# bkj/pytorch-graphsage

Measured on AMD Instinct MI355X. Metric: seed-nodes/sec, higher is better.
Workload: dtype bf16; 1 GPU; Reddit-shaped mean-aggregator 2-layer fanout 25/10 hidden 128/128 (BASELINE configs[1]); N=232965 D=602 nnz=98191232; batch_per_gpu=512, global_batch=512, rng=philox, engine=fused, launch=cmdlist, pipelined=False, batch_queue=True, parallelism=dp1, ranks=1

## Files before the change

include/gsage.h:

```cpp
#ifndef GSAGE_H
#define GSAGE_H

#include <stdint.h>

#ifdef __cplusplus
extern "C" {
#endif

#define GSAGE_ABI_VERSION 6

enum { GSAGE_F32 = 0, GSAGE_BF16 = 1, GSAGE_FP8 = 2 };
enum {
    GSAGE_OK = 0,
    GSAGE_EINVAL = -1,
    GSAGE_ELAUNCH = -2,
    GSAGE_ENODEV = -3
};
enum { GSAGE_POOL_MAX = 0, GSAGE_POOL_MEAN = 1 };
enum { GSAGE_ACT_NONE = 0, GSAGE_ACT_RELU = 1, GSAGE_ACT_TANH = 2 };

int gsage_abi_version(void);
const char *gsage_last_error(void);
uint64_t gsage_launch_count(void);
int gsage_debug_abort_trace(int fd);
int gsage_device_info(char *arch, int arch_len, int *cu_count, int *wave_size);

int gsage_stream_create_masked(const uint32_t *cu_mask, int32_t words, void **stream);
int gsage_stream_destroy(void *stream);
int gsage_event_create(void **event);
void gsage_event_destroy(void *event);
int gsage_cmdlist_replay_pair(const void *list_a, void *stream_a, void *wait_a, void *record_a,
                              const void *list_b, void *stream_b, void *wait_b, void *record_b,
                              void *then_wait_stream, int then_wait_on_b);
int gsage_cmdlist_begin(void);
int gsage_cmdlist_end(void **list);
int gsage_cmdlist_mark(int slot);
int gsage_cmdlist_time_next(int slot_a, int slot_b);
int gsage_cmdlist_elapsed(const void *list, int slot_a, int slot_b, float *ms);
int64_t gsage_cmdlist_size(const void *list);
int gsage_cmdlist_replay(const void *list, void *stream);
int gsage_cmdlist_side_begin(void);
int gsage_cmdlist_side_end(void);
int gsage_cmdlist_join(void);
void gsage_cmdlist_destroy(void *list);
typedef int (*gsage_host_fn)(void *ctx, void *stream);
int gsage_host_call(gsage_host_fn fn, void *ctx, void *stream);

int gsage_comm_load(const char *path);
int gsage_comm_unique_id(void *id128);
int gsage_comm_create(const void *id128, int32_t rank, int32_t world, void **comm);
int gsage_comm_destroy(void *comm);
int gsage_comm_all_reduce_f32(void *comm, float *buf, int64_t n, int32_t average, void *stream);
int gsage_comm_all_gather(void *comm, const void *send, void *recv, int64_t bytes, void *stream);
int gsage_comm_group(void *comm, int32_t begin, void *stream);


int gsage_sample_csr_sel(const int64_t *rowptr, const int32_t *col, int64_t n_rows,
                         const int64_t *ids, int64_t M, int32_t n, const int32_t *sel,
                         int64_t *out, int32_t *err_flag, void *stream);

int gsage_sample_dense(const int64_t *adj, int64_t ld, int64_t n_rows, const int64_t *ids, int64_t M,
                       const int64_t *keep, int32_t n, int64_t *out, int32_t *err_flag, void *stream);

int gsage_sample_csr_philox(const int64_t *rowptr, const int32_t *col, int64_t n_rows,
                            const int64_t *ids, int64_t M, int32_t n, uint32_t max_deg,
                            uint64_t seed, const uint64_t *call_ctr, uint64_t call_base,
                            uint64_t g0, int64_t *out, int32_t *sel_out, int32_t *err_flag,
                            void *stream);

int gsage_sample_hops_philox(const int64_t *rowptr, const int32_t *col, int64_t n_rows, int64_t *ids,
                             int64_t B, int32_t n_hops, const int32_t *fan, uint32_t max_deg,
                             uint64_t seed, const uint64_t *call_ctr, uint64_t call_base,
                             uint64_t rank, const int64_t *seed_queue, const int64_t *batch_idx,
                             int64_t n_batches, int32_t *err_flag, void *stream);
typedef struct gsage_hops_desc {
    const int64_t *rowptr;
    const int32_t *col;
    int64_t n_rows;
    int64_t *ids;
    int64_t B;
    int32_t n_hops;
    int32_t fan[5];
    uint32_t max_deg;
    uint64_t seed;
    const uint64_t *call_ctr;
    uint64_t call_base;
    uint64_t rank;
    const int64_t *seed_queue;
    const int64_t *batch_idx;
    int64_t batch_base;
    int64_t n_batches;
    int32_t *err_flag;
    const int32_t *sel;
    int64_t sel_stride;
    const int64_t *dense_adj;
    int64_t dense_ld;
} gsage_hops_desc;
int gsage_sample_hops(const gsage_hops_desc *hops, void *stream);

int gsage_counter_add(uint64_t *ctr, uint64_t inc, void *stream);
int gsage_copy_pair(void *dst0, const void *src0, int64_t bytes0, void *dst1, const void *src1, int64_t bytes1,
                    void *stream);

void *gsage_mt_create(uint32_t seed);
void gsage_mt_destroy(void *mt);
void gsage_mt_seed(void *mt, uint32_t seed);
int64_t gsage_mt_choice_i32(void *mt, int64_t high, int64_t count, int32_t *out);
int gsage_mt_choice_device(uint32_t *state, int64_t high, int64_t count, int32_t *out, void *stream);
int gsage_mt_choice_segments(uint32_t *state, int64_t high, int64_t n_seg, const int64_t *seg_off,
                             const int64_t *seg_cnt, int32_t *out, void *stream);

int gsage_mt_choice_par(uint32_t *state, int64_t high, int64_t n_seg, const int64_t *seg_cum, const int64_t *seg_off,
                        int64_t n_total, int32_t *out, const uint64_t *table, void *scratch, int64_t scratch_bytes,
                        int32_t n_wg, int32_t units_per_wg, void *stream);
int64_t gsage_mt_choice_par_scratch(int32_t n_wg);
int gsage_mt_jump_table(uint64_t *out, int64_t words);
int64_t gsage_mt_jump_table_words(void);
int gsage_mt_jump_host(const uint32_t *state, const uint64_t *poly, uint32_t *out);
void gsage_mt_permutation(void *mt, int64_t n, int64_t *out);

int gsage_gather_mean(const void *table, int dtype, int64_t ld, const int64_t *ids, int64_t M,
                      int32_t n, int64_t D, void *out, int out_dtype, int64_t out_ld,
                      void *stream);

int gsage_gather_mean_multi(int32_t n_seg, const void *const *tables, const int64_t *const *ids,
                            void *const *outs, const int64_t *M, const int32_t *n, int dtype,
                            int64_t ld, int64_t D, int out_dtype, int64_t out_ld, void *stream);

int gsage_quantize_fp8(const void *table, int dtype, int64_t ld, int64_t n_rows, int64_t D, void *table_q,
                       int64_t ld_q, float *scale, void *stream);

int gsage_gather_rows_fp8(const void *table_q, int64_t ld, const float *scale, const int64_t *ids, int64_t M,
                          int64_t D, void *out, int out_dtype, int64_t out_ld, void *stream);

int gsage_gather_mean_fp8(const void *table_q, int64_t ld, const float *scale, const int64_t *ids, int64_t M,
                          int32_t n, int64_t D, void *out, int out_dtype, int64_t out_ld, void *stream);
int gsage_gather_mean_multi_fp8(int32_t n_seg, const void *const *tables_q, const int64_t *const *ids,
                                void *const *outs, const int64_t *M, const int32_t *n, const float *scale,
                                int64_t ld, int64_t D, int out_dtype, int64_t out_ld, void *stream);

int gsage_segment_mean_bwd(const float *dagg, int64_t ld, int64_t M, int32_t n, int64_t D,
                           float *dneibs, int64_t out_ld, void *stream);

int gsage_scatter_add_rows(const float *rows, int64_t ld, const int64_t *ids, int64_t M,
                           int32_t n, int64_t D, float scale, float *table_grad,
                           int64_t table_ld, void *stream);

int gsage_linear_nt(const void *A, int dtype, int64_t lda, const int64_t *a_rows,
                    int a_rows_group0_only, const void *W, int64_t ldw, const float *bias,
                    void *C, int c_dtype, int64_t ldc, int64_t M, int64_t N, int64_t K, int act,
                    int groups, int64_t a_gstride, int64_t w_gstride, int64_t c_gstride,
                    void *stream);

int64_t gsage_packed_weight_elems(int64_t N, int64_t K, int32_t groups);
int gsage_pack_weight(const void *W, int dtype, int64_t ldw, int64_t w_gstride, int64_t N, int64_t K,
                      int32_t groups, void *Wp, void *stream);
int gsage_linear_nt_packed(const void *A, int64_t lda, const int64_t *a_rows, int a_rows_group0_only,
                           const void *Wp, const float *bias, void *C, int c_dtype, int64_t ldc,
                           int64_t M, int64_t N, int64_t K, int act, int groups, int64_t a_gstride,
                           int64_t c_gstride, void *stream);

int gsage_wgrad(const void *dC, int dtype, int64_t ldc, const void *A, int64_t lda, int64_t a_gstride, int64_t M,
                int64_t Ntot, int64_t K,
                int64_t n_per_group, int64_t rows_per_split, float *slabs, int64_t ldk, float *out,
                int64_t out_gstride, void *stream);
int gsage_wgrad_slabs(int64_t M, int64_t rows_per_split);
typedef struct gsage_wgrad_desc {
    const void *dC;
    const void *A;
    float *slabs;
    int64_t ldc, lda, a_gstride;
    int64_t M, Ntot, K, n_per_group, ldk, rows_per_split;
    const int64_t *a_rows;
} gsage_wgrad_desc;
int gsage_wgrad_multi(int32_t n_prob, const gsage_wgrad_desc *probs, int dtype, void *stream);
int gsage_wgrad_pair_ok(int dtype, int64_t M, int64_t Ntot, int64_t n_per_group, int64_t rows_per_split);
int gsage_wgrad_ticks_next(int64_t *tick, int64_t *tick1, int64_t inc1, int64_t *tick2, int64_t inc2);

int gsage_pool_mlp(const void *A, int dtype, int64_t lda, const int64_t *a_rows, const void *W,
                   int64_t ldw, const float *bias, int64_t M, int32_t n, int64_t H, int64_t K,
                   int pool, float *pooled, int64_t pooled_ld, int32_t *argmax, void *pooled_bf16,
                   int64_t pooled_bf16_ld, uint32_t *relu_mask, void *stream);

int gsage_pool_mlp_packed(const void *A, int64_t lda, const int64_t *a_rows, const void *Wp,
                          const float *bias, int64_t M, int32_t n, int64_t H, int64_t K, int pool,
                          float *pooled, int64_t pooled_ld, int32_t *argmax, void *pooled_bf16,
                          int64_t pooled_bf16_ld, uint32_t *relu_mask, void *stream);

int gsage_pool_route_bwd(const float *g, int64_t ldg, const float *pooled, int64_t ldp,
                         const int32_t *argmax, int64_t lda, int64_t M, int32_t n, int32_t H, void *out,
                         int out_dtype, int64_t ldo, void *stream);

int gsage_pool_route_mean_bwd(const float *g, int64_t ldg, const uint32_t *relu_mask, int64_t M, int32_t n,
                              int32_t H, void *out, int out_dtype, int64_t ldo, float *bias_part, int32_t n_part,
                              void *stream);

int gsage_pool_bias_partials(const float *g, int64_t ldg, const float *pooled, int64_t ldp, int64_t M,
                             int32_t H, float *part, int32_t n_part, void *stream);

int gsage_pool_merge_bwd(const void *Hprev, int dtype, int64_t ldh, const float *DX, int64_t ldx, int64_t r_x,
                         const float *DN, int64_t ldn, int64_t r0, void *dH, int64_t ldo, int64_t R,
                         int32_t D, void *stream);

int gsage_attn_aggregate(const float *na, int64_t na_ld, const float *xa, int64_t xa_ld,
                         const void *table, int dtype, int64_t ld, const int64_t *ids, int64_t M,
                         int32_t n, int64_t Ha, int64_t D, float *agg, int64_t agg_ld, float *ws,
                         void *stream);
int gsage_attn_aggregate_lp(const float *na, int64_t na_ld, const float *xa, int64_t xa_ld, const void *table,
                            int dtype, int64_t ld, const int64_t *ids, int64_t M, int32_t n, int64_t Ha, int64_t D,
                            float *agg, int64_t agg_ld, float *ws, void *agg_lp, int64_t agg_lp_ld, void *stream);
int gsage_attn_mlp2_fwd(const void *hid, int dtype, int64_t ldh, const void *W2, int64_t ldw, float *a, int64_t lda,
                        int64_t M, int32_t Ha, void *stream);
int gsage_attn_mlp2_bwd(const float *dan, int64_t ldn, const float *dax, int64_t ldx, const void *hid, int dtype,
                        int64_t ldh, const void *W2T, int64_t ldw, void *da, int64_t ldda, void *dhid, int64_t lddh,
                        int64_t M, int32_t Ha, void *stream);
int gsage_attn_bwd(const float *g, int64_t g_ld, const float *ws, const float *na, int64_t na_ld,
                   const float *xa, int64_t xa_ld, const void *table, int dtype, int64_t ld,
                   const int64_t *ids, int64_t M, int32_t n, int64_t Ha, int64_t D, float *dna,
                   int64_t dna_ld, float *dxa, int64_t dxa_ld, void *stream);

int gsage_attn_fused_ok(int dtype, int64_t ld, int64_t D, int32_t n, int64_t Ha);
int gsage_attn_fused_fwd(const void *table, int dtype, int64_t ld, const int64_t *ids, int64_t row0, const void *W0,
                         int64_t ldw0, const void *W2, int64_t ldw2, const float *xa, int64_t xa_ld, int64_t M,
                         int32_t n, int64_t D, void *hid, int64_t hid_ld, float *a, int64_t a_ld, float *ws, void *agg_lp,
                         int64_t lp_ld, void *stream);
int gsage_attn_fused_bwd(const void *table, int dtype, int64_t ld, const int64_t *ids, int64_t row0, const void *W2T,
                         int64_t ldw2t, const float *g, int64_t g_ld, const float *ws, const float *na, int64_t na_ld,
                         const float *xa, int64_t xa_ld, const void *hid, int64_t hid_ld, int64_t M, int32_t n, int64_t D,
                         void *da, int64_t da_ld, void *dhid, int64_t dhid_ld, float *dxa, int64_t dxa_ld, void *stream);

int gsage_prep_rows_ok(int dtype, int64_t E);
int gsage_prep_rows_fwd(const float *table, int64_t ldt, const int64_t *ids, int64_t n_seed, int64_t spare, const void *W,
                        int64_t ldw, const float *bias, int64_t M, int64_t E, void *eraw, int64_t lde, void *out,
                        int64_t ldo, void *stream);
int gsage_prep_rows_bwd(const void *dhid, int64_t lddh, const void *W0T, int64_t ldw0t, const float *DATT, int64_t ldatt,
                        const float *DX, int64_t ldx, int64_t r_x, const float *DAGG, int64_t ldagg, const float *ws,
                        int32_t n_hops, const int64_t *off, const int32_t *fan, int64_t R, int64_t E, void *din0,
                        int64_t ldd, float *bias_part, int32_t n_part, const void *WpT, int64_t ldwpt, const int64_t *ids,
                        int64_t n_seed, int64_t spare, float *g_table, int64_t ldg, float *deraw, int64_t ldde,
                        void *stream);

int gsage_lstm_ok(int dtype, int64_t H, int32_t n);
int gsage_lstm_tile(int dtype, int64_t M, int64_t H, int backward);
int64_t gsage_lstm_packed_elems(int64_t H);
int gsage_lstm_pack_whh(const float *W_hh, int64_t ldw, int64_t H, int dtype, void *Wp, void *stream);
int gsage_lstm_fwd(void *gates, int dtype, int64_t ldg, const void *Wp, int64_t M, int32_t n, int64_t H, float *cseq,
                   void *hprev, int64_t ldh, void *out, int64_t ldo, void *stream);
int gsage_lstm_bwd(const void *gates, int dtype, int64_t ldg, const void *Wp, int64_t M, int32_t n, int64_t H,
                   const float *cseq, const float *dh, int64_t lddh, void *dG, int64_t lddg, float *carry, void *stream);

int gsage_add_cast(const float *a, int64_t lda, const float *b, int64_t ldb, void *dst, int dst_dtype, int64_t ldd,
                   int64_t M, int64_t D, void *stream);
int gsage_tanh_bwd(const float *g, int64_t ldg, const void *hid, int dtype, int64_t ldh, void *out, int64_t ldo,
                   int64_t M, int64_t D, void *stream);
int gsage_attn_merge_bwd(const void *H, int h_dtype, int64_t ldh, const float *DATT, int64_t ldatt, const float *DX,
                         int64_t ldx, int64_t r_x, const float *DAGG, int64_t ldagg, const float *ws, void *out,
                         int out_dtype, int64_t ldo, int64_t R, int32_t D, int32_t n_hops, const int64_t *off,
                         const int32_t *fan, void *stream);
int gsage_attn_merge_bwd2(const void *H, int h_dtype, int64_t ldh, const float *DATT, int64_t ldatt, const float *DX,
                         int64_t ldx, int64_t r_x, const float *DAGG, int64_t ldagg, const float *ws, void *out,
                         int out_dtype, int64_t ldo, int64_t R, int32_t D, int32_t n_hops, const int64_t *off,
                         const int32_t *fan, void *out2_bf16, int64_t ldo2,
                          void *stream);

int gsage_head_l1(const float *E, int64_t lde, const float *W, const float *bias, const float *targets, int64_t B,
                  int64_t D, float *preds, void *dE, int dE_dtype, int64_t ldd, float *scratch, void *stream);
int gsage_head_l1_scratch(int64_t B, int64_t D);
int gsage_head_l1_sharded(const float *E, int64_t lde, const float *W, const float *bias, const float *targets,
                          int64_t T, int64_t B, int64_t D, float *preds, void *dE, int dE_dtype, int64_t ldd,
                          float *scratch, void *stream);

int gsage_head_ce(const float *E, int64_t lde, const float *W, const float *bias,
                  const int64_t *targets, int32_t B, int32_t C, int32_t D, float *preds, void *dE,
                  int dE_dtype, int64_t ldd, float *dW, float *db, float *loss, float *scratch,
                  const int64_t *batch_idx, int64_t n_batches, void *stream);
int64_t gsage_head_ce_scratch(int32_t B, int32_t C, int32_t D);

int gsage_head_wide(const float *E, int64_t lde, const float *W, const float *bias, const void *targets, int task,
                    int64_t ldy, int32_t B, int32_t C, int32_t D, float *preds, void *dE, int dE_dtype, int64_t ldd,
                    float *dW, float *db, float *loss, float *scratch, const int64_t *batch_idx, int64_t n_batches,
                    void *stream);
int64_t gsage_head_wide_scratch(int32_t B, int32_t C, int32_t D);

typedef struct gsage_tail_gather_desc {
    const void *table;
    const int64_t *ids;
    void *out;
    int64_t ld, out_ld, D, rows;
    int32_t n, n_workgroups;
} gsage_tail_gather_desc;
int gsage_mean_tail_ce(const void *H, int32_t B, int32_t n, const void *w2, int64_t ldw2,
                       const void *w2t, int64_t ldw2t, const float *Wfc, const float *bfc, int32_t C,
                       const int64_t *targets, const int64_t *batch_idx, int64_t n_batches, void *agg,
                       void *dE, float *preds, void *dH, float *partial,
                       const gsage_tail_gather_desc *gather, int dtype, void *stream);
int gsage_gather_role_next(const gsage_tail_gather_desc *gather);
int gsage_hops_role_next(const gsage_hops_desc *hops);
int64_t gsage_mean_tail_ce_scratch(int32_t B, int32_t C);
int gsage_mean_tail_mfma(const void *H, int32_t B, int32_t n, const void *w2, int64_t ldw2,
                         const void *w2t, int64_t ldw2t, const float *Wfc, const float *bfc, int32_t C,
                         const int64_t *targets, const int64_t *batch_idx, int64_t n_batches, void *agg,
                         void *dE, float *preds, void *dH, float *partial,
                         const gsage_tail_gather_desc *gather, void *stream);
int64_t gsage_mean_tail_mfma_scratch(int32_t B, int32_t C);
int32_t gsage_mean_tail_mfma_sampler_wgs(int64_t B, int64_t widest);


int gsage_clip_adam_step(float *p, float *g, float *m, float *v, int64_t n, float *partial,
                         const float *lr, int64_t *step, float beta1, float beta2, float eps,
                         float weight_decay, float max_norm, float *norm_out, int step_is_current,
                         int32_t n_partial_ready, const void *prep_descs, int32_t n_prep,
                         int64_t *tick1, int64_t inc1, int64_t *tick2, int64_t inc2, void *stream);
typedef struct gsage_adam_desc {
    float *p, *g, *m, *v;
    int64_t n;
    float *partial;
    const float *lr;
    int64_t *step;
    float beta1, beta2, eps, weight_decay, max_norm;
    float *norm_out;
    int32_t step_is_current, n_partial_ready;
    const void *prep_descs;
    int32_t n_prep;
    int64_t *tick1;
    int64_t inc1;
    int64_t *tick2;
    int64_t inc2;
    uint64_t *norm_slots;
    const void *reduce_descs;
    int32_t n_reduce;
} gsage_adam_desc;
int gsage_clip_adam_meet(const gsage_adam_desc *adam, void *stream);
int gsage_gather_adam_capacity(int dtype, int64_t lds_bytes);
int gsage_head_n_valid_next(const int32_t *n_valid);
int gsage_head_n_valid_pending(void);

int gsage_gather_mean_multi_adam(int32_t n_seg, const void *const *tables, const int64_t *const *ids,
                                 void *const *outs, const int64_t *M, const int32_t *n, int dtype,
                                 int64_t ld, int64_t D, int out_dtype, int64_t out_ld,
                                 const gsage_adam_desc *adam, const gsage_hops_desc *hops, void *stream);

typedef struct {
    const float *src;
    int64_t stride;
    int64_t out_off;
    int32_t S, rows, cols, ld;
} gsage_reduce_desc;
int gsage_finalize_grads(const void *descs, int32_t n_desc, int64_t max_elems, float *flat_g,
                         float *partial_sq, int64_t *tick, int64_t *tick1, int64_t inc1,
                         int64_t *tick2, int64_t inc2, void *stream);
int gsage_finalize_partials(int32_t n_desc, int64_t max_elems);
int gsage_grad_sqnorm(const float *g, int64_t n, float *partial, int32_t n_partial, void *stream);
int gsage_zero_rows(float *table, int64_t ld, const int64_t *ids, int64_t M, int64_t D, void *stream);
int gsage_colsum_partials(const float *src, int64_t ld, int64_t M, int32_t D, float *part, int32_t n_part, void *stream);
int gsage_adam_partials(int64_t n);

typedef struct gsage_row_adam {
    float *p, *g, *m, *v;
    int32_t *last, *seen;
    float *hist;
    const float *lr;
    const int64_t *step;
    int64_t n_rows;
    int32_t E, hist_cap;
    float beta1, beta2, eps, weight_decay, max_norm;
    int32_t sorted_ids;
} gsage_row_adam;
int gsage_rows_catch_up(const gsage_row_adam *d, const int64_t *ids0, int64_t n0, const int64_t *ids1, int64_t n1,
                        int32_t step_off, void *stream);
int gsage_rows_catch_up_all(const gsage_row_adam *d, int32_t step_off, void *stream);
int gsage_rows_sqnorm(const gsage_row_adam *d, const int64_t *ids0, int64_t n0, const int64_t *ids1, int64_t n1,
                      int32_t step_off, float *partial, int32_t n_partial, void *stream);
int gsage_rows_adam(const gsage_row_adam *d, const int64_t *ids0, int64_t n0, const int64_t *ids1, int64_t n1,
                    int32_t step_off, const float *partial, int32_t n_partial_ready, void *stream);

int64_t gsage_sort_rows_temp_bytes(int64_t n, int32_t key_bits);
int gsage_sort_rows(const int64_t *ids0, int64_t n0, int64_t tail_id, int64_t n_tail, int32_t key_bits,
                    int64_t *ids_sorted, int32_t *pos_sorted, void *temp, int64_t temp_bytes, void *stream);
int gsage_segment_sum_rows(const int64_t *ids_sorted, const int32_t *pos_sorted, int64_t n, const float *rows0,
                           int64_t ld0, int64_t n0, const float *rows1, int64_t ld1, int32_t E, float scale,
                           float *table, int64_t ldt, void *stream);

typedef struct {
    const float *src;
    uint16_t *dst;
    uint16_t *dst_t;
    int32_t rows, cols, dst_ld, dst_t_ld;
    uint16_t *dst_p;
    int64_t kc_p;
    int32_t dst_f32;
    int32_t reserved;
} gsage_prep_desc;
int gsage_prep_weights(const void *descs, int32_t n_desc, int64_t max_elems, int64_t *tick0,
                       int64_t inc0, int64_t *tick1, int64_t inc1, void *stream);

int gsage_bwd_merge(const void *H, int dtype, int64_t ldh, const float *DG, int64_t ldg, int64_t dagg_off,
                    void *dH, int64_t ldo, int64_t R, int64_t r_x, int32_t D, int32_t n_hops,
                    const int64_t *off, const int32_t *fan, void *stream);

int gsage_metric_f1(const float *logits, int64_t ld, const void *targets, int multilabel, int targets_f32,
                    int64_t ldy, int64_t B, int32_t C, int32_t *counts, double *out, void *stream);
int gsage_metric_mae(const float *y_true, const float *y_pred, int64_t n, double *out, void *stream);

enum { GSAGE_SEG_MEAN = 0, GSAGE_SEG_MAX = 1, GSAGE_SEG_SOFTMAX_WEIGHTED = 2, GSAGE_SEG_WEIGHTED_MEAN = 3 };
int64_t gsage_segment_reduce_ldp(int64_t D);
int gsage_segment_reduce(int mode, const void *table, int dtype, int64_t ld, int64_t D, const float *keys,
                         int64_t ldk, const int64_t *rowptr, const int32_t *col, int64_t n_rows,
                         const int32_t *order, int64_t n_short, const int64_t *slices, int64_t n_slices,
                         const int64_t *long_rows, int64_t n_long, int32_t slice_len, float *partials,
                         int64_t ldp, void *out, int out_dtype, int64_t out_ld, int act, int32_t *err_flag,
                         void *stream);

int gsage_unsup_batch(const int64_t *rowptr, const int32_t *col, int64_t n_rows, const int64_t *seeds, int64_t B,
                      int32_t walk_len, int64_t Q, const double *cdf, double cdf_total, uint64_t seed,
                      const uint64_t *call_ctr, uint64_t call_base, uint64_t g0, int64_t *ids, float *pair_w,
                      int32_t *err_flag, void *stream);

int gsage_head_skipgram(const float *E, int64_t lde, int32_t B, int32_t Q, int32_t D, const float *pair_w,
                        float neg_weight, void *dE, int dE_dtype, int64_t ldd, float *loss, float *aff, float *scratch,
                        void *stream);
int64_t gsage_head_skipgram_scratch(int32_t B, int32_t Q, int32_t D);

int gsage_head_skipgram_live(const float *E, int64_t lde, int32_t B, int32_t Q, int32_t D, const float *pair_w,
                             float neg_weight, const int32_t *n_valid, void *dE, int dE_dtype, int64_t ldd, float *loss,
                             float *aff, float *scratch, void *stream);

int gsage_edge_cdf_build(const int64_t *rowptr, const float *weight, int64_t n_rows, uint64_t *cdf, void *stream);
int gsage_sample_csr_weighted(const int64_t *rowptr, const int32_t *col, const uint64_t *cdf, int64_t n_rows,
                              const int64_t *ids, int64_t M, int32_t n, uint64_t seed, const uint64_t *call_ctr,
                              uint64_t call_base, uint64_t g0, int64_t *out, int32_t *err_flag, void *stream);
int gsage_segment_reduce_weighted(const void *table, int dtype, int64_t ld, int64_t D, const int64_t *rowptr,
                                  const int32_t *col, const uint64_t *cdf, int64_t n_rows, const int32_t *order,
                                  int64_t n_short, const int64_t *slices, int64_t n_slices, const int64_t *long_rows,
                                  int64_t n_long, int32_t slice_len, float *partials, int64_t ldp, void *out,
                                  int out_dtype, int64_t out_ld, int act, int32_t *err_flag, void *stream);

int64_t gsage_closure_span(void);
int gsage_closure_seed_count(const int64_t *queries, int64_t nq, int64_t n_rows, int32_t *local, int64_t *sums,
                             int64_t *counts, int32_t *err_flag, void *stream);
int gsage_closure_seed_write(const int64_t *queries, int64_t nq, int64_t n_rows, int32_t *local, const int64_t *sums,
                             int64_t *set, int64_t n_set, int64_t *pos, void *stream);
int gsage_closure_expand_count(const int64_t *rowptr, const int32_t *col, int64_t n_rows, const int64_t *set, int64_t lo,
                               int64_t hi, const int32_t *local, uint32_t *bitmap, int64_t *sums_words,
                               int64_t *sums_rows, int64_t *counts, int32_t *err_flag, void *stream);
int gsage_closure_expand_write(const int64_t *rowptr, const int32_t *col, const uint64_t *cdf, int64_t n_rows,
                               int64_t *set, int64_t n_dst, int32_t *local, uint32_t *bitmap, const int64_t *sums_words,
                               const int64_t *sums_rows, int64_t *blk_rowptr, int32_t *blk_col, uint64_t *blk_cdf,
                               int32_t *err_flag, void *stream);
int gsage_closure_restore(const int64_t *set, int64_t n, int32_t *local, void *stream);
int gsage_segment_reduce_block(int mode, const void *table, int dtype, int64_t ld, int64_t D, const float *keys,
                               int64_t ldk, const int64_t *rowptr, const int32_t *col, const uint64_t *cdf,
                               int64_t n_dst, int64_t n_src, int64_t dummy, const int32_t *order, int64_t n_short,
                               const int64_t *slices, int64_t n_slices, const int64_t *long_rows, int64_t n_long,
                               int32_t slice_len, float *partials, int64_t ldp, void *out, int out_dtype,
                               int64_t out_ld, int act, int32_t *err_flag, void *stream);

int64_t gsage_topk_ip_workspace(int64_t Q, int64_t N, int64_t k, int64_t splits, int64_t *splits_used);
int gsage_topk_ip(const void *table, int table_dtype, int64_t ldt, int64_t N, const void *queries, int query_dtype,
                  int64_t ldq, int64_t Q, int64_t D, const int64_t *query_ids, const int64_t *rowptr,
                  const int32_t *col, int exclude, int32_t k, int32_t splits, void *workspace, int64_t workspace_bytes,
                  int64_t *out_ids, float *out_scores, void *stream);

int64_t gsage_rank_ip_workspace(int64_t Q, int64_t N, int64_t splits, int64_t *splits_used);
int gsage_rank_ip(const void *table, int table_dtype, int64_t ldt, int64_t N, const void *queries, int query_dtype,
                  int64_t ldq, int64_t Q, int64_t D, const int64_t *target_ids, const int64_t *query_ids,
                  const int64_t *rowptr, const int32_t *col, int exclude, int32_t splits, void *workspace,
                  int64_t workspace_bytes, int64_t *out_rank, float *out_score, int32_t *err_flag, void *stream);

int64_t gsage_probe_pass_scratch(int64_t n, int32_t C, int32_t D, int32_t splits);
int gsage_probe_loss_index_next(const int64_t *index);
int gsage_probe_pass(const void *table, int dtype, int64_t ldx, int64_t N, const int64_t *ids, int64_t n,
                     const void *targets, int task, int64_t ldy, const float *W, const float *bias, int32_t C,
                     int32_t D, int32_t splits, float *partial, float *loss_out, void *stream);

#ifdef __cplusplus
}
#endif
#endif
```

pytorch-graphsage_amd/_native.py:

```python
import ctypes
import os

_HERE = os.path.dirname(os.path.abspath(__file__))
LIB_PATH = os.path.join(_HERE, "libgsage_hip.so")

F32, BF16, FP8 = 0, 1, 2
POOL_MAX, POOL_MEAN = 0, 1
ACT_NONE, ACT_RELU, ACT_TANH = 0, 1, 2
SEG_MEAN, SEG_MAX, SEG_SOFTMAX_WEIGHTED, SEG_WEIGHTED_MEAN = 0, 1, 2, 3
ABI_VERSION = 6

_vp = ctypes.c_void_p
_i64 = ctypes.c_int64
_i32 = ctypes.c_int32
_u32 = ctypes.c_uint32
_u64 = ctypes.c_uint64
_int = ctypes.c_int
_f32 = ctypes.c_float

SIGNATURES = {
    "gsage_abi_version": (_int, []),
    "gsage_last_error": (ctypes.c_char_p, []),
    "gsage_launch_count": (_u64, []),
    "gsage_debug_abort_trace": (_int, [_int]),
    "gsage_device_info": (_int, [ctypes.c_char_p, _int, ctypes.POINTER(_int), ctypes.POINTER(_int)]),
    "gsage_stream_create_masked": (_int, [_vp, _i32, ctypes.POINTER(_vp)]),
    "gsage_stream_destroy": (_int, [_vp]),
    "gsage_event_create": (_int, [ctypes.POINTER(_vp)]),
    "gsage_event_destroy": (None, [_vp]),
    "gsage_cmdlist_replay_pair": (_int, [_vp, _vp, _vp, _vp, _vp, _vp, _vp, _vp, _vp, _int]),
    "gsage_cmdlist_begin": (_int, []),
    "gsage_cmdlist_end": (_int, [ctypes.POINTER(_vp)]),
    "gsage_cmdlist_mark": (_int, [_int]),
    "gsage_cmdlist_time_next": (_int, [_int, _int]),
    "gsage_cmdlist_elapsed": (_int, [_vp, _int, _int, ctypes.POINTER(_f32)]),
    "gsage_cmdlist_size": (_i64, [_vp]),
    "gsage_cmdlist_replay": (_int, [_vp, _vp]),
    "gsage_cmdlist_side_begin": (_int, []),
    "gsage_cmdlist_side_end": (_int, []),
    "gsage_cmdlist_join": (_int, []),
    "gsage_cmdlist_destroy": (None, [_vp]),
    "gsage_host_call": (_int, [_vp, _vp, _vp]),
    "gsage_comm_load": (_int, [ctypes.c_char_p]),
    "gsage_comm_unique_id": (_int, [_vp]),
    "gsage_comm_create": (_int, [_vp, _i32, _i32, ctypes.POINTER(_vp)]),
    "gsage_comm_destroy": (_int, [_vp]),
    "gsage_comm_all_reduce_f32": (_int, [_vp, _vp, _i64, _i32, _vp]),
    "gsage_comm_all_gather": (_int, [_vp, _vp, _vp, _i64, _vp]),
    "gsage_comm_group": (_int, [_vp, _i32, _vp]),
    "gsage_sort_rows_temp_bytes": (_i64, [_i64, _i32]),
    "gsage_sort_rows": (_int, [_vp, _i64, _i64, _i64, _i32, _vp, _vp, _vp, _i64, _vp]),
    "gsage_segment_sum_rows": (_int, [_vp, _vp, _i64, _vp, _i64, _i64, _vp, _i64, _i32, _f32, _vp, _i64, _vp]),
    "gsage_head_l1_sharded": (_int, [_vp, _i64, _vp, _vp, _vp, _i64, _i64, _i64, _vp, _vp, _int, _i64, _vp, _vp]),
    "gsage_sample_csr_sel": (_int, [_vp, _vp, _i64, _vp, _i64, _i32, _vp, _vp, _vp, _vp]),
    "gsage_sample_dense": (_int, [_vp, _i64, _i64, _vp, _i64, _vp, _i32, _vp, _vp, _vp]),
    "gsage_sample_csr_philox": (_int, [_vp, _vp, _i64, _vp, _i64, _i32, _u32, _u64, _vp, _u64, _u64,
                                       _vp, _vp, _vp, _vp]),
    "gsage_sample_hops_philox": (_int, [_vp, _vp, _i64, _vp, _i64, _i32, _vp, _u32, _u64, _vp, _u64, _u64,
                                        _vp, _vp, _i64, _vp, _vp]),
    "gsage_sample_hops": (_int, [_vp, _vp]),
    "gsage_counter_add": (_int, [_vp, _u64, _vp]),
    "gsage_copy_pair": (_int, [_vp, _vp, _i64, _vp, _vp, _i64, _vp]),
    "gsage_mt_create": (_vp, [_u32]),
    "gsage_mt_destroy": (None, [_vp]),
    "gsage_mt_seed": (None, [_vp, _u32]),
    "gsage_mt_choice_i32": (_i64, [_vp, _i64, _i64, _vp]),
    "gsage_mt_permutation": (None, [_vp, _i64, _vp]),
    "gsage_mt_choice_device": (_int, [_vp, _i64, _i64, _vp, _vp]),
    "gsage_mt_choice_segments": (_int, [_vp, _i64, _i64, _vp, _vp, _vp, _vp]),
    "gsage_mt_choice_par": (_int, [_vp, _i64, _i64, _vp, _vp, _i64, _vp, _vp, _vp, _i64, _i32, _i32, _vp]),
    "gsage_mt_choice_par_scratch": (_i64, [_i32]),
    "gsage_mt_jump_table": (_int, [_vp, _i64]),
    "gsage_mt_jump_table_words": (_i64, []),
    "gsage_mt_jump_host": (_int, [_vp, _vp, _vp]),
    "gsage_head_n_valid_next": (_int, [_vp]),
    "gsage_head_n_valid_pending": (_int, []),
    "gsage_gather_role_next": (_int, [_vp]),
    "gsage_hops_role_next": (_int, [_vp]),
    "gsage_gather_mean": (_int, [_vp, _int, _i64, _vp, _i64, _i32, _i64, _vp, _int, _i64, _vp]),
    "gsage_gather_mean_multi": (_int, [_i32, _vp, _vp, _vp, _vp, _vp, _int, _i64, _i64, _int, _i64, _vp]),
    "gsage_gather_mean_multi_adam": (_int, [_i32, _vp, _vp, _vp, _vp, _vp, _int, _i64, _i64, _int, _i64,
                                            _vp, _vp, _vp]),
    "gsage_quantize_fp8": (_int, [_vp, _int, _i64, _i64, _i64, _vp, _i64, _vp, _vp]),
    "gsage_gather_rows_fp8": (_int, [_vp, _i64, _vp, _vp, _i64, _i64, _vp, _int, _i64, _vp]),
    "gsage_gather_mean_fp8": (_int, [_vp, _i64, _vp, _vp, _i64, _i32, _i64, _vp, _int, _i64, _vp]),
    "gsage_gather_mean_multi_fp8": (_int, [_i32, _vp, _vp, _vp, _vp, _vp, _vp, _i64, _i64, _int, _i64, _vp]),
    "gsage_segment_mean_bwd": (_int, [_vp, _i64, _i64, _i32, _i64, _vp, _i64, _vp]),
    "gsage_scatter_add_rows": (_int, [_vp, _i64, _vp, _i64, _i32, _i64, _f32, _vp, _i64, _vp]),
    "gsage_linear_nt": (_int, [_vp, _int, _i64, _vp, _int, _vp, _i64, _vp, _vp, _int, _i64, _i64,
                               _i64, _i64, _int, _int, _i64, _i64, _i64, _vp]),
    "gsage_packed_weight_elems": (_i64, [_i64, _i64, _i32]),
    "gsage_pack_weight": (_int, [_vp, _int, _i64, _i64, _i64, _i64, _i32, _vp, _vp]),
    "gsage_linear_nt_packed": (_int, [_vp, _i64, _vp, _int, _vp, _vp, _vp, _int, _i64, _i64, _i64, _i64, _int,
                                      _int, _i64, _i64, _vp]),
    "gsage_wgrad": (_int, [_vp, _int, _i64, _vp, _i64, _i64, _i64, _i64, _i64, _i64, _i64, _vp, _i64, _vp,
                           _i64, _vp]),
    "gsage_wgrad_slabs": (_int, [_i64, _i64]),
    "gsage_pool_route_bwd": (_int, [_vp, _i64, _vp, _i64, _vp, _i64, _i64, _i32, _i32, _vp, _int, _i64, _vp]),
    "gsage_wgrad_multi": (_int, [_i32, _vp, _int, _vp]),
    "gsage_wgrad_pair_ok": (_int, [_int, _i64, _i64, _i64, _i64]),
    "gsage_wgrad_ticks_next": (_int, [_vp, _vp, _i64, _vp, _i64]),
    "gsage_clip_adam_meet": (_int, [_vp, _vp]),
    "gsage_gather_adam_capacity": (_int, [_int, _i64]),
    "gsage_head_ce": (_int, [_vp, _i64, _vp, _vp, _vp, _i32, _i32, _i32, _vp, _vp, _int, _i64, _vp, _vp,
                             _vp, _vp, _vp, _i64, _vp]),
    "gsage_head_ce_scratch": (_i64, [_i32, _i32, _i32]),
    "gsage_head_wide": (_int, [_vp, _i64, _vp, _vp, _vp, _int, _i64, _i32, _i32, _i32, _vp, _vp, _int, _i64, _vp, _vp,
                               _vp, _vp, _vp, _i64, _vp]),
    "gsage_head_wide_scratch": (_i64, [_i32, _i32, _i32]),
    "gsage_mean_tail_ce": (_int, [_vp, _i32, _i32, _vp, _i64, _vp, _i64, _vp, _vp, _i32, _vp, _vp, _i64,
                                  _vp, _vp, _vp, _vp, _vp, _vp, _int, _vp]),
    "gsage_mean_tail_ce_scratch": (_i64, [_i32, _i32]),
    "gsage_mean_tail_mfma": (_int, [_vp, _i32, _i32, _vp, _i64, _vp, _i64, _vp, _vp, _i32, _vp, _vp, _i64,
                                    _vp, _vp, _vp, _vp, _vp, _vp, _vp]),
    "gsage_mean_tail_mfma_scratch": (_i64, [_i32, _i32]),
    "gsage_mean_tail_mfma_sampler_wgs": (_i32, [_i64, _i64]),
    "gsage_clip_adam_step": (_int, [_vp, _vp, _vp, _vp, _i64, _vp, _vp, _vp, _f32, _f32, _f32, _f32,
                                    _f32, _vp, _int, _i32, _vp, _i32, _vp, _i64, _vp, _i64, _vp]),
    "gsage_finalize_grads": (_int, [_vp, _i32, _i64, _vp, _vp, _vp, _vp, _i64, _vp, _i64, _vp]),
    "gsage_finalize_partials": (_int, [_i32, _i64]),
    "gsage_grad_sqnorm": (_int, [_vp, _i64, _vp, _i32, _vp]),
    "gsage_zero_rows": (_int, [_vp, _i64, _vp, _i64, _i64, _vp]),
    "gsage_colsum_partials": (_int, [_vp, _i64, _i64, _i32, _vp, _i32, _vp]),
    "gsage_rows_catch_up": (_int, [_vp, _vp, _i64, _vp, _i64, _i32, _vp]),
    "gsage_rows_catch_up_all": (_int, [_vp, _i32, _vp]),
    "gsage_rows_sqnorm": (_int, [_vp, _vp, _i64, _vp, _i64, _i32, _vp, _i32, _vp]),
    "gsage_rows_adam": (_int, [_vp, _vp, _i64, _vp, _i64, _i32, _vp, _i32, _vp]),
    "gsage_adam_partials": (_int, [_i64]),
    "gsage_prep_weights": (_int, [_vp, _i32, _i64, _vp, _i64, _vp, _i64, _vp]),
    "gsage_bwd_merge": (_int, [_vp, _int, _i64, _vp, _i64, _i64, _vp, _i64, _i64, _i64, _i32, _i32, _vp,
                               _vp, _vp]),
    "gsage_pool_mlp": (_int, [_vp, _int, _i64, _vp, _vp, _i64, _vp, _i64, _i32, _i64, _i64, _int,
                              _vp, _i64, _vp, _vp, _i64, _vp, _vp]),
    "gsage_pool_mlp_packed": (_int, [_vp, _i64, _vp, _vp, _vp, _i64, _i32, _i64, _i64, _int, _vp, _i64, _vp, _vp,
                                     _i64, _vp, _vp]),
    "gsage_pool_route_mean_bwd": (_int, [_vp, _i64, _vp, _i64, _i32, _i32, _vp, _int, _i64, _vp, _i32, _vp]),
    "gsage_pool_bias_partials": (_int, [_vp, _i64, _vp, _i64, _i64, _i32, _vp, _i32, _vp]),
    "gsage_pool_merge_bwd": (_int, [_vp, _int, _i64, _vp, _i64, _i64, _vp, _i64, _i64, _vp, _i64, _i64, _i32, _vp]),
    "gsage_attn_aggregate": (_int, [_vp, _i64, _vp, _i64, _vp, _int, _i64, _vp, _i64, _i32, _i64,
                                    _i64, _vp, _i64, _vp, _vp]),
    "gsage_attn_aggregate_lp": (_int, [_vp, _i64, _vp, _i64, _vp, _int, _i64, _vp, _i64, _i32, _i64,
                                       _i64, _vp, _i64, _vp, _vp, _i64, _vp]),
    "gsage_attn_fused_ok": (_int, [_int, _i64, _i64, _i32, _i64]),
    "gsage_attn_fused_fwd": (_int, [_vp, _int, _i64, _vp, _i64, _vp, _i64, _vp, _i64, _vp, _i64, _i64, _i32, _i64, _vp,
                                    _i64, _vp, _i64, _vp, _vp, _i64, _vp]),
    "gsage_attn_fused_bwd": (_int, [_vp, _int, _i64, _vp, _i64, _vp, _i64, _vp, _i64, _vp, _vp, _i64, _vp, _i64, _vp, _i64,
                                    _i64, _i32, _i64, _vp, _i64, _vp, _i64, _vp, _i64, _vp]),
    "gsage_prep_rows_ok": (_int, [_int, _i64]),
    "gsage_prep_rows_fwd": (_int, [_vp, _i64, _vp, _i64, _i64, _vp, _i64, _vp, _i64, _i64, _vp, _i64, _vp, _i64, _vp]),
    "gsage_prep_rows_bwd": (_int, [_vp, _i64, _vp, _i64, _vp, _i64, _vp, _i64, _i64, _vp, _i64, _vp, _i32, _vp, _vp, _i64,
                                   _i64, _vp, _i64, _vp, _i32, _vp, _i64, _vp, _i64, _i64, _vp, _i64, _vp, _i64, _vp]),
    "gsage_lstm_ok": (_int, [_int, _i64, _i32]),
    "gsage_lstm_tile": (_int, [_int, _i64, _i64, _int]),
    "gsage_lstm_packed_elems": (_i64, [_i64]),
    "gsage_lstm_pack_whh": (_int, [_vp, _i64, _i64, _int, _vp, _vp]),
    "gsage_lstm_fwd": (_int, [_vp, _int, _i64, _vp, _i64, _i32, _i64, _vp, _vp, _i64, _vp, _i64, _vp]),
    "gsage_lstm_bwd": (_int, [_vp, _int, _i64, _vp, _i64, _i32, _i64, _vp, _vp, _i64, _vp, _i64, _vp, _vp]),
    "gsage_attn_mlp2_fwd": (_int, [_vp, _int, _i64, _vp, _i64, _vp, _i64, _i64, _i32, _vp]),
    "gsage_attn_mlp2_bwd": (_int, [_vp, _i64, _vp, _i64, _vp, _int, _i64, _vp, _i64, _vp, _i64, _vp, _i64, _i64, _i32,
                                   _vp]),
    "gsage_add_cast": (_int, [_vp, _i64, _vp, _i64, _vp, _int, _i64, _i64, _i64, _vp]),
    "gsage_tanh_bwd": (_int, [_vp, _i64, _vp, _int, _i64, _vp, _i64, _i64, _i64, _vp]),
    "gsage_attn_merge_bwd": (_int, [_vp, _int, _i64, _vp, _i64, _vp, _i64, _i64, _vp, _i64, _vp, _vp, _int, _i64,
                                    _i64, _i32, _i32, _vp, _vp, _vp]),
    "gsage_attn_merge_bwd2": (_int, [_vp, _int, _i64, _vp, _i64, _vp, _i64, _i64, _vp, _i64, _vp, _vp, _int, _i64,
                                     _i64, _i32, _i32, _vp, _vp, _vp, _i64, _vp]),
    "gsage_head_l1": (_int, [_vp, _i64, _vp, _vp, _vp, _i64, _i64, _vp, _vp, _int, _i64, _vp, _vp]),
    "gsage_head_l1_scratch": (_int, [_i64, _i64]),
    "gsage_metric_f1": (_int, [_vp, _i64, _vp, _int, _int, _i64, _i64, _i32, _vp, _vp, _vp]),
    "gsage_metric_mae": (_int, [_vp, _vp, _i64, _vp, _vp]),
    "gsage_segment_reduce_ldp": (_i64, [_i64]),
    "gsage_segment_reduce": (_int, [_int, _vp, _int, _i64, _i64, _vp, _i64, _vp, _vp, _i64, _vp, _i64, _vp, _i64,
                                    _vp, _i64, _i32, _vp, _i64, _vp, _int, _i64, _int, _vp, _vp]),
    "gsage_attn_bwd": (_int, [_vp, _i64, _vp, _vp, _i64, _vp, _i64, _vp, _int, _i64, _vp, _i64, _i32, _i64, _i64,
                              _vp, _i64, _vp, _i64, _vp]),
    "gsage_unsup_batch": (_int, [_vp, _vp, _i64, _vp, _i64, _i32, _i64, _vp, ctypes.c_double, _u64, _vp, _u64, _u64,
                                 _vp, _vp, _vp, _vp]),
    "gsage_head_skipgram": (_int, [_vp, _i64, _i32, _i32, _i32, _vp, _f32, _vp, _int, _i64, _vp, _vp, _vp, _vp]),
    "gsage_head_skipgram_scratch": (_i64, [_i32, _i32, _i32]),
    "gsage_head_skipgram_live": (_int, [_vp, _i64, _i32, _i32, _i32, _vp, _f32, _vp, _vp, _int, _i64, _vp, _vp, _vp,
                                        _vp]),
    "gsage_edge_cdf_build": (_int, [_vp, _vp, _i64, _vp, _vp]),
    "gsage_sample_csr_weighted": (_int, [_vp, _vp, _vp, _i64, _vp, _i64, _i32, _u64, _vp, _u64, _u64, _vp, _vp, _vp]),
    "gsage_segment_reduce_weighted": (_int, [_vp, _int, _i64, _i64, _vp, _vp, _vp, _i64, _vp, _i64, _vp, _i64, _vp, _i64,
                                             _i32, _vp, _i64, _vp, _int, _i64, _int, _vp, _vp]),
    "gsage_closure_span": (_i64, []),
    "gsage_closure_seed_count": (_int, [_vp, _i64, _i64, _vp, _vp, _vp, _vp, _vp]),
    "gsage_closure_seed_write": (_int, [_vp, _i64, _i64, _vp, _vp, _vp, _i64, _vp, _vp]),
    "gsage_closure_expand_count": (_int, [_vp, _vp, _i64, _vp, _i64, _i64, _vp, _vp, _vp, _vp, _vp, _vp, _vp]),
    "gsage_closure_expand_write": (_int, [_vp, _vp, _vp, _i64, _vp, _i64, _vp, _vp, _vp, _vp, _vp, _vp, _vp, _vp, _vp]),
    "gsage_closure_restore": (_int, [_vp, _i64, _vp, _vp]),
    "gsage_segment_reduce_block": (_int, [_int, _vp, _int, _i64, _i64, _vp, _i64, _vp, _vp, _vp, _i64, _i64, _i64, _vp,
                                          _i64, _vp, _i64, _vp, _i64, _i32, _vp, _i64, _vp, _int, _i64, _int, _vp, _vp]),
    "gsage_topk_ip_workspace": (_i64, [_i64, _i64, _i64, _i64, ctypes.POINTER(_i64)]),
    "gsage_topk_ip": (_int, [_vp, _int, _i64, _i64, _vp, _int, _i64, _i64, _i64, _vp, _vp, _vp, _int, _i32, _i32, _vp,
                             _i64, _vp, _vp, _vp]),
    "gsage_rank_ip_workspace": (_i64, [_i64, _i64, _i64, ctypes.POINTER(_i64)]),
    "gsage_rank_ip": (_int, [_vp, _int, _i64, _i64, _vp, _int, _i64, _i64, _i64, _vp, _vp, _vp, _vp, _int, _i32, _vp, _i64,
                             _vp, _vp, _vp, _vp]),
    "gsage_probe_pass_scratch": (_i64, [_i64, _i32, _i32, _i32]),
    "gsage_probe_loss_index_next": (_int, [_vp]),
    "gsage_probe_pass": (_int, [_vp, _int, _i64, _i64, _vp, _i64, _vp, _int, _i64, _vp, _vp, _i32, _i32, _i32, _vp, _vp,
                                _vp]),
}


class NativeLibraryError(RuntimeError):
    pass


_LIB = None


def lib():
    global _LIB
    if _LIB is not None:
        return _LIB
    if not os.path.exists(LIB_PATH):
        raise NativeLibraryError(
            "libgsage_hip.so is missing (%s). Build it with `make hip` or "
            "`python -c 'import __graft_entry__ as g; g.build()'`; there is no fallback path."
            % LIB_PATH)
    try:
        L = ctypes.CDLL(LIB_PATH)
    except OSError as e:
        raise NativeLibraryError("cannot load %s: %s" % (LIB_PATH, e))
    for name, (res, args) in SIGNATURES.items():
        try:
            fn = getattr(L, name)
        except AttributeError:
            raise NativeLibraryError("%s does not export %s (stale build?)" % (LIB_PATH, name))
        fn.restype = res
        fn.argtypes = args
    if L.gsage_abi_version() != ABI_VERSION:
        raise NativeLibraryError("ABI version mismatch: library %d, binding %d"
                                 % (L.gsage_abi_version(), ABI_VERSION))
    _LIB = L
    return _LIB


def available():
    try:
        lib()
        return True
    except NativeLibraryError:
        return False


def check(rc, what=""):
    if rc != 0:
        msg = lib().gsage_last_error()
        raise RuntimeError("gsage %s failed (%d): %s" % (what, rc, msg.decode() if msg else "?"))


def launch_count():
    return int(lib().gsage_launch_count())


class HopsDesc(ctypes.Structure):
    _fields_ = [("rowptr", _vp), ("col", _vp), ("n_rows", _i64), ("ids", _vp), ("B", _i64),
                ("n_hops", _i32), ("fan", _i32 * 5), ("max_deg", _u32), ("seed", _u64),
                ("call_ctr", _vp), ("call_base", _u64), ("rank", _u64), ("seed_queue", _vp),
                ("batch_idx", _vp), ("batch_base", _i64), ("n_batches", _i64), ("err_flag", _vp),
                ("sel", _vp), ("sel_stride", _i64), ("dense_adj", _vp), ("dense_ld", _i64)]


class AdamDesc(ctypes.Structure):
    _fields_ = [("p", _vp), ("g", _vp), ("m", _vp), ("v", _vp), ("n", _i64), ("partial", _vp),
                ("lr", _vp), ("step", _vp), ("beta1", _f32), ("beta2", _f32), ("eps", _f32),
                ("weight_decay", _f32), ("max_norm", _f32), ("norm_out", _vp),
                ("step_is_current", _i32), ("n_partial_ready", _i32), ("prep_descs", _vp),
                ("n_prep", _i32), ("tick1", _vp), ("inc1", _i64), ("tick2", _vp), ("inc2", _i64),
                ("norm_slots", _vp), ("reduce_descs", _vp), ("n_reduce", _i32)]


class RowAdamDesc(ctypes.Structure):
    _fields_ = [("p", _vp), ("g", _vp), ("m", _vp), ("v", _vp), ("last", _vp), ("seen", _vp), ("hist", _vp),
                ("lr", _vp), ("step", _vp), ("n_rows", _i64), ("E", _i32), ("hist_cap", _i32), ("beta1", _f32),
                ("beta2", _f32), ("eps", _f32), ("weight_decay", _f32), ("max_norm", _f32), ("sorted_ids", _i32)]


class TailGatherDesc(ctypes.Structure):
    _fields_ = [("table", _vp), ("ids", _vp), ("out", _vp), ("ld", _i64), ("out_ld", _i64), ("D", _i64),
                ("rows", _i64), ("n", _i32), ("n_workgroups", _i32)]


class WgradDesc(ctypes.Structure):
    _fields_ = [("dC", _vp), ("A", _vp), ("slabs", _vp), ("ldc", _i64), ("lda", _i64),
                ("a_gstride", _i64), ("M", _i64), ("Ntot", _i64), ("K", _i64), ("n_per_group", _i64),
                ("ldk", _i64), ("rows_per_split", _i64), ("a_rows", _vp)]


class CommandList(object):

    def __init__(self):
        self._h = None

    @classmethod
    def record(cls):
        return _Recorder(cls())

    def __len__(self):
        return int(lib().gsage_cmdlist_size(self._h)) if self._h else 0

    def replay(self, stream):
        check(lib().gsage_cmdlist_replay(self._h, stream), "cmdlist_replay")

    def elapsed_ms(self, slot_a, slot_b):
        ms = _f32(0.0)
        check(lib().gsage_cmdlist_elapsed(self._h, slot_a, slot_b, ctypes.byref(ms)), "cmdlist_elapsed")
        return float(ms.value)

    def __del__(self):
        if self._h and _LIB is not None:
            _LIB.gsage_cmdlist_destroy(self._h)
            self._h = None


class _Recorder(object):
    def __init__(self, cl):
        self.cl = cl

    def __enter__(self):
        check(lib().gsage_cmdlist_begin(), "cmdlist_begin")
        return self.cl

    def __exit__(self, et, ev, tb):
        h = _vp()
        rc = lib().gsage_cmdlist_end(ctypes.byref(h))
        if rc == 0:
            self.cl._h = h.value
        if et is None:
            check(rc, "cmdlist_end")
        return False


HOST_FN = ctypes.CFUNCTYPE(_int, _vp, _vp)


def host_call(fn, stream=None):
    def tramp(_ctx, s):
        try:
            fn(s)
            return 0
        except Exception:
            import traceback
            traceback.print_exc()
            return 1
    cb = HOST_FN(tramp)
    check(lib().gsage_host_call(ctypes.cast(cb, _vp), None, stream), "host_call")
    return cb


class NativeComm(object):

    @staticmethod
    def load():
        import torch
        cand = os.path.join(os.path.dirname(torch.__file__), "lib", "librccl.so")
        check(lib().gsage_comm_load(cand.encode() if os.path.exists(cand) else None), "comm_load")

    def __init__(self, rank, world, exchange_id):
        self.load()
        buf = ctypes.create_string_buffer(128)
        err = None
        if rank == 0:
            try:
                check(lib().gsage_comm_unique_id(buf), "comm_unique_id")
            except Exception as e:
                err = e
        raw = exchange_id((b"\0" * 128 if err is not None else bytes(buf.raw)) if rank == 0 else None)
        if err is not None:
            raise err
        if len(raw) != 128 or raw == b"\0" * 128:
            raise NativeLibraryError("gsage_comm_unique_id failed on rank 0: no RCCL id to join")
        h = _vp()
        check(lib().gsage_comm_create(ctypes.create_string_buffer(raw, 128), rank, world, ctypes.byref(h)), "comm_create")
        self._h, self.rank, self.world = h.value, rank, world

    def all_reduce(self, t, average, stream):
        assert t.dtype.is_floating_point and t.element_size() == 4 and t.is_contiguous()
        check(lib().gsage_comm_all_reduce_f32(self._h, t.data_ptr(), t.numel(), 1 if average else 0, stream),
              "comm_all_reduce_f32")

    def all_gather(self, send, recv, stream):
        nbytes = send.numel() * send.element_size()
        assert send.is_contiguous() and recv.is_contiguous() and recv.numel() * recv.element_size() == nbytes * self.world
        check(lib().gsage_comm_all_gather(self._h, send.data_ptr(), recv.data_ptr(), nbytes, stream), "comm_all_gather")

    def group(self, begin, stream):
        check(lib().gsage_comm_group(self._h, 1 if begin else 0, stream), "comm_group")

    def close(self):
        if self._h and _LIB is not None:
            _LIB.gsage_comm_destroy(self._h)
        self._h = None


def device_info():
    arch = ctypes.create_string_buffer(64)
    cu, ws = _int(0), _int(0)
    rc = lib().gsage_device_info(arch, 64, ctypes.byref(cu), ctypes.byref(ws))
    if rc != 0:
        return None
    return {"arch": arch.value.decode(), "cu_count": cu.value, "wave_size": ws.value}
```

pytorch-graphsage_amd/csrc/gsage_packed.hip:

```cpp
#include "gsage_common.h"
#include "gsage_gather_dev.h"
#include "gsage_mma_dev.h"
#include "gsage_sample_dev.h"

namespace gsage {

#ifndef GSAGE_WP_R
#define GSAGE_WP_R 4
#endif
constexpr int WP_R = GSAGE_WP_R;
constexpr int WP_WAIT = ((6 * (WP_R - 1)) & 15) | (7 << 4) | (15 << 8) | (((6 * (WP_R - 1)) >> 4) << 14);
static_assert(WP_R == 4 || WP_R == 6 || WP_R == 8, "WP_R");
static_assert(WP_R != 4 || WP_WAIT == 0x4F72, "vmcnt(18)");
constexpr int WP_NBUF = WP_R + 1;
constexpr int WP_UNROLL = 24;

struct PackedParams {
    const uint16_t *A;
    const uint16_t *Wp;
    const float *bias;
    const int64_t *a_rows;
    void *C;
    int64_t lda, ldc;
    int64_t M, N, K;
    int64_t a_gstride, wp_gstride, c_gstride;
    int32_t kc_total;
    int32_t a_rows_group0_only;
    int32_t c_dtype;
};

constexpr int WP_SMEM_VEC = (BM * (BN + 4) * 4) / 16 > WP_NBUF * (BM * CH) ? (BM * (BN + 4) * 4) / 16 : WP_NBUF * (BM * CH);

template <int ACT, int GN, bool HOPS>
__global__ void __launch_bounds__(256)
k_linear_nt_packed(const PackedParams p, const TailGather tg, const HopsParams hp)
{
    constexpr int EPC = 8;
    constexpr int ATILE = BM * CH;
    __shared__ vec16 smem[WP_SMEM_VEC];
    if (HOPS && blockIdx.z + 1 == gridDim.z) {
        sample_hops_workgroup<false>(hp, (int)(blockIdx.y * gridDim.x + blockIdx.x), reinterpret_cast<int64_t *>(smem));
        return;
    }
    if (GN > 0 && blockIdx.z + 1 == gridDim.z) {
        gather_role<(GN > 0 ? GN : 1), 2>(tg, (int)(blockIdx.y * gridDim.x + blockIdx.x));
        return;
    }

    const int tid = threadIdx.x;
    const int lane = tid & 63;
    const int wave = tid >> 6;
    const int g = blockIdx.z;
    const int64_t m0 = (int64_t)blockIdx.x * BM;
    const int64_t n0 = (int64_t)blockIdx.y * BN;
    const uint16_t *A = p.A + (int64_t)g * p.a_gstride;
    const int64_t *a_rows = (p.a_rows && (g == 0 || !p.a_rows_group0_only)) ? p.a_rows : nullptr;
    const int nk = (int)((p.K + 63) / 64);
    const int64_t jb_last = (p.N - 1) >> 5;
    const int64_t jb = min((n0 >> 5) + wave, jb_last);
    const vec16 *wp = reinterpret_cast<const vec16 *>(p.Wp + (int64_t)g * p.wp_gstride) +
                      (jb * p.kc_total) * 64 + lane;

    const int cdst = lane & 7;
    const uint16_t *a_src[2];
#pragma unroll
    for (int s2 = 0; s2 < 2; ++s2) {
        const int R = 32 * s2 + 8 * wave + (lane >> 3);
        const int row = (R & ~9) | ((R & 1) << 3) | ((R >> 3) & 1);
        int64_t m = m0 + row;
        if (m >= p.M) m = p.M - 1;
        const int64_t r = a_rows ? a_rows[m] : m;
        a_src[s2] = A + r * p.lda + (cdst ^ (row & 7)) * EPC;
    }
    const int a_dst0 = (8 * wave) * CH, a_dst1 = (32 + 8 * wave) * CH;

    vec16 wr[WP_R][4];
    auto issue_tile = [&](int kt, int buf, vec16 (&w)[4]) {
        vec16 *base = smem + buf * ATILE;
        const int64_t ko = (int64_t)kt * 64;
        __builtin_amdgcn_sched_barrier(0);
        __builtin_amdgcn_global_load_lds((global_void_t *)(a_src[0] + ko), (lds_void_t *)(base + a_dst0), 16, 0, 0);
        __builtin_amdgcn_global_load_lds((global_void_t *)(a_src[1] + ko), (lds_void_t *)(base + a_dst1), 16, 0, 0);
#pragma unroll
        for (int kk = 0; kk < 4; ++kk) w[kk] = wp[(int64_t)(kt * 4 + kk) * 64];
        __builtin_amdgcn_sched_barrier(0);
    };

    f32x16_t acc0, acc1;
#pragma unroll
    for (int r = 0; r < 16; ++r) { acc0[r] = 0.f; acc1[r] = 0.f; }
    const int arow0 = lane & 31, arow1 = arow0 + 32;

    auto compute_tile = [&](int kt, const vec16 (&w)[4]) {
        const vec16 *sA = smem + (kt % WP_NBUF) * ATILE;
        vec16 fa0[4], fa1[4];
#pragma unroll
        for (int kk = 0; kk < 4; ++kk) {
            const int ch = kk * 2 + (lane >> 5);
            fa0[kk] = sA[lds_slot(arow0, ch)];
            fa1[kk] = sA[lds_slot(arow1, ch)];
        }
        __builtin_amdgcn_s_waitcnt(0xC07F);
        __builtin_amdgcn_sched_barrier(0);
#pragma unroll
        for (int kk = 0; kk < 4; ++kk) {
            mma_chunk<uint16_t>::run(fa0[kk], w[kk], acc0);
            mma_chunk<uint16_t>::run(fa1[kk], w[kk], acc1);
        }
        __builtin_amdgcn_sched_barrier(0);
    };

    int kt = 0, phase = 0;
    if (nk > WP_R) {
#pragma unroll
        for (int t = 0; t < WP_R; ++t) issue_tile(t, t, wr[t]);
#pragma unroll
        for (int u = 0; u < WP_UNROLL; ++u) {
            if (kt + WP_R >= nk) { phase = u % WP_R; goto drain; }
            __builtin_amdgcn_s_waitcnt(WP_WAIT);
            __builtin_amdgcn_s_barrier();
            compute_tile(kt, wr[u % WP_R]);
            issue_tile(kt + WP_R, (kt + WP_R) % WP_NBUF, wr[u % WP_R]);
            ++kt;
        }
        for (;;) {
#pragma unroll
            for (int s = 0; s < WP_R; ++s) {
                if (kt + WP_R >= nk) { phase = s; goto drain; }
                __builtin_amdgcn_s_waitcnt(WP_WAIT);
                __builtin_amdgcn_s_barrier();
                compute_tile(kt, wr[s]);
                issue_tile(kt + WP_R, (kt + WP_R) % WP_NBUF, wr[s]);
                ++kt;
            }
        }
    } else {
#pragma unroll
        for (int t = 0; t < WP_R; ++t)
            if (t < nk) issue_tile(t, t, wr[t]);
    }
drain:
    __builtin_amdgcn_s_waitcnt(0x0F70);
    __builtin_amdgcn_s_barrier();
#pragma unroll
    for (int t = 0; t < WP_R; ++t) {
        if (kt + t < nk) {
            const int idx = (phase + t) % WP_R;
#pragma unroll
            for (int s = 0; s < WP_R; ++s)
                if (idx == s) compute_tile(kt + t, wr[s]);
        }
    }

    const float *bias = p.bias ? p.bias + (int64_t)g * p.N : nullptr;
    const int esz = p.c_dtype == GSAGE_BF16 ? 2 : 4;
    const int epc = 16 / esz;
    const int64_t cbase = (int64_t)g * p.c_gstride + n0;
    const bool wide = n0 + BN <= p.N && p.ldc % epc == 0 && cbase % epc == 0 && ((uintptr_t)p.C % 16) == 0;
    const int jl = wave * 32 + (lane & 31);
    const float bj = (bias && n0 + jl < p.N) ? bias[n0 + jl] : 0.f;
    if (wide) {
        __syncthreads();
        const int ldt = BN + epc;
#pragma unroll
        for (int rb = 0; rb < 2; ++rb) {
            const f32x16_t &acc = rb ? acc1 : acc0;
#pragma unroll
            for (int r = 0; r < 16; ++r) {
                const int i = rb * 32 + (r & 3) + 8 * (r >> 2) + 4 * (lane >> 5);
                const float v = apply_act(acc[r] + bj, ACT);
                if (p.c_dtype == GSAGE_BF16)
                    ((uint16_t *)smem)[i * ldt + jl] = f32_to_bf16(v);
                else
                    ((float *)smem)[i * ldt + jl] = v;
            }
        }
        __syncthreads();
        const int cpr = BN / epc;
        for (int q = tid; q < BM * cpr; q += 256) {
            const int row = q / cpr, ch = q - row * cpr;
            const int64_t m = m0 + row;
            if (m < p.M) {
                const vec16 v = *reinterpret_cast<const vec16 *>((const char *)smem +
                                                                 ((size_t)row * ldt + ch * epc) * esz);
                *reinterpret_cast<vec16 *>((char *)p.C + ((size_t)m * p.ldc + cbase + ch * epc) * esz) = v;
            }
        }
        return;
    }
    const int64_t j = n0 + jl;
#pragma unroll
    for (int rb = 0; rb < 2; ++rb) {
        const f32x16_t &acc = rb ? acc1 : acc0;
#pragma unroll
        for (int r = 0; r < 16; ++r) {
            const int64_t m = m0 + rb * 32 + (r & 3) + 8 * (r >> 2) + 4 * (lane >> 5);
            if (m < p.M && j < p.N) {
                const float v = apply_act(acc[r] + bj, ACT);
                const int64_t off = m * p.ldc + (int64_t)g * p.c_gstride + j;
                if (p.c_dtype == GSAGE_BF16)
                    ((uint16_t *)p.C)[off] = f32_to_bf16(v);
                else
                    ((float *)p.C)[off] = v;
            }
        }
    }
}

constexpr int WS_TPW = 8;
constexpr int WS_LDT = BN + 8;

template <int NK> constexpr int ws_ring() { return NK == 3 ? 3 : 4; }
template <int NK> constexpr size_t ws_lds_bytes()
{
    return (size_t)(ws_ring<NK>() + 1) * BM * CH * 16 + (size_t)BM * WS_LDT * 2 + (size_t)WS_TPW * 2 * 256 * 4;
}

template <int N>
__device__ __forceinline__ void ws_wait_vm()
{
    static_assert(N >= 0 && N < 64, "vmcnt is six bits");
    asm volatile("s_waitcnt vmcnt(%0)" ::"n"(N) : "memory");
}

template <int BASE, int STEP>
__device__ __forceinline__ void ws_wait_vm_sel(int t)
{
    if (t == 0) ws_wait_vm<BASE>();
    else if (t == 1) ws_wait_vm<BASE + STEP>();
    else if (t == 2) ws_wait_vm<BASE + 2 * STEP>();
    else ws_wait_vm<BASE + 3 * STEP>();
}

template <int ACT, int NK>
__global__ void __launch_bounds__(256)
k_linear_nt_packed_ws(const PackedParams p, const int tpw)
{
    constexpr int R = ws_ring<NK>(), TR = R / NK, NBUF = R + 1, ATILE = BM * CH, NST = 4;
    constexpr int STEADY = 2 * (R - 1) + NST * TR;
    extern __shared__ __attribute__((aligned(16))) char ws_smem[];
    vec16 *ring = reinterpret_cast<vec16 *>(ws_smem);
    uint16_t *stage = reinterpret_cast<uint16_t *>(ws_smem + (size_t)NBUF * ATILE * 16);
    uint32_t *rid_s = reinterpret_cast<uint32_t *>(ws_smem + (size_t)NBUF * ATILE * 16 + (size_t)BM * WS_LDT * 2);

    const int tid = threadIdx.x, lane = tid & 63;
    const int wave = __builtin_amdgcn_readfirstlane(tid >> 6);
    const int g = blockIdx.z;
    const int64_t n0 = (int64_t)blockIdx.y * BN;
    const int64_t n_tiles = (p.M + BM - 1) / BM;
    const int64_t tile0 = (int64_t)blockIdx.x * tpw;
    const uint16_t *A = p.A + (int64_t)g * p.a_gstride;
    const int64_t *a_rows = (p.a_rows && (g == 0 || !p.a_rows_group0_only)) ? p.a_rows : nullptr;

    const int cdst = lane & 7;
    int rowof[2];
#pragma unroll
    for (int s2 = 0; s2 < 2; ++s2) {
        const int Rr = 32 * s2 + 8 * wave + (lane >> 3);
        rowof[s2] = (Rr & ~9) | ((Rr & 1) << 3) | ((Rr >> 3) & 1);
    }
    for (int t = 0; t < tpw; ++t) {
        int64_t tile = tile0 + t;
        if (tile >= n_tiles) tile = n_tiles - 1;
#pragma unroll
        for (int s2 = 0; s2 < 2; ++s2) {
            int64_t m = tile * BM + rowof[s2];
            if (m >= p.M) m = p.M - 1;
            rid_s[(t * 2 + s2) * 256 + tid] = (uint32_t)(a_rows ? a_rows[m] : m);
        }
    }
    const vec16 *wp = reinterpret_cast<const vec16 *>(p.Wp + (int64_t)g * p.wp_gstride) +
                      (((n0 >> 5) + wave) * p.kc_total) * 64 + lane;
    vec16 wr[NK][4];
#pragma unroll
    for (int kt = 0; kt < NK; ++kt)
#pragma unroll
        for (int kk = 0; kk < 4; ++kk) wr[kt][kk] = wp[(int64_t)(kt * 4 + kk) * 64];
    const int jl = wave * 32 + (lane & 31);
    float bj = p.bias ? p.bias[(int64_t)g * p.N + n0 + jl] : 0.f;
    const uint32_t ring_lds = (uint32_t)(uintptr_t)(lds_void_t *)ring;
    const uint32_t dst0 = (uint32_t)((8 * wave) * CH * 16), dst1 = (uint32_t)((32 + 8 * wave) * CH * 16);

    auto issue = [&](int t, int kt, int buf) {
        const int tc = t < tpw ? t : tpw - 1;
        const uint32_t r0 = rid_s[(tc * 2 + 0) * 256 + tid], r1 = rid_s[(tc * 2 + 1) * 256 + tid];
        const uint16_t *s0 = A + (int64_t)r0 * p.lda + (cdst ^ (rowof[0] & 7)) * 8 + kt * 64;
        const uint16_t *s1 = A + (int64_t)r1 * p.lda + (cdst ^ (rowof[1] & 7)) * 8 + kt * 64;
        const uint32_t base = ring_lds + (uint32_t)(buf * ATILE * 16);
        const uint32_t m0a = __builtin_amdgcn_readfirstlane(base + dst0), m0b = __builtin_amdgcn_readfirstlane(base + dst1);
        asm volatile("s_mov_b32 m0, %1\n\ts_nop 0\n\tglobal_load_lds_dwordx4 %0, off" ::"v"(s0), "s"(m0a) : "memory", "m0");
        asm volatile("s_mov_b32 m0, %1\n\ts_nop 0\n\tglobal_load_lds_dwordx4 %0, off" ::"v"(s1), "s"(m0b) : "memory", "m0");
    };
    f32x16_t acc0, acc1;
    const int arow0 = lane & 31, arow1 = arow0 + 32;
    auto compute = [&](int buf, const vec16 (&w)[4]) {
        const vec16 *sA = ring + buf * ATILE;
        vec16 fa0[4], fa1[4];
#pragma unroll
        for (int kk = 0; kk < 4; ++kk) {
            const int ch = kk * 2 + (lane >> 5);
            fa0[kk] = sA[lds_slot(arow0, ch)];
            fa1[kk] = sA[lds_slot(arow1, ch)];
        }
        asm volatile("s_waitcnt lgkmcnt(0)" ::: "memory");
        __builtin_amdgcn_sched_barrier(0);
#pragma unroll
        for (int kk = 0; kk < 4; ++kk) {
            mma_chunk<uint16_t>::run(fa0[kk], w[kk], acc0);
            mma_chunk<uint16_t>::run(fa1[kk], w[kk], acc1);
        }
        __builtin_amdgcn_sched_barrier(0);
    };
    auto epilogue = [&](int t) {
        int64_t tile = tile0 + t;
        if (tile >= n_tiles) tile = n_tiles - 1;
#pragma unroll
        for (int rb = 0; rb < 2; ++rb) {
            const f32x16_t &acc = rb ? acc1 : acc0;
#pragma unroll
            for (int r = 0; r < 16; ++r) {
                const int i = rb * 32 + (r & 3) + 8 * (r >> 2) + 4 * (lane >> 5);
                stage[i * WS_LDT + jl] = f32_to_bf16(apply_act(acc[r] + bj, ACT));
            }
        }
        __syncthreads();
        const int64_t cbase = (int64_t)g * p.c_gstride + n0;
#pragma unroll
        for (int u = 0; u < NST; ++u) {
            const int qd = tid + 256 * u, row = qd >> 4, ch = qd & 15;
            int64_t m = tile * BM + row;
            if (m >= p.M) m = p.M - 1;
            const vec16 v = *reinterpret_cast<const vec16 *>(stage + row * WS_LDT + ch * 8);
            *reinterpret_cast<vec16 *>((uint16_t *)p.C + m * p.ldc + cbase + ch * 8) = v;
        }
    };
    auto zero = [&]() {
#pragma unroll
        for (int r = 0; r < 16; ++r) { acc0[r] = 0.f; acc1[r] = 0.f; }
    };

    asm volatile("s_waitcnt vmcnt(0) lgkmcnt(0)" ::: "memory");
#pragma unroll
    for (int kt = 0; kt < NK; ++kt)
        asm volatile("" : "+v"(wr[kt][0]), "+v"(wr[kt][1]), "+v"(wr[kt][2]), "+v"(wr[kt][3]));
    asm volatile("" : "+v"(bj));
#pragma unroll
    for (int j = 0; j < R; ++j) issue(j / NK, j % NK, j);
    int buf = 0;
#pragma unroll
    for (int t = 0; t < TR; ++t) {
        zero();
#pragma unroll
        for (int kt = 0; kt < NK; ++kt) {
            ws_wait_vm_sel<2 * (R - 1), NST>(t);
            __builtin_amdgcn_s_barrier();
            compute(buf, wr[kt]);
            issue(t + TR, kt, (buf + R) % NBUF);
            buf = (buf + 1) % NBUF;
        }
        epilogue(t);
    }
    for (int t = TR; t < tpw; ++t) {
        zero();
#pragma unroll
        for (int kt = 0; kt < NK; ++kt) {
            ws_wait_vm<STEADY>();
            __builtin_amdgcn_s_barrier();
            compute(buf, wr[kt]);
            issue(t + TR, kt, buf == 0 ? NBUF - 1 : buf - 1);
            buf = buf + 1 == NBUF ? 0 : buf + 1;
        }
        epilogue(t);
    }
    asm volatile("s_waitcnt vmcnt(0)" ::: "memory");
}

constexpr int PK_R = 3;
constexpr int PK_NBUF = PK_R + 1;

struct PoolPackedParams {
    const uint16_t *A;
    const uint16_t *Wp;
    const float *bias;
    const int64_t *a_rows;
    int64_t lda;
    int64_t M, N, K;
    int32_t kc_total;
    int32_t pool_n, pool_groups, pool_mode;
    float *pooled;
    int64_t pooled_ld;
    uint16_t *pooled_b;
    int64_t pooled_b_ld;
    int32_t *argmax;
    uint32_t *relu_mask;
};

template <int NW, int PN>
__global__ void __launch_bounds__(NW * 64)
k_pool_mlp_packed(const PoolPackedParams p)
{
    constexpr int EPC = 8;
    constexpr int PK_BN = NW * 64;
    constexpr int PK_LDT = PK_BN + 8;
    constexpr int NDMA = 8 / NW;
    constexpr int WAIT_STEADY = NW == 8 ? 0x4F72 : 0x4F74;
    constexpr int ATILE = BM * CH;
    __shared__ vec16 smem[PN > 0 ? PK_NBUF * ATILE : (BM * PK_LDT * 4) / 16];

    const int tid = threadIdx.x;
    const int lane = tid & 63;
    const int wave = tid >> 6;
    const int rows_per_wg = p.pool_groups * p.pool_n;
    const int64_t m0 = (int64_t)blockIdx.x * rows_per_wg;
    const int64_t n0 = (int64_t)blockIdx.y * PK_BN;
    const int nk = (int)((p.K + 63) / 64);
    const int64_t jb_last = (p.N - 1) >> 5;
    const int64_t jb0 = min((n0 >> 5) + wave * 2, jb_last), jb1 = min((n0 >> 5) + wave * 2 + 1, jb_last);
    const vec16 *wp0 = reinterpret_cast<const vec16 *>(p.Wp) + (jb0 * p.kc_total) * 64 + lane;
    const vec16 *wp1 = reinterpret_cast<const vec16 *>(p.Wp) + (jb1 * p.kc_total) * 64 + lane;

    const uint16_t *a_src[NDMA];
#pragma unroll
    for (int d = 0; d < NDMA; ++d) {
        const int R = 8 * (NW * d + wave) + (lane >> 3);
        const int row = (R & ~9) | ((R & 1) << 3) | ((R >> 3) & 1);
        int64_t m = m0 + min(row, rows_per_wg - 1);
        if (m >= p.M) m = p.M - 1;
        const int64_t r = p.a_rows ? p.a_rows[m] : m;
        a_src[d] = p.A + r * p.lda + ((lane & 7) ^ (row & 7)) * EPC;
    }
    const int a_dst = (8 * wave) * CH;

    vec16 wr[PK_R][2][4];
    auto issue_tile = [&](int kt, int buf, vec16 (&w)[2][4]) {
        vec16 *base = smem + buf * ATILE;
        __builtin_amdgcn_sched_barrier(0);
#pragma unroll
        for (int d = 0; d < NDMA; ++d)
            __builtin_amdgcn_global_load_lds((global_void_t *)(a_src[d] + (int64_t)kt * 64),
                                             (lds_void_t *)(base + a_dst + 8 * NW * d * CH), 16, 0, 0);
#pragma unroll
        for (int kk = 0; kk < 4; ++kk) {
            w[0][kk] = wp0[(int64_t)(kt * 4 + kk) * 64];
            w[1][kk] = wp1[(int64_t)(kt * 4 + kk) * 64];
        }
        __builtin_amdgcn_sched_barrier(0);
    };

    f32x16_t acc[2][2];
#pragma unroll
    for (int i = 0; i < 2; ++i)
#pragma unroll
        for (int j = 0; j < 2; ++j)
#pragma unroll
            for (int r = 0; r < 16; ++r) acc[i][j][r] = 0.f;
    const int arow0 = lane & 31, arow1 = arow0 + 32;

#ifndef GSAGE_PK_READ_AHEAD
#define GSAGE_PK_READ_AHEAD 1
#endif
    auto compute_tile = [&](int kt, const vec16 (&w)[2][4]) {
        const vec16 *sA = smem + (kt % PK_NBUF) * ATILE;
        vec16 fa0[4], fa1[4];
#if GSAGE_PK_READ_AHEAD
        auto rd = [&](int kk) {
            const int ch = kk * 2 + (lane >> 5);
            fa0[kk] = sA[lds_slot(arow0, ch)];
            fa1[kk] = sA[lds_slot(arow1, ch)];
        };
        rd(0);
        rd(1);
        __builtin_amdgcn_sched_barrier(0);
#pragma unroll
        for (int kk = 0; kk < 4; ++kk) {
            if (kk < 3) __builtin_amdgcn_s_waitcnt(0xC27F);
            else __builtin_amdgcn_s_waitcnt(0xC07F);
            __builtin_amdgcn_sched_barrier(0);
            mma_chunk<uint16_t>::run(fa0[kk], w[0][kk], acc[0][0]);
            mma_chunk<uint16_t>::run(fa0[kk], w[1][kk], acc[0][1]);
            mma_chunk<uint16_t>::run(fa1[kk], w[0][kk], acc[1][0]);
            mma_chunk<uint16_t>::run(fa1[kk], w[1][kk], acc[1][1]);
            if (kk + 2 < 4) rd(kk + 2);
            __builtin_amdgcn_sched_barrier(0);
        }
#else
#pragma unroll
        for (int kk = 0; kk < 4; ++kk) {
            const int ch = kk * 2 + (lane >> 5);
            fa0[kk] = sA[lds_slot(arow0, ch)];
            fa1[kk] = sA[lds_slot(arow1, ch)];
        }
        __builtin_amdgcn_s_waitcnt(0xC07F);
        __builtin_amdgcn_sched_barrier(0);
#pragma unroll
        for (int kk = 0; kk < 4; ++kk) {
            mma_chunk<uint16_t>::run(fa0[kk], w[0][kk], acc[0][0]);
            mma_chunk<uint16_t>::run(fa0[kk], w[1][kk], acc[0][1]);
            mma_chunk<uint16_t>::run(fa1[kk], w[0][kk], acc[1][0]);
            mma_chunk<uint16_t>::run(fa1[kk], w[1][kk], acc[1][1]);
        }
        __builtin_amdgcn_sched_barrier(0);
#endif
    };

    int kt = 0, phase = 0;
    if (nk > PK_R) {
#pragma unroll
        for (int t = 0; t < PK_R; ++t) issue_tile(t, t, wr[t]);
#pragma unroll
        for (int u = 0; u < WP_UNROLL; ++u) {
            if (kt + PK_R >= nk) { phase = u % PK_R; goto drain; }
            __builtin_amdgcn_s_waitcnt(WAIT_STEADY);
            __builtin_amdgcn_s_barrier();
            compute_tile(kt, wr[u % PK_R]);
            issue_tile(kt + PK_R, (kt + PK_R) % PK_NBUF, wr[u % PK_R]);
            ++kt;
        }
        for (;;) {
#pragma unroll
            for (int s = 0; s < PK_R; ++s) {
                if (kt + PK_R >= nk) { phase = s; goto drain; }
                __builtin_amdgcn_s_waitcnt(WAIT_STEADY);
                __builtin_amdgcn_s_barrier();
                compute_tile(kt, wr[s]);
                issue_tile(kt + PK_R, (kt + PK_R) % PK_NBUF, wr[s]);
                ++kt;
            }
        }
    } else {
#pragma unroll
        for (int t = 0; t < PK_R; ++t)
            if (t < nk) issue_tile(t, t, wr[t]);
    }
drain:
    __builtin_amdgcn_s_waitcnt(0x0F70);
    __builtin_amdgcn_s_barrier();
#pragma unroll
    for (int t = 0; t < PK_R; ++t) {
        if (kt + t < nk) {
            const int idx = (phase + t) % PK_R;
#pragma unroll
            for (int s = 0; s < PK_R; ++s)
                if (idx == s) compute_tile(kt + t, wr[s]);
        }
    }

    if constexpr (PN > 0) {
        constexpr int G = BM / PN;
        const int h = lane >> 5;
        float best[2][G];
        int arg[2][G];
#pragma unroll
        for (int cb = 0; cb < 2; ++cb) {
            const int64_t jc = n0 + wave * 64 + cb * 32 + (lane & 31);
            const float bj = (p.bias && jc < p.N) ? p.bias[jc] : 0.f;
#pragma unroll
            for (int sg = 0; sg < G; ++sg) { best[cb][sg] = -1.f; arg[cb][sg] = 0; }
#pragma unroll
            for (int rb = 0; rb < 2; ++rb)
#pragma unroll
                for (int r = 0; r < 16; ++r) {
                    const int i0 = 32 * rb + (r & 3) + 8 * (r >> 2);
                    float v = acc[rb][cb][r] + bj;
                    v = v > 0.f ? v : 0.f;
#pragma unroll
                    for (int sg = 0; sg < G; ++sg) {
                        const bool in0 = i0 / PN == sg, in1 = (i0 + 4) / PN == sg;
                        if (!in0 && !in1) continue;
                        const bool mine = (in0 && in1) || (in0 ? h == 0 : h == 1);
                        const bool take = mine && v > best[cb][sg];
                        best[cb][sg] = take ? v : best[cb][sg];
                        arg[cb][sg] = take ? i0 - sg * PN + 4 * h : arg[cb][sg];
                    }
                }
#pragma unroll
            for (int sg = 0; sg < G; ++sg) {
                const float ob = __shfl_xor(best[cb][sg], 32, 64);
                const int oa = __shfl_xor(arg[cb][sg], 32, 64);
                const bool take = ob > best[cb][sg] || (ob == best[cb][sg] && oa < arg[cb][sg]);
                best[cb][sg] = take ? ob : best[cb][sg];
                arg[cb][sg] = take ? oa : arg[cb][sg];
            }
        }
        const int64_t j = n0 + wave * 64 + lane;
#pragma unroll
        for (int sg = 0; sg < G; ++sg) {
            const float bv = h ? best[1][sg] : best[0][sg];
            const int av = h ? arg[1][sg] : arg[0][sg];
            const int64_t seg = (int64_t)blockIdx.x * G + sg;
            if (seg * PN < p.M && j < p.N) {
                p.pooled[seg * p.pooled_ld + j] = bv;
                if (p.pooled_b) p.pooled_b[seg * p.pooled_b_ld + j] = f32_to_bf16(bv);
                if (p.argmax) p.argmax[seg * p.N + j] = av;
            }
        }
        return;
    }
    float *tile = reinterpret_cast<float *>(smem);
    __syncthreads();
#pragma unroll
    for (int cb = 0; cb < 2; ++cb) {
        const int jl = wave * 64 + cb * 32 + (lane & 31);
        const int64_t j = n0 + jl;
        const float bj = (p.bias && j < p.N) ? p.bias[j] : 0.f;
#pragma unroll
        for (int rb = 0; rb < 2; ++rb)
#pragma unroll
            for (int r = 0; r < 16; ++r) {
                const int i = rb * 32 + (r & 3) + 8 * (r >> 2) + 4 * (lane >> 5);
                const float v = acc[rb][cb][r] + bj;
                tile[i * PK_LDT + jl] = v > 0.f ? v : 0.f;
            }
    }
    __syncthreads();
    if (p.relu_mask) {
        for (int task = tid; task < BM * (PK_BN / 32); task += NW * 64) {
            const int i = task / (PK_BN / 32), q = task % (PK_BN / 32);
            const int64_t row = m0 + i;
            if (i < rows_per_wg && row < p.M && n0 + q * 32 < p.N) {
                uint32_t bits = 0;
#pragma unroll
                for (int e0 = 0; e0 < 32; ++e0) {
                    const int e = (e0 + i) & 31;
                    bits |= (tile[i * PK_LDT + q * 32 + e] > 0.f ? 1u : 0u) << e;
                }
                p.relu_mask[row * (p.N / 32) + (n0 >> 5) + q] = bits;
            }
        }
    }
    const int64_t j = n0 + tid;
    if (j < p.N) {
        for (int sg = 0; sg < p.pool_groups; ++sg) {
            const int64_t seg = (int64_t)blockIdx.x * p.pool_groups + sg;
            if (seg * p.pool_n >= p.M) break;
            const float *colp = tile + (sg * p.pool_n) * PK_LDT + tid;
            float best = colp[0];
            int arg = 0;
            float sum = best;
            for (int r = 1; r < p.pool_n; ++r) {
                const float v = colp[r * PK_LDT];
                sum += v;
                if (v > best) { best = v; arg = r; }
            }
            if (p.pool_mode == GSAGE_POOL_MAX) {
                p.pooled[seg * p.pooled_ld + j] = best;
                if (p.pooled_b) p.pooled_b[seg * p.pooled_b_ld + j] = f32_to_bf16(best);
                if (p.argmax) p.argmax[seg * p.N + j] = arg;
            } else {
                p.pooled[seg * p.pooled_ld + j] = sum / (float)p.pool_n;
                if (p.pooled_b) p.pooled_b[seg * p.pooled_b_ld + j] = f32_to_bf16(sum / (float)p.pool_n);
            }
        }
    }
}


template <typename TW>
__global__ void __launch_bounds__(256)
k_pack_weight(const TW *__restrict__ W, int64_t ldw, int64_t w_gstride, int64_t N, int64_t K,
              int32_t kc_total, int32_t jb_total, int32_t groups, uint16_t *__restrict__ Wp)
{
    const int64_t total = (int64_t)groups * jb_total * kc_total * 64;
    const int64_t stride = (int64_t)gridDim.x * 256;
    for (int64_t t = (int64_t)blockIdx.x * 256 + threadIdx.x; t < total; t += stride) {
        const int lane = (int)(t & 63);
        int64_t u = t >> 6;
        const int kc = (int)(u % kc_total);
        u /= kc_total;
        const int jb = (int)(u % jb_total);
        const int g = (int)(u / jb_total);
        const int64_t j = (int64_t)jb * 32 + (lane & 31);
        const int64_t k0 = (int64_t)kc * 16 + (lane >> 5) * 8;
        uint16_t out[8];
#pragma unroll
        for (int e = 0; e < 8; ++e) {
            float v = 0.f;
            if (j < N && k0 + e < K) {
                const TW w = W[(int64_t)g * w_gstride + j * ldw + k0 + e];
                v = sizeof(TW) == 2 ? bf16_to_f32((uint16_t)w) : (float)w;
            }
            out[e] = f32_to_bf16(v);
        }
        vec16 o;
#pragma unroll
        for (int e = 0; e < 4; ++e) o[e] = (uint32_t)out[2 * e] | ((uint32_t)out[2 * e + 1] << 16);
        reinterpret_cast<vec16 *>(Wp)[t] = o;
    }
}

}

using namespace gsage;

extern "C" {

int64_t gsage_packed_weight_elems(int64_t N, int64_t K, int32_t groups)
{
    return (int64_t)groups * ceil_div(N, 32) * (ceil_div(K, 64) * 4) * 64 * 8;
}

int gsage_pack_weight(const void *W, int dtype, int64_t ldw, int64_t w_gstride, int64_t N, int64_t K,
                      int32_t groups, void *Wp, void *stream)
{
    GSAGE_REQUIRE(W && Wp && N > 0 && K > 0 && groups >= 1 && ldw >= K, "pack_weight: bad arguments");
    GSAGE_REQUIRE(dtype == GSAGE_BF16 || dtype == GSAGE_F32, "pack_weight: bad dtype %d", dtype);
    GSAGE_REQUIRE(((uintptr_t)Wp % 16) == 0, "pack_weight: output must be 16-byte aligned");
    const int32_t kc = (int32_t)(ceil_div(K, 64) * 4), jb = (int32_t)ceil_div(N, 32);
    const int64_t slots = (int64_t)groups * jb * kc * 64;
    int64_t blocks = ceil_div(slots, 256);
    if (blocks > 4096) blocks = 4096;
    if (dtype == GSAGE_BF16)
        launch(k_pack_weight<uint16_t>, dim3((unsigned)blocks), dim3(256), 0, (hipStream_t)stream,
               (const uint16_t *)W, ldw, w_gstride, N, K, kc, jb, groups, (uint16_t *)Wp);
    else
        launch(k_pack_weight<float>, dim3((unsigned)blocks), dim3(256), 0, (hipStream_t)stream,
               (const float *)W, ldw, w_gstride, N, K, kc, jb, groups, (uint16_t *)Wp);
    return check_launch("pack_weight");
}

int gsage_linear_nt_packed(const void *A, int64_t lda, const int64_t *a_rows, int a_rows_group0_only,
                           const void *Wp, const float *bias, void *C, int c_dtype, int64_t ldc,
                           int64_t M, int64_t N, int64_t K, int act, int groups, int64_t a_gstride,
                           int64_t c_gstride, void *stream)
{
    const gsage_tail_gather_desc *gd = take_gather_role();
    const gsage_hops_desc *hd = t_hops_role;
    t_hops_role = nullptr;
    GSAGE_REQUIRE(A && Wp && C, "linear_nt_packed: null pointer");
    GSAGE_REQUIRE(M >= 0 && N > 0 && K > 0, "linear_nt_packed: bad sizes");
    GSAGE_REQUIRE(c_dtype == GSAGE_BF16 || c_dtype == GSAGE_F32, "linear_nt_packed: bad c_dtype");
    GSAGE_REQUIRE(groups >= 1 && groups <= 65535, "linear_nt_packed: bad group count");
    GSAGE_REQUIRE(act >= ACT_NONE && act <= ACT_TANH, "linear_nt_packed: bad activation code");
    GSAGE_REQUIRE(lda % 64 == 0 && ceil_div(K, 64) * 64 <= lda && ((uintptr_t)A % 16) == 0 &&
                  ((uintptr_t)Wp % 16) == 0, "linear_nt_packed: A rows must be whole zero-padded 128-byte lines");
    if (M == 0) return GSAGE_OK;
    PackedParams p;
    p.A = (const uint16_t *)A; p.Wp = (const uint16_t *)Wp; p.bias = bias; p.a_rows = a_rows; p.C = C;
    p.lda = lda; p.ldc = ldc; p.M = M; p.N = N; p.K = K;
    p.a_gstride = a_gstride; p.c_gstride = c_gstride;
    p.kc_total = (int32_t)(ceil_div(K, 64) * 4);
    p.wp_gstride = ceil_div(N, 32) * (int64_t)p.kc_total * 64 * 8;
    p.a_rows_group0_only = a_rows_group0_only; p.c_dtype = c_dtype;
    dim3 grid((unsigned)ceil_div(M, BM), (unsigned)ceil_div(N, BN), (unsigned)groups);
    hipStream_t s = (hipStream_t)stream;
    TailGather tg = {};
    HopsParams hp = {};
    if (hd) {
        GSAGE_REQUIRE(!(gd && gd->rows > 0) && act == ACT_RELU && !hd->dense_adj,
                      "linear_nt_packed: the sampler role rides with the ReLU projection, walks a CSR, and excludes the "
                      "gather role");
        size_t lds = 0;
        const int rc = fill_hops(hp, lds, *hd);
        if (rc != GSAGE_OK) return rc;
        const int64_t slots = (int64_t)grid.x * grid.y;
        hp.spw = (int32_t)ceil_div(hd->B > 0 ? hd->B : 1, slots);
        int64_t widest = 1, width = 1;
        for (int k = 1; k <= hp.n_hops; ++k) { width *= hp.fan[k]; widest = width > widest ? width : widest; }
        GSAGE_REQUIRE(sizeof(int64_t) * 2 * (size_t)hp.spw * (size_t)widest <= sizeof(vec16) * WP_SMEM_VEC,
                      "linear_nt_packed: the sampler role's frontier (%d seeds x %lld ids, twice) does not fit the "
                      "projection's LDS", hp.spw, (long long)widest);
        grid.z += 1;
        launch(k_linear_nt_packed<ACT_RELU, 0, true>, grid, dim3(256), 0, s, p, tg, hp);
        return check_launch("linear_nt_packed");
    }
    if (gd && gd->rows > 0) {
        const int rc = fill_gather_role(tg, *gd, "linear_nt_packed (gather role)");
        if (rc != GSAGE_OK) return rc;
        GSAGE_REQUIRE(act == ACT_RELU && (gd->n == 10 || gd->n == 5),
                      "linear_nt_packed: the gather role rides with the ReLU projection, fan-out 5 or 10");
        tg.n_wg = (int32_t)(grid.x * grid.y);
        grid.z += 1;
        if (gd->n == 10) launch(k_linear_nt_packed<ACT_RELU, 10, false>, grid, dim3(256), 0, s, p, tg, hp);
        else launch(k_linear_nt_packed<ACT_RELU, 5, false>, grid, dim3(256), 0, s, p, tg, hp);
        return check_launch("linear_nt_packed");
    }
    {
        const char *ws_env = getenv("GSAGE_K5_WS");
        const bool ws_on = !ws_env || atoi(ws_env) != 0;
        const int nk = (int)ceil_div(K, 64);
        const int tr = nk == 1 ? 4 : nk == 2 ? 2 : 1;
        const int64_t n_tiles = ceil_div(M, BM);
        if (ws_on && c_dtype == GSAGE_BF16 && nk <= 4 && N % BN == 0 && ldc % 8 == 0 && c_gstride % 8 == 0 &&
            ((uintptr_t)C % 16) == 0 && n_tiles >= 4 * tr && (act == ACT_RELU || act == ACT_NONE)) {
            int dev = 0, cus = 256;
            if (hipGetDevice(&dev) == hipSuccess) {
                int v = 0;
                if (hipDeviceGetAttribute(&v, hipDeviceAttributeMultiprocessorCount, dev) == hipSuccess && v > 0) cus = v;
                else (void)hipGetLastError();
            } else (void)hipGetLastError();
            const int64_t slices = (int64_t)grid.y * groups;
            int64_t per = ceil_div(2 * (int64_t)cus, slices);
            if (per < 1) per = 1;
            int64_t tpw = ceil_div(n_tiles, per);
            if (const char *e = getenv("GSAGE_K5_WS_TPW")) tpw = atoi(e);
            if (tpw < tr) tpw = tr;
            if (tpw > WS_TPW) tpw = WS_TPW;
            grid.x = (unsigned)ceil_div(n_tiles, tpw);
#define GSAGE_WS_LAUNCH(ACTV, NKV)                                                                                        \
            do {                                                                                                      \
                static bool raised = false;                                                                           \
                if (!raised) {                                                                                        \
                    if (hipFuncSetAttribute((const void *)k_linear_nt_packed_ws<ACTV, NKV>,                           \
                                            hipFuncAttributeMaxDynamicSharedMemorySize, (int)ws_lds_bytes<NKV>()) != hipSuccess) { \
                        (void)hipGetLastError();                                                                      \
                        set_error("linear_nt_packed: cannot raise the dynamic LDS limit");                          \
                        return GSAGE_ELAUNCH;                                                                         \
                    }                                                                                                 \
                    raised = true;                                                                                    \
                }                                                                                                     \
                launch(k_linear_nt_packed_ws<ACTV, NKV>, grid, dim3(256), ws_lds_bytes<NKV>(), s, p, (int)tpw);       \
            } while (0)
#define GSAGE_WS_NK(ACTV)                                                                                                 \
            do {                                                                                                      \
                if (nk == 1) GSAGE_WS_LAUNCH(ACTV, 1);                                                                \
                else if (nk == 2) GSAGE_WS_LAUNCH(ACTV, 2);                                                           \
                else if (nk == 3) GSAGE_WS_LAUNCH(ACTV, 3);                                                           \
                else GSAGE_WS_LAUNCH(ACTV, 4);                                                                        \
            } while (0)
            if (act == ACT_RELU) GSAGE_WS_NK(ACT_RELU);
            else GSAGE_WS_NK(ACT_NONE);
#undef GSAGE_WS_NK
#undef GSAGE_WS_LAUNCH
            return check_launch("linear_nt_packed");
        }
    }
    if (act == ACT_RELU)
        launch(k_linear_nt_packed<ACT_RELU, 0, false>, grid, dim3(256), 0, s, p, tg, hp);
    else if (act == ACT_TANH)
        launch(k_linear_nt_packed<ACT_TANH, 0, false>, grid, dim3(256), 0, s, p, tg, hp);
    else
        launch(k_linear_nt_packed<ACT_NONE, 0, false>, grid, dim3(256), 0, s, p, tg, hp);
    return check_launch("linear_nt_packed");
}

int gsage_pool_mlp_packed(const void *A, int64_t lda, const int64_t *a_rows, const void *Wp,
                          const float *bias, int64_t M, int32_t n, int64_t H, int64_t K, int pool,
                          float *pooled, int64_t pooled_ld, int32_t *argmax, void *pooled_bf16,
                          int64_t pooled_bf16_ld, uint32_t *relu_mask, void *stream)
{
    GSAGE_REQUIRE(A && Wp && pooled && pooled_ld >= H, "pool_mlp_packed: bad pointers / output");
    GSAGE_REQUIRE(M >= 0 && H > 0 && K > 0, "pool_mlp_packed: bad sizes");
    GSAGE_REQUIRE(n >= 1 && n <= BM, "pool_mlp_packed: fanout must be in [1, %d]", BM);
    GSAGE_REQUIRE(!relu_mask || H % 32 == 0, "pool_mlp_packed: relu_mask needs H % 32 == 0");
    GSAGE_REQUIRE(!pooled_bf16 || pooled_bf16_ld >= H, "pool_mlp_packed: bad bf16 output");
    GSAGE_REQUIRE(pool == GSAGE_POOL_MAX || pool == GSAGE_POOL_MEAN, "pool_mlp_packed: bad pool mode");
    GSAGE_REQUIRE(lda % 64 == 0 && ceil_div(K, 64) * 64 <= lda && ((uintptr_t)A % 16) == 0 &&
                  ((uintptr_t)Wp % 16) == 0, "pool_mlp_packed: A rows must be whole zero-padded 128-byte lines");
    if (M == 0) return GSAGE_OK;
    PoolPackedParams p;
    p.A = (const uint16_t *)A; p.Wp = (const uint16_t *)Wp; p.bias = bias; p.a_rows = a_rows; p.lda = lda;
    p.M = M * (int64_t)n; p.N = H; p.K = K; p.kc_total = (int32_t)(ceil_div(K, 64) * 4);
    p.pool_n = n; p.pool_groups = BM / n; p.pool_mode = pool; p.pooled = pooled; p.pooled_ld = pooled_ld;
    p.pooled_b = (uint16_t *)pooled_bf16; p.pooled_b_ld = pooled_bf16_ld; p.argmax = argmax;
    p.relu_mask = relu_mask;
    const int64_t subs = ceil_div(M, p.pool_groups);
    dim3 grid((unsigned)subs, (unsigned)ceil_div(H, 256), 1);
    static const bool regs = [] { const char *e = getenv("GSAGE_POOL_REGS"); return !e || atoi(e) != 0; }();
    const bool rp = regs && pool == GSAGE_POOL_MAX && !relu_mask;
    hipStream_t s = (hipStream_t)stream;
    if (rp && n == 10) launch(k_pool_mlp_packed<4, 10>, grid, dim3(256), 0, s, p);
    else if (rp && n == 25) launch(k_pool_mlp_packed<4, 25>, grid, dim3(256), 0, s, p);
    else if (rp && n == 5) launch(k_pool_mlp_packed<4, 5>, grid, dim3(256), 0, s, p);
    else if (rp && n == 15) launch(k_pool_mlp_packed<4, 15>, grid, dim3(256), 0, s, p);
    else if (rp && n == 20) launch(k_pool_mlp_packed<4, 20>, grid, dim3(256), 0, s, p);
    else launch(k_pool_mlp_packed<4, 0>, grid, dim3(256), 0, s, p);
    return check_launch("pool_mlp_packed");
}

}
```

pytorch-graphsage_amd/csrc/gsage_tail_mfma.hip:

```cpp
#include "gsage_common.h"
#include "gsage_gather_dev.h"
#include "gsage_sample_dev.h"

namespace gsage {

typedef __attribute__((ext_vector_type(8))) __bf16 tm_bf16x8;
typedef float tm_f32x4 __attribute__((ext_vector_type(4)));

constexpr int TM_S = 16;
constexpr int TM_T = 512;
constexpr int TM_D = 256;
constexpr int TM_CMAX = 64;
constexpr int TM_LDH = 264;
constexpr int TM_LDF = 260;
constexpr int TM_LDP = 68;

struct TailMfmaParams {
    const uint16_t *H;
    const uint16_t *w2;
    const uint16_t *w2t;
    const float *Wfc;
    const float *bfc;
    const int64_t *targets;
    const int64_t *batch_idx;
    int64_t n_batches;
    const int32_t *n_valid;
    uint16_t *agg;
    uint16_t *dE;
    float *preds;
    uint16_t *dH;
    float *partial;
    int64_t ldw2, ldw2t;
    int32_t B, n, C;
    int32_t stop;
    int32_t n_smp;
};

constexpr size_t tm_lds_bytes()
{
    return sizeof(float) * ((size_t)TM_CMAX * TM_LDF
                            + (size_t)TM_S * TM_LDF
                            + (size_t)8 * TM_S * TM_LDP
                            + (size_t)TM_S * TM_LDP
                            + 2 * 8 * TM_S + TM_S + 16)
           + sizeof(uint16_t) * (size_t)3 * TM_S * TM_LDH;
}
static_assert(2 * TM_S * TM_LDF <= 8 * TM_S * TM_LDP, "gxs | gns must fit the logit partials they alias");
static_assert(tm_lds_bytes() <= 160 * 1024, "seed level: LDS budget");

__device__ __forceinline__ uint32_t tm_bf16(float f)
{
    const uint32_t u = __float_as_uint(f);
    const uint32_t r = (u + 0x7fffu + ((u >> 16) & 1u)) >> 16;
    return (u & 0x7fffffffu) > 0x7f800000u ? ((u >> 16) | 0x0040u) : r;
}
__device__ __forceinline__ uint32_t tm_pack(float lo, float hi) { return tm_bf16(lo) | (tm_bf16(hi) << 16); }

__device__ __forceinline__ float tm_wave_sum(float v)
{
#pragma unroll
    for (int o = 32; o > 0; o >>= 1) v += __shfl_xor(v, o, 64);
    return v;
}
__device__ __forceinline__ float tm_wave_max(float v)
{
#pragma unroll
    for (int o = 32; o > 0; o >>= 1) v = fmaxf(v, __shfl_xor(v, o, 64));
    return v;
}
__device__ __forceinline__ float tm_sum16(float v)
{
#pragma unroll
    for (int o = 8; o > 0; o >>= 1) v += __shfl_xor(v, o, 64);
    return v;
}

typedef __attribute__((__vector_size__(4 * sizeof(unsigned int)))) unsigned int tm_u32x4;
__device__ __forceinline__ __amdgpu_buffer_rsrc_t tm_rsrc(const void *base, uint32_t bytes)
{
    return __builtin_amdgcn_make_buffer_rsrc(const_cast<void *>(base), 0, (int)bytes, 0x00020000);
}
__device__ __forceinline__ vec16 tm_bload(__amdgpu_buffer_rsrc_t r, uint32_t voff, uint32_t soff)
{
    return __builtin_bit_cast(vec16, __builtin_amdgcn_raw_buffer_load_b128(r, (int)voff, (int)soff, 0));
}

__device__ __forceinline__ tm_f32x4 tm_mma_bf16(const vec16 a, const vec16 b, const tm_f32x4 c)
{
    return __builtin_amdgcn_mfma_f32_16x16x32_bf16(__builtin_bit_cast(tm_bf16x8, a), __builtin_bit_cast(tm_bf16x8, b),
                                                   c, 0, 0, 0);
}
__device__ __forceinline__ tm_f32x4 tm_mma_f32(const float a, const float b, const tm_f32x4 c)
{
    return __builtin_amdgcn_mfma_f32_16x16x4f32(a, b, c, 0, 0, 0);
}

#ifndef GSAGE_TM_ROLE_U
#define GSAGE_TM_ROLE_U 2
#endif
template <int N, int GN>
__global__ void __launch_bounds__(TM_T)
k_mean_tail_mfma(const TailMfmaParams p, const TailGather tg, const HopsParams hp)
{
    extern __shared__ __attribute__((aligned(16))) unsigned char lds_raw[];
    if (GN > 0) {
        const int n_tail = (p.B + TM_S - 1) / TM_S;
        if ((int)blockIdx.x >= n_tail) {
            const int r = (int)blockIdx.x - n_tail;
            if (r < p.n_smp) {
                sample_hops_wide<TM_T, 4>(hp, r, reinterpret_cast<int64_t *>(lds_raw));
                return;
            }
            gather_role<(GN > 0 ? GN : 1), (GN > 10 ? 2 : GSAGE_TM_ROLE_U), TM_T>(tg, r - p.n_smp);
            return;
        }
    }
    constexpr int NB = N > 0 ? N : 32;
    float *Ws = reinterpret_cast<float *>(lds_raw);
    float *zs = Ws + TM_CMAX * TM_LDF;
    float *part = zs + TM_S * TM_LDF;
    float *gxs = part, *gns = part + TM_S * TM_LDF;
    float *dls = part + 8 * TM_S * TM_LDP;
    float *red = dls + TM_S * TM_LDP;
    float *red2 = red + 8 * TM_S;
    float *lss = red2 + 8 * TM_S;
    uint16_t *xs = reinterpret_cast<uint16_t *>(lss + TM_S + 16);
    uint16_t *as = xs + TM_S * TM_LDH;
    uint16_t *des = as + TM_S * TM_LDH;

    const int t = threadIdx.x, lane = t & 63;
    const int wave = __builtin_amdgcn_readfirstlane(t >> 6);
    const int half = lane >> 5, cg = lane & 31;
    const int li = lane & 15, lg = lane >> 4;
    const int sr = 2 * wave + half;
    const int C = p.C, n = p.n;
    const int CT = (C + 15) >> 4;
    const int64_t B = p.B;
    const int row0 = blockIdx.x * TM_S;

    const int64_t bq = p.batch_idx ? (int64_t)((uint64_t)*p.batch_idx % (uint64_t)p.n_batches) : 0;
    const int64_t *tgt = p.targets + bq * B;
    const int64_t Bv = p.n_valid ? (int64_t)min(max(p.n_valid[bq], 1), (int32_t)B) : B;

    const int64_t iw = row0 + sr;
    const bool live = iw < B;
    const int64_t iwc = live ? iw : B - 1;
    vec16 wf[8];
    {
        const __amdgpu_buffer_rsrc_t rF = tm_rsrc(p.Wfc, (uint32_t)(C * TM_D * 4));
#pragma unroll
        for (int u = 0; u < 8; ++u) wf[u] = tm_bload(rF, (uint32_t)t * 16u, (uint32_t)u * TM_T * 16u);
    }
    const __amdgpu_buffer_rsrc_t rH = tm_rsrc(p.H, (uint32_t)(B * (1 + n) * TM_D * 2));
    vec16 xraw = tm_bload(rH, (uint32_t)(iwc * TM_D + cg * 8) * 2u, 0u);
    vec16 nb[NB];
    {
        const uint32_t base = (uint32_t)((B + iwc * n) * TM_D + cg * 8) * 2u;
#pragma unroll
        for (int u = 0; u < NB; ++u) {
            if (N > 0) nb[u] = tm_bload(rH, base, (uint32_t)u * TM_D * 2u);
            else nb[u] = tm_bload(rH, base + (uint32_t)(u < n ? u : n - 1) * TM_D * 2u, 0u);
        }
    }
    const int g2 = wave >> 2;
    vec16 bw[2][8];
    const __amdgpu_buffer_rsrc_t rW = tm_rsrc(p.w2, (uint32_t)(2 * 128 * p.ldw2 * 2));
    auto load_fwd_frags = [&]() {
        const uint32_t wr = (uint32_t)(((int64_t)g2 * 128 + (wave & 3) * 32 + li) * p.ldw2 + 8 * lg) * 2u;
        const uint32_t ct1 = (uint32_t)(16 * p.ldw2) * 2u;
#pragma unroll
        for (int ks = 0; ks < 8; ++ks) {
            bw[0][ks] = tm_bload(rW, wr, 64u * ks);
            bw[1][ks] = tm_bload(rW, wr + ct1, 64u * ks);
        }
    };
    if (N > 0) load_fwd_frags();
    __builtin_amdgcn_sched_barrier(0);
#pragma unroll
    for (int u = 0; u < 8; ++u) {
        const int q = t + u * TM_T;
        *reinterpret_cast<vec16 *>(Ws + (q >> 6) * TM_LDF + (q & 63) * 4) = wf[u];
    }
    __builtin_amdgcn_sched_barrier(0);

    uint32_t mbits[(NB + 3) / 4];
    uint32_t xbits = 0;
    {
        float s[8];
#pragma unroll
        for (int e = 0; e < 8; ++e) s[e] = 0.f;
#pragma unroll
        for (int w = 0; w < (NB + 3) / 4; ++w) mbits[w] = 0;
#pragma unroll
        for (int u = 0; u < NB; ++u) {
            const bool valid = N > 0 || u < n;
#pragma unroll
            for (int e = 0; e < 8; ++e) {
                const float f = valid ? tail_elem(nb[u], e) : 0.f;
                s[e] += f;
                mbits[u >> 2] |= (f > 0.f ? 1u : 0u) << ((u & 3) * 8 + e);
            }
            asm volatile("" : "+v"(s[0]), "+v"(s[1]), "+v"(s[2]), "+v"(s[3]), "+v"(s[4]), "+v"(s[5]), "+v"(s[6]),
                         "+v"(s[7]), "+v"(mbits[u >> 2]));
            __builtin_amdgcn_sched_barrier(0);
        }
        vec16 am;
        const float fn = (float)n;
#pragma unroll
        for (int e = 0; e < 8; e += 2) am[e >> 1] = tm_pack(s[e] / fn, s[e + 1] / fn);
#pragma unroll
        for (int e = 0; e < 8; ++e) xbits |= (tail_elem(xraw, e) > 0.f ? 1u : 0u) << e;
#pragma unroll
        for (int w = 0; w < (NB + 3) / 4; ++w) asm volatile("" : "+v"(mbits[w]));
        asm volatile("" : "+v"(xbits));
        if (live) *reinterpret_cast<vec16 *>(p.agg + iw * TM_D + cg * 8) = am;
        const vec16 zero = {0u, 0u, 0u, 0u};
        *reinterpret_cast<vec16 *>(xs + sr * TM_LDH + cg * 8) = live ? xraw : zero;
        *reinterpret_cast<vec16 *>(as + sr * TM_LDH + cg * 8) = live ? am : zero;
    }
    if (N == 0) load_fwd_frags();
    const float my_bias = (lane < C) ? p.bfc[lane] : 0.f;
    const int64_t tg0 = (row0 + 2 * wave < B) ? tgt[row0 + 2 * wave] : -1;
    const int64_t tg1 = (row0 + 2 * wave + 1 < B) ? tgt[row0 + 2 * wave + 1] : -1;
    lds_barrier();
    if (p.stop == 1) return;

    tm_f32x4 acc[2];
    acc[0] = tm_f32x4{0.f, 0.f, 0.f, 0.f};
    acc[1] = acc[0];
    {
        const uint16_t *arow = (g2 ? as : xs) + li * TM_LDH + 8 * lg;
#pragma unroll
        for (int ks = 0; ks < 8; ++ks) {
            const vec16 a = *reinterpret_cast<const vec16 *>(arow + 32 * ks);
            acc[0] = tm_mma_bf16(a, bw[0][ks], acc[0]);
            acc[1] = tm_mma_bf16(a, bw[1][ks], acc[1]);
        }
    }
    const int col0 = 32 * wave + li;
#pragma unroll
    for (int r = 0; r < 4; ++r) {
        const float q = tm_sum16(acc[0][r] * acc[0][r] + acc[1][r] * acc[1][r]);
        if (li == 0) red[wave * TM_S + 4 * lg + r] = q;
    }
    vec16 bb[2][2][4];
    {
        const __amdgpu_buffer_rsrc_t rT = tm_rsrc(p.w2t, (uint32_t)(2 * TM_D * p.ldw2t * 2));
        const uint32_t wr = (uint32_t)((32 * wave + li) * p.ldw2t + 8 * lg) * 2u;
        const uint32_t ct1 = (uint32_t)(16 * p.ldw2t) * 2u, g1 = (uint32_t)(TM_D * p.ldw2t) * 2u;
#pragma unroll
        for (int g = 0; g < 2; ++g)
#pragma unroll
            for (int ct = 0; ct < 2; ++ct)
#pragma unroll
                for (int ks = 0; ks < 4; ++ks) bb[g][ct][ks] = tm_bload(rT, wr + g * g1 + ct * ct1, 64u * ks);
    }
    lds_barrier();
    float nrm[4], z[2][4];
#pragma unroll
    for (int r = 0; r < 4; ++r) {
        float ss = 0.f;
#pragma unroll
        for (int w = 0; w < 8; ++w) ss += red[w * TM_S + 4 * lg + r];
        nrm[r] = fmaxf(sqrtf(ss), 1e-12f);
#pragma unroll
        for (int ct = 0; ct < 2; ++ct) {
            z[ct][r] = acc[ct][r] / nrm[r];
            zs[(4 * lg + r) * TM_LDF + col0 + 16 * ct] = z[ct][r];
        }
    }
    lds_barrier();
    if (p.stop == 2) return;

    {
        const float *za = zs + li * TM_LDF + 32 * wave + lg;
        float a[8];
#pragma unroll
        for (int ks = 0; ks < 8; ++ks) a[ks] = za[4 * ks];
        for (int tt = 0; tt < CT; ++tt) {
            const float *wb = Ws + (16 * tt + li) * TM_LDF + 32 * wave + lg;
            tm_f32x4 lacc = {0.f, 0.f, 0.f, 0.f};
#pragma unroll
            for (int ks = 0; ks < 8; ++ks) lacc = tm_mma_f32(a[ks], wb[4 * ks], lacc);
#pragma unroll
            for (int r = 0; r < 4; ++r) part[(wave * TM_S + 4 * lg + r) * TM_LDP + 16 * tt + li] = lacc[r];
        }
    }
    lds_barrier();
    const float invB = 1.f / (float)Bv;
#pragma unroll
    for (int q = 0; q < 2; ++q) {
        const int s = 2 * wave + q;
        const int64_t i = row0 + s;
        const int64_t my_target = q ? tg1 : tg0;
        float logit = -INFINITY;
        if (lane < C) {
            float v = 0.f;
#pragma unroll
            for (int w = 0; w < 8; ++w) v += part[(w * TM_S + s) * TM_LDP + lane];
            logit = v + my_bias;
        }
        const float mx = tm_wave_max(logit);
        const float ex = (lane < C) ? expf(logit - mx) : 0.f;
        const float den = tm_wave_sum(ex);
        const bool ok = lane < C && i < Bv;
        dls[s * TM_LDP + lane] = ok ? (ex / den - ((int64_t)lane == my_target ? 1.f : 0.f)) * invB : 0.f;
        if (lane < C && i < B) p.preds[i * C + lane] = logit;
        const int tl = (my_target >= 0 && my_target < C) ? (int)my_target : 0;
        const float lt = __shfl(logit, tl, 64);
        if (lane == 0) lss[s] = (i < Bv && my_target >= 0 && my_target < C) ? -(lt - mx - logf(den)) : 0.f;
    }
    lds_barrier();
    if (p.stop == 3) return;

    {
        tm_f32x4 dz[2];
        dz[0] = tm_f32x4{0.f, 0.f, 0.f, 0.f};
        dz[1] = dz[0];
        const float *da = dls + li * TM_LDP + lg;
        const float *wb = Ws + lg * TM_LDF + col0;
        for (int ks = 0; ks < 4 * CT; ++ks) {
            const float a = da[4 * ks];
            dz[0] = tm_mma_f32(a, wb[4 * ks * TM_LDF], dz[0]);
            dz[1] = tm_mma_f32(a, wb[4 * ks * TM_LDF + 16], dz[1]);
        }
#pragma unroll
        for (int r = 0; r < 4; ++r) {
            const float q = tm_sum16(z[0][r] * dz[0][r] + z[1][r] * dz[1][r]);
            if (li == 0) red2[wave * TM_S + 4 * lg + r] = q;
        }
        lds_barrier();
#pragma unroll
        for (int r = 0; r < 4; ++r) {
            float zdz = 0.f;
#pragma unroll
            for (int w = 0; w < 8; ++w) zdz += red2[w * TM_S + 4 * lg + r];
            const bool in = row0 + 4 * lg + r < B;
#pragma unroll
            for (int ct = 0; ct < 2; ++ct) {
                const float gb = (dz[ct][r] - z[ct][r] * zdz) / nrm[r];
                des[(4 * lg + r) * TM_LDH + col0 + 16 * ct] = in ? (uint16_t)tm_bf16(gb) : (uint16_t)0;
            }
        }
    }
    {
        float *out = p.partial + (int64_t)blockIdx.x * ((int64_t)C * TM_D + C + 1);
        for (int rt = 0; rt < CT; ++rt) {
            tm_f32x4 wacc[2];
            wacc[0] = tm_f32x4{0.f, 0.f, 0.f, 0.f};
            wacc[1] = wacc[0];
#pragma unroll
            for (int ks = 0; ks < 4; ++ks) {
                const float a = dls[(4 * ks + lg) * TM_LDP + 16 * rt + li];
                const float *zb = zs + (4 * ks + lg) * TM_LDF + col0;
                wacc[0] = tm_mma_f32(a, zb[0], wacc[0]);
                wacc[1] = tm_mma_f32(a, zb[16], wacc[1]);
            }
#pragma unroll
            for (int r = 0; r < 4; ++r) {
                const int c = 16 * rt + 4 * lg + r;
                if (c < C) {
                    out[c * TM_D + col0] = wacc[0][r];
                    out[c * TM_D + col0 + 16] = wacc[1][r];
                }
            }
        }
        if (wave == 0) {
            if (lane < C) {
                float s = 0.f;
#pragma unroll
                for (int q = 0; q < TM_S; ++q) s += dls[q * TM_LDP + lane];
                out[C * TM_D + lane] = s;
            }
            if (lane == 0) {
                float s = 0.f;
#pragma unroll
                for (int q = 0; q < TM_S; ++q) s += lss[q];
                out[C * TM_D + C] = s;
            }
        }
    }
    lds_barrier();
    if (p.stop == 4) return;

    if (live) *reinterpret_cast<vec16 *>(p.dE + iw * TM_D + cg * 8) = *reinterpret_cast<const vec16 *>(des + sr * TM_LDH + cg * 8);
    {
        tm_f32x4 ga[2][2];
#pragma unroll
        for (int g = 0; g < 2; ++g)
#pragma unroll
            for (int ct = 0; ct < 2; ++ct) ga[g][ct] = tm_f32x4{0.f, 0.f, 0.f, 0.f};
        const uint16_t *drow = des + li * TM_LDH + 8 * lg;
#pragma unroll
        for (int g = 0; g < 2; ++g)
#pragma unroll
            for (int ks = 0; ks < 4; ++ks) {
                const vec16 a = *reinterpret_cast<const vec16 *>(drow + 128 * g + 32 * ks);
                ga[g][0] = tm_mma_bf16(a, bb[g][0][ks], ga[g][0]);
                ga[g][1] = tm_mma_bf16(a, bb[g][1][ks], ga[g][1]);
            }
#pragma unroll
        for (int r = 0; r < 4; ++r)
#pragma unroll
            for (int ct = 0; ct < 2; ++ct) {
                gxs[(4 * lg + r) * TM_LDF + col0 + 16 * ct] = ga[0][ct][r];
                gns[(4 * lg + r) * TM_LDF + col0 + 16 * ct] = ga[1][ct][r];
            }
    }
    lds_barrier();
    if (p.stop == 5) return;

    if (live) {
        const float inv_n = 1.f / (float)n;
        const float4 x0 = *reinterpret_cast<const float4 *>(gxs + sr * TM_LDF + cg * 8);
        const float4 x1 = *reinterpret_cast<const float4 *>(gxs + sr * TM_LDF + cg * 8 + 4);
        const float4 a0 = *reinterpret_cast<const float4 *>(gns + sr * TM_LDF + cg * 8);
        const float4 a1 = *reinterpret_cast<const float4 *>(gns + sr * TM_LDF + cg * 8 + 4);
        const float gx[8] = {x0.x, x0.y, x0.z, x0.w, x1.x, x1.y, x1.z, x1.w};
        const float gz[8] = {a0.x, a0.y, a0.z, a0.w, a1.x, a1.y, a1.z, a1.w};
        uint32_t zb[8];
#pragma unroll
        for (int q = 0; q < 8; ++q) zb[q] = tm_bf16(gz[q] * inv_n);
        {
            vec16 o;
#pragma unroll
            for (int q = 0; q < 8; q += 2)
                o[q >> 1] = tm_pack(((xbits >> q) & 1u) ? gx[q] : 0.f, ((xbits >> (q + 1)) & 1u) ? gx[q + 1] : 0.f);
            *reinterpret_cast<vec16 *>(p.dH + iw * TM_D + cg * 8) = o;
        }
        uint16_t *base = p.dH + (B + iw * n) * TM_D + cg * 8;
#pragma unroll
        for (int u = 0; u < NB; ++u) {
            if (N > 0 || u < n) {
                const uint32_t m = mbits[u >> 2] >> ((u & 3) * 8);
                vec16 o;
#pragma unroll
                for (int q = 0; q < 8; q += 2)
                    o[q >> 1] = (((m >> q) & 1u) ? zb[q] : 0u) | ((((m >> (q + 1)) & 1u) ? zb[q + 1] : 0u) << 16);
                *reinterpret_cast<vec16 *>(base + (int64_t)u * TM_D) = o;
            }
        }
    }
}

}

using namespace gsage;

extern "C" {

int64_t gsage_mean_tail_mfma_scratch(int32_t B, int32_t C)
{
    const int64_t n_wg = (B + TM_S - 1) / TM_S;
    return n_wg * ((int64_t)C * TM_D + C + 1);
}

int32_t gsage_mean_tail_mfma_sampler_wgs(int64_t B_hops, int64_t widest)
{
    const char *e = getenv("GSAGE_TAIL_SMP_WGS");
    const int x = e ? atoi(e) : 32;
    const int want = x >= 1 && x <= 128 ? x : 32;
    if (B_hops <= 0 || widest <= 0) return 0;
    const int64_t spw = ceil_div(B_hops, (int64_t)want);
    if (sizeof(int64_t) * 2 * (size_t)spw * (size_t)widest > tm_lds_bytes()) return 0;
    return (int32_t)ceil_div(B_hops, spw);
}

int gsage_mean_tail_mfma(const void *H, int32_t B, int32_t n, const void *w2, int64_t ldw2,
                         const void *w2t, int64_t ldw2t, const float *Wfc, const float *bfc, int32_t C,
                         const int64_t *targets, const int64_t *batch_idx, int64_t n_batches, void *agg,
                         void *dE, float *preds, void *dH, float *partial, const gsage_tail_gather_desc *gather,
                         void *stream)
{
    const int32_t *n_valid = take_head_n_valid();
    const gsage_hops_desc *hd = t_hops_role;
    t_hops_role = nullptr;
    GSAGE_REQUIRE(H && w2 && w2t && Wfc && bfc && targets && agg && dE && preds && dH && partial,
                  "mean_tail_mfma: null pointer");
    GSAGE_REQUIRE(B > 0 && n >= 1 && n <= 32 && C >= 1 && C <= TM_CMAX,
                  "mean_tail_mfma: needs fan-out <= 32 and n_classes <= %d", TM_CMAX);
    GSAGE_REQUIRE(ldw2 >= TM_D && ldw2t >= 128 && ldw2 % 8 == 0 && ldw2t % 8 == 0,
                  "mean_tail_mfma: operand copies too narrow or rows not 16-byte multiples");
    GSAGE_REQUIRE((((uintptr_t)H | (uintptr_t)w2 | (uintptr_t)w2t | (uintptr_t)Wfc | (uintptr_t)agg | (uintptr_t)dE |
                    (uintptr_t)dH) & 15) == 0, "mean_tail_mfma: buffers must be 16-byte aligned");
    GSAGE_REQUIRE(!batch_idx || n_batches > 0, "mean_tail_mfma: bad target queue");
    GSAGE_REQUIRE((int64_t)B * (1 + n) * TM_D * 2 < ((int64_t)1 << 31) && 2 * 128 * ldw2 * 2 < ((int64_t)1 << 31) &&
                  2 * TM_D * ldw2t * 2 < ((int64_t)1 << 31),
                  "mean_tail_mfma: H and the operand copies are addressed with 32-bit buffer offsets (< 2 GiB each)");
    TailMfmaParams p;
    p.H = (const uint16_t *)H; p.w2 = (const uint16_t *)w2; p.w2t = (const uint16_t *)w2t;
    p.Wfc = Wfc; p.bfc = bfc; p.targets = targets; p.batch_idx = batch_idx; p.n_batches = n_batches;
    p.n_valid = n_valid;
    p.agg = (uint16_t *)agg; p.dE = (uint16_t *)dE; p.preds = preds; p.dH = (uint16_t *)dH;
    p.partial = partial; p.ldw2 = ldw2; p.ldw2t = ldw2t; p.B = B; p.n = n; p.C = C;
    {
        const char *e = getenv("GSAGE_TAIL_STOP");
        p.stop = e ? atoi(e) : 0;
    }
    TailGather tg = {};
    const bool fused = gather && gather->rows > 0;
    if (fused) {
        const int rc = fill_gather_role(tg, *gather, "mean_tail_mfma");
        if (rc != GSAGE_OK) return rc;
    }
    HopsParams hp = {};
    p.n_smp = 0;
    if (hd) {
        GSAGE_REQUIRE(fused && !hd->dense_adj, "mean_tail_mfma: the sampler role rides beside the gather role and walks a CSR");
        size_t lds = 0;
        const int rc = fill_hops(hp, lds, *hd);
        if (rc != GSAGE_OK) return rc;
        int64_t widest = 1, width = 1;
        for (int k = 1; k <= hp.n_hops; ++k) { width *= hp.fan[k]; widest = width > widest ? width : widest; }
        p.n_smp = gsage_mean_tail_mfma_sampler_wgs(hd->B, widest);
        GSAGE_REQUIRE(p.n_smp > 0, "mean_tail_mfma: the sampler role's frontier (%lld ids per seed, twice) does not fit the "
                      "launch's LDS (gsage_mean_tail_mfma_sampler_wgs)", (long long)widest);
        hp.spw = (int32_t)ceil_div(hd->B, (int64_t)p.n_smp);
    }
    const int gn = fused ? gather->n : 0;
    const int ex = n == 25 ? 1 : n == 15 ? 2 : n == 10 ? 3 : 0;
    typedef void (*kern_t)(const TailMfmaParams, const TailGather, const HopsParams);
    static const kern_t table[4][4] = {
        {k_mean_tail_mfma<0, 0>, k_mean_tail_mfma<0, 10>, k_mean_tail_mfma<0, 5>, k_mean_tail_mfma<0, 15>},
        {k_mean_tail_mfma<25, 0>, k_mean_tail_mfma<25, 10>, k_mean_tail_mfma<25, 5>, k_mean_tail_mfma<25, 15>},
        {k_mean_tail_mfma<15, 0>, k_mean_tail_mfma<15, 10>, k_mean_tail_mfma<15, 5>, k_mean_tail_mfma<15, 15>},
        {k_mean_tail_mfma<10, 0>, k_mean_tail_mfma<10, 10>, k_mean_tail_mfma<10, 5>, k_mean_tail_mfma<10, 15>}};
    const int gi = gn == 10 ? 1 : gn == 5 ? 2 : gn == 15 ? 3 : 0;
    kern_t kern = table[ex][gi];
    {
        static bool raised[16] = {};
        const int slot = ex * 4 + gi;
        if (!raised[slot]) {
            if (hipFuncSetAttribute((const void *)kern, hipFuncAttributeMaxDynamicSharedMemorySize,
                                    (int)tm_lds_bytes()) != hipSuccess) {
                (void)hipGetLastError();
                set_error("mean_tail_mfma: cannot raise the dynamic LDS limit");
                return GSAGE_ELAUNCH;
            }
            raised[slot] = true;
        }
    }
    const unsigned n_tail = (unsigned)((B + TM_S - 1) / TM_S);
    launch(kern, dim3(n_tail + (unsigned)p.n_smp + (fused ? (unsigned)tg.n_wg : 0u)), dim3(TM_T), tm_lds_bytes(),
           (hipStream_t)stream, p, tg, hp);
    return check_launch("mean_tail_mfma");
}

}
```

pytorch-graphsage_amd/engine/mean.py:

```python
import ctypes
import os

import torch

from .. import _native as nat
from .. import ops
from ..nn_modules import IdentityPrep, MeanAggregator
from .common import FusedTrainStep, _PrepDesc, _Wgrad, _round64


class FusedMeanTrainStep(FusedTrainStep):

    MEAN_ENGINE = True
    TIMED = {"gather": (0, 1), "seed_level": (2, 3), "k5": (4, 5), "k5b": (6, 7)}

    @classmethod
    def why_not(cls, model, feats, ddp=None):
        why = cls._why_not_common(model, feats, (MeanAggregator,), "mean") or \
            cls._why_not_input(model, feats, ddp, concat_ok=True, fp8_ok=True)
        if why:
            return why
        if not all(l.output_dim_ % 8 == 0 for l in model.agg_layers.children()):
            return "output dims that are not multiples of 8"
        return None

    def _init_levels(self, example_ids, example_targets):
        model, feats, dev, L, B = self.model, self.store, self.dev, self.L, self.B
        self.h = [l.output_dim_ for l in self.layers]
        if self.emb:
            d0 = self.D0 + self.E
            ld0 = _round64(d0) if (self.tdt == torch.bfloat16 or self.D0) else d0
        elif self.fp8:
            d0, ld0 = feats.dim, _round64(feats.dim)
        else:
            d0, ld0 = feats.dim, feats.ld
        self.din = [d0] + [2 * h for h in self.h[:-1]]
        self.ldin = [ld0] + [2 * h for h in self.h[:-1]]
        self.rows = [self.off[L - l] for l in range(L)]
        self.w2, self.w2t, self.wp = [], [], []
        for l, layer in enumerate(self.layers):
            h, din = self.h[l], self.din[l]
            assert tuple(layer.fc_x.weight.shape) == (h, din) == tuple(layer.fc_neib.weight.shape)
            ix, inb = self.pidx[id(layer.fc_x.weight)], self.pidx[id(layer.fc_neib.weight)]
            assert inb == ix + 1, "fc_x / fc_neib must be adjacent in the parameter order"
            w2 = torch.zeros(2, h, _round64(din), dtype=self.tdt, device=dev)
            w2t = torch.zeros(2, din, _round64(h), dtype=self.tdt, device=dev) if (l > 0 or self.emb) else None
            tail_level = self._will_fuse_tail(example_targets) and l == L - 1
            self.w2.append(w2)
            self.w2t.append(w2t)
            lda = self.ldin[l]
            packed = (self.code == nat.BF16 and lda % 64 == 0 and lda >= -(-din // 64) * 64 and not tail_level)
            gstride = nat.lib().gsage_packed_weight_elems(h, din, 1)
            wp = torch.zeros(2 * gstride, dtype=torch.bfloat16, device=dev) if packed else None
            self.wp.append(wp)
            for g, prm in enumerate((layer.fc_x.weight, layer.fc_neib.weight)):
                self._prep_descs.append(_PrepDesc(
                    prm.data_ptr(), w2[g].data_ptr() if (not packed or tail_level) else None,
                    w2t[g].data_ptr() if w2t is not None else None, h, din, w2.shape[2],
                    w2t.shape[2] if w2t is not None else 0, wp[g * gstride:].data_ptr() if packed else None,
                    4 * (-(-din // 64)), int(self.code == nat.F32), 0))
        if self.emb:
            self._init_emb()

        bf, f32 = self.tdt, torch.float32
        r0 = self.off[L + 1] if self.emb else self.rows[0]
        self.xa0_set = [torch.zeros(2, r0, ld0, dtype=bf, device=dev) for _ in range(self.nset)]
        self.g0_set = [xa[0] for xa in self.xa0_set]
        self.inplace_x = (os.environ.get("GSAGE_MEAN_INPLACE_X", "1") == "1" and self.L >= 2 and not self.emb
                          and not self.fp8)
        self.agg, self.hout, self.dc, self.dg = [], [], [], []
        for l in range(L):
            R = self.rows[l]
            ld = self.ldin[l]
            assert ld % 8 == 0
            self.agg.append(None if l == 0 else torch.zeros(R, ld, dtype=bf, device=dev))
            last = l == L - 1
            self.hout.append(torch.zeros(R, 2 * self.h[l], dtype=f32 if last else bf, device=dev))
            self.dc.append(torch.zeros(R, 2 * self.h[l], dtype=bf, device=dev))
            self.dg.append(torch.zeros(R, 2 * (self.din[l] if l > 0 else self.E), dtype=f32, device=dev)
                           if (l > 0 or self.emb) else None)

    def _will_fuse_tail(self, example_targets):
        L = self.L
        hs = [l.output_dim_ for l in self.layers]
        return bool(self._will_fuse_head(example_targets) and L >= 2 and
                    2 * hs[L - 2] == 256 and 2 * hs[L - 1] == 256 and self.fan[1] <= 32 and
                    os.environ.get("GSAGE_NO_FUSED_TAIL", "0") != "1")

    def _tail_on_mfma(self):
        return self.code == nat.BF16 and os.environ.get("GSAGE_TAIL_MFMA", "1") == "1"

    def _init_reduce(self):
        srcs = self._plan_wgrad()
        prms = [p for layer in self.layers for p in (layer.fc_x.weight, layer.fc_neib.weight)]
        prms += [self.model.prep.fc.weight] if self.emb else []
        self._install_reduce([srcs[id(p)] for p in prms if id(p) in srcs])

    def _wgrad_problems(self, s):
        probs = [self._emb_wgrad_problem()] if self.emb else []
        for l in range(self.L - 1, -1, -1):
            R, h, din, dc, layer = self.rows[l], self.h[l], self.din[l], self.dc[l], self.layers[l]
            xbuf, lda = (self.xa0_set[s][0], self.ldin[0]) if l == 0 else (self.hout[l - 1], din)
            rows = None
            if l == 0 and self.inplace_x:
                xbuf, rows = self.store.data, self._front
            aggl = self.xa0_set[s][1] if l == 0 else self.agg[l]
            if h % 128 == 0:
                delta = (aggl.data_ptr() - xbuf.data_ptr()) // self.esz
                probs.append(_Wgrad(dc, xbuf, lda, delta, R, 2 * h, din, h, rows, layer.fc_x.weight))
            else:
                probs += [_Wgrad(dc, xbuf, lda, 0, R, h, din, h, rows, layer.fc_x.weight),
                          _Wgrad(dc[:, h:], aggl, lda, 0, R, h, din, h, None, layer.fc_neib.weight)]
        return probs

    def _wgrad_targets(self, probs):
        shapes = [(p.M, p.Ntot, p.K) for p in probs]
        plain = [int(os.environ.get("GSAGE_WGRAD_TARGET", "240"))] * len(shapes)
        n_wg = sum(ops.wgrad_plan(m, nt, k, t)[1] * ((nt + 127) // 128) * ((k + 127) // 128)
                   for (m, nt, k), t in zip(shapes, plain))
        cus = int(torch.cuda.get_device_properties(self.dev).multi_processor_count)
        return ops.wgrad_balance(shapes, budget=cus - 8) if n_wg > cus else plain

    def _stage_gather(self, s, with_adam=False, ids=None, hops=None, skip_rows=0, part=None, adam=None, stop_rows=None):
        L, st = self.L, self.store
        if self.emb:
            return False
        if ids is None:
            ids = self.ids_set[s]
        R = self.rows[0]
        xa = self.xa0_set[s]
        segs = []
        for k in range(L):
            n, r0 = self.fan[k + 1], (skip_rows if k == L - 1 else 0)
            r1 = self.size[k] if (k < L - 1 or stop_rows is None) else min(int(stop_rows), self.size[k])
            if r1 > r0 and (part is None or (part == "means") == (k == L - 1)):
                segs.append((st.data, ids[self.off[k + 1] + r0 * n:self.off[k + 1] + r1 * n],
                             xa[1][self.off[k] + r0:self.off[k] + r1], r1 - r0, n))
        if part != "means" and not self.inplace_x:
            segs.append((st.data, ids[:R], xa[0], R, 1))
        if adam is None and with_adam:
            adam = self._adam_desc()
        if self.fp8:
            if segs:
                ops.gather_mean_multi(segs, st.ld, st.dim, self.ldin[0], scale=st.scale)
            if adam is not None:
                self._stage_opt(adam)
            if hops is not None:
                nat.check(nat.lib().gsage_sample_hops(ctypes.addressof(hops), ops._stream()), "sample_hops")
            return bool(segs)
        if not segs:
            return False
        ops.gather_mean_multi(segs, st.ld, st.dim, st.ld, adam=adam, hops=hops)
        return True

    def _stage_compute(self, s):
        L, B, st, lib = self.L, self.B, self.store, nat.lib()
        stream = ops._stream()
        esz = self.esz
        if self.emb:
            self._prep_forward(s)
        for l in range(L - 1 if self.fused_tail else L):
            R, h, din = self.rows[l], self.h[l], self.din[l]
            rows = None
            if l == 0 and self.emb:
                xa, ld0 = self.xa0_set[s], self.ldin[0]
                xbuf, agg, lda = xa[0], xa[1], ld0
                segs = [(xa[0][self.off[k + 1]:self.off[k + 2]], None, xa[1][self.off[k]:self.off[k + 1]],
                         self.size[k], self.fan[k + 1]) for k in range(L)]
                ops.gather_mean_multi(segs, ld0, din, ld0)
            elif l == 0 and self.inplace_x:
                xbuf, agg, lda = st.data, self.xa0_set[s][1], st.ld
                rows = self._front.data_ptr()
            elif l == 0:
                xbuf, agg, lda = self.xa0_set[s][0], self.xa0_set[s][1], self.ldin[0]
            else:
                xbuf, agg, lda = self.hout[l - 1], self.agg[l], din
                segs = [(xbuf[self.off[k + 1]:self.off[k + 2]], None, agg[self.off[k]:self.off[k + 1]],
                         self.size[k], self.fan[k + 1]) for k in range(L - l)]
                ops.gather_mean_multi(segs, din, din, din)
            delta = agg.data_ptr() - xbuf.data_ptr()
            assert delta % esz == 0 and agg.stride(0) == lda
            last = l == L - 1
            if self.wp[l] is not None:
                if l == 0 and self._k5_hops is not None and self._k1_in_k5():
                    nat.check(lib.gsage_hops_role_next(ctypes.addressof(self._k5_hops)), "hops_role_next")
                if l == 0:
                    self._time_next(4, 5)
                ops._linear_packed_launch(xbuf.data_ptr(), lda, rows, int(rows is not None), self.wp[l].data_ptr(), None,
                                          self.hout[l].data_ptr(), 2 * h, R, h, din,
                                          nat.ACT_NONE if last else nat.ACT_RELU, 2, delta // esz, h,
                                          nat.F32 if last else nat.BF16)
                continue
            self._linear(xbuf.data_ptr(), lda, rows, int(rows is not None), self.w2[l].data_ptr(), self.w2[l].shape[2],
                         self.hout[l].data_ptr(), nat.F32 if last else self.code, 2 * h, R, h, din,
                         nat.ACT_NONE if last else nat.ACT_RELU, delta // esz,
                         h * self.w2[l].shape[2], h)

        m = self.model
        if self.fused_tail:
            C = m.fc.weight.shape[0]
            tg = self.queue[1] if self.queue else self.tg_set[s].view(-1)
            self._time_next(2, 3)
            self._head_live_rows()
            args = (self.hout[L - 2].data_ptr(), B, self.fan[1], self.w2[L - 1].data_ptr(),
                    self.w2[L - 1].shape[2], self.w2t[L - 1].data_ptr(), self.w2t[L - 1].shape[2],
                    m.fc.weight.data_ptr(), m.fc.bias.data_ptr(), C, tg.data_ptr(),
                    self.batch_idx.data_ptr() if self.queue else None, self.queue[2] if self.queue else 0,
                    self.agg[L - 1].data_ptr(), self.dc[L - 1].data_ptr(), self.preds.data_ptr(),
                    self.dc[L - 2].data_ptr(), self.head_scratch.data_ptr(),
                    ctypes.addressof(self._tail_gather) if self._tail_gather is not None else None)
            if self._tail_on_mfma():
                if self._k5_hops is not None and self._tail_gather is not None and self._k1_in_tail():
                    nat.check(lib.gsage_hops_role_next(ctypes.addressof(self._k5_hops)), "hops_role_next")
                nat.check(lib.gsage_mean_tail_mfma(*args, stream), "mean_tail_mfma")
            else:
                nat.check(lib.gsage_mean_tail_ce(*args, self.code, stream), "mean_tail_ce")
        else:
            self._stage_head(s)
        if self.eval_only:
            return
        self._backward_levels(s)

    def _backward_levels(self, s):
        L, lib = self.L, nat.lib()
        stream = ops._stream()
        esz = self.esz
        for l in range(L - 1, 0, -1):
            if self.fused_tail and l == L - 1:
                continue
            R, h, din = self.rows[l], self.h[l], self.din[l]
            w2t = self.w2t[l]
            self._linear(self.dc[l].data_ptr(), 2 * h, None, 0, w2t.data_ptr(), w2t.shape[2],
                         self.dg[l].data_ptr(), nat.F32, 2 * din, R, din, h, nat.ACT_NONE, h,
                         din * w2t.shape[2], din)
            below = self.hout[l - 1]
            nat.check(lib.gsage_bwd_merge(below.data_ptr(), self.code, below.stride(0), self.dg[l].data_ptr(),
                                          2 * din, din, self.dc[l - 1].data_ptr(),
                                          self.dc[l - 1].stride(0), self.rows[l - 1], R, din,
                                          L - l + 1, self.off_host, self.fan_host, stream),
                      "bwd_merge")
        if self.emb:
            R, h, E, d0 = self.rows[0], self.h[0], self.E, self.din[0]
            w2t, dg = self.w2t[0], self.dg[0]
            self._linear(self.dc[0].data_ptr(), 2 * h, None, 0, w2t.data_ptr() + self.D0 * w2t.shape[2] * esz,
                         w2t.shape[2], dg.data_ptr(), nat.F32, 2 * E, R, E, h, nat.ACT_NONE, h, d0 * w2t.shape[2], E)
            if self.rows_ok:
                self._prep_backward_rows(s, None, None, None, 0, dg.data_ptr(), 2 * E, R, dg.data_ptr() + 4 * E, 2 * E, None)
            else:
                lp = self.din0 is not self.din0f
                nat.check(lib.gsage_attn_merge_bwd2(
                    None, self.code, 0, None, 0, dg.data_ptr(), 2 * E, R, dg.data_ptr() + 4 * E, 2 * E, None,
                    self.din0f.data_ptr(), nat.F32, E, self.off[L + 1], E, L + 1, self.off_host, self.fan_host,
                    self.din0.data_ptr() if lp else None, self.din0.stride(0) if lp else 0, stream), "merge_bwd (level 0)")
                self._prep_backward(s)
        self._stage_wgrad(s)
        self._stage_finalize(s)

    def gather_launch_rows(self):
        total = self.off[self.L + 1]
        tail = self._tail_rows * self.fan[self.L]
        if self.inplace_x:
            total -= self.rows[0]
        return total - tail, tail

    def _tail_gather_rows(self):
        if not self.fused_tail or self.emb or self.fan[self.L] not in (5, 10, 15) or self.code != nat.BF16 or self.fp8:
            return 0
        mfma = self._tail_on_mfma()
        n_idle = self._tail_idle_cus(self._k1_in_tail())
        if n_idle < 32:
            return 0
        frac = float(os.environ.get("GSAGE_TAIL_GATHER_FRAC", "0.7" if mfma else "0.4"))
        n_idle = max(32, min(n_idle, int(os.environ.get("GSAGE_TAIL_GATHER_WGS", n_idle))))
        self._tail_wgs = n_idle
        per_cu = 100.0 * frac * (10.0 * 1204.0) / (self.fan[self.L] * max(self.store.dim * self.esz, 256))
        return min(int(self.size[self.L - 1]), max(int(per_cu * n_idle), 0))

    def _tail_idle_cus(self, with_sampler):
        n_cu = int(torch.cuda.get_device_properties(self.dev).multi_processor_count)
        n_idle = n_cu - ((self.B + 15) // 16 if self._tail_on_mfma() else (self.B + 3) // 4)
        if with_sampler:
            n_smp = self._tail_sampler_wgs()
            n_idle = n_idle - n_smp if n_smp > 0 else -1
        return n_idle

    def _tail_sampler_wgs(self):
        widest, width = 1, 1
        for k in range(1, self.L + 1):
            width *= int(self.fan[k])
            widest = max(widest, width)
        return int(nat.lib().gsage_mean_tail_mfma_sampler_wgs(self.B, widest))

    def _k1_early(self):
        return (not self.dense) and os.environ.get("GSAGE_DDP_K1_EARLY", "1") == "1"

    def _queue_front_means(self, par):
        self._stage_gather(self._qset(1 - par), ids=self.ids_q[1 - par], skip_rows=self._ahead_rows(), part="means",
                           hops=self._hops_desc(self.ids_q[par], True) if self._k1_early() else None)

    def _queue_front_rest(self, par):
        d = self._adam_desc()
        if not d.norm_slots:
            n = self.flat_g.numel()
            n_sq = nat.lib().gsage_adam_partials(n)
            nat.check(nat.lib().gsage_grad_sqnorm(self.flat_g.data_ptr(), n, self.partial.data_ptr(), n_sq, ops._stream()),
                      "grad_sqnorm")
            d.n_partial_ready = n_sq
        self._stage_gather(self._qset(1 - par), ids=self.ids_q[1 - par], part="rest", adam=d,
                           hops=None if (self.dense or self._k1_early()) else self._hops_desc(self.ids_q[par], True))
        if self.dense:
            self._stage_sample(0, ids=self.ids_q[par], ahead=True)

    def _k1_in_k5(self):
        if self._k1_where is not None:
            return self._k1_where == "k5"
        return bool(self.wp and self.wp[0] is not None and self.L >= 2 and not self.dense and not self.emb and
                    self.ddp is None and os.environ.get("GSAGE_K1_IN_K5", "0") == "1")

    def _k1_in_tail(self):
        if self._k1_where is not None:
            return self._k1_where == "tail"
        return bool(self.fused_tail and self._tail_on_mfma() and self.L >= 2 and not self.dense and not self.emb and
                    self.ddp is None and self.fan[self.L] in (5, 10, 15) and not self._k1_in_k5() and
                    self._tail_idle_cus(True) >= 32 and
                    float(os.environ.get("GSAGE_TAIL_GATHER_FRAC", "0.7")) > 0 and
                    os.environ.get("GSAGE_K1_IN_TAIL", "1") == "1")

    def _queue_compute_body(self, par):
        nx = self._nx(par)
        if self.P == 3:
            self._k5_hops = self._hops_desc(self.ids_q[self._nx2(par)], 2)
        if self._tail_rows:
            L, st, nxt = self.L, self.store, self.ids_q[nx]
            d = nat.TailGatherDesc()
            d.table, d.ids = st.data.data_ptr(), nxt[self.off[L]:].data_ptr()
            d.out = self.xa0_set[nx][1][self.off[L - 1]:].data_ptr()
            d.ld, d.out_ld, d.D, d.rows = st.ld, st.ld, st.dim, self._tail_rows
            d.n, d.n_workgroups = self.fan[L], self._tail_wgs
            self._tail_gather = d
        try:
            self._stage_compute(self._qset(par))
        finally:
            self._tail_gather = None
            self._k5_hops = None
```

pytorch-graphsage_amd/ops.py:

```python
import ctypes
import os

import numpy as np
import torch
import torch.nn.functional as F

from . import _native as nat
from .store import FP8, FeatureStore, RowRef, _round_up, quantize_fp8_host

_vp = ctypes.c_void_p


class _Config(object):
    compute_dtype = "bf16"


config = _Config()


def set_compute_dtype(name):
    assert name in ("bf16", "fp32")
    config.compute_dtype = name


# ... 264 lines not shown


def sample_csr_weighted(csr, ids, n, philox, out=None):
    assert n > 0, "SparseWeightedNeighborSampler: n_samples must be set explicitly"
    if csr.edge_cdf is None:
        raise ValueError("sample_csr_weighted: the adjacency carries no edge weights (DeviceCSR.with_weights)")
    ids = ids.contiguous().view(-1)
    M = int(ids.shape[0])
    seed, base, g0 = int(philox["seed"]), int(philox.get("call_base", 0)), int(philox.get("g0", 0))
    ctr = philox.get("call_ctr")
    if ids.is_cuda:
        if out is None:
            out = torch.empty(M * n, dtype=torch.int64, device=ids.device)
        assert out.dtype == torch.int64 and out.numel() == M * n and out.is_contiguous()
        nat.check(nat.lib().gsage_sample_csr_weighted(_ptr(csr.rowptr), _ptr(csr.col), _ptr(csr.edge_cdf), csr.n_rows,
                                                      _ptr(ids), M, n, seed, _ptr(ctr), base, g0, _ptr(out),
                                                      _ptr(csr.err_flag), _stream()), "sample_csr_weighted")
        return out
    idn = ids.numpy()
    if idn.size and (idn.min() < 0 or idn.max() >= csr.n_rows):
        raise IndexError("sampler: node id out of range of the adjacency")
    count = M * n
    if count == 0 or csr.nnz == 0:
        return torch.zeros(count, dtype=torch.int64)
    call = (base + (int(ctr.item()) if ctr is not None else 0)) & 0xFFFFFFFFFFFFFFFF
    g = (np.arange(count, dtype=np.uint64) + np.uint64(g0 & 0xFFFFFFFFFFFFFFFF))
    blk = g >> np.uint64(1)
    mask, s32 = np.uint64(0xFFFFFFFF), np.uint64(32)
    c = [blk & mask, blk >> s32, np.full(count, call & 0xFFFFFFFF, dtype=np.uint64),
         np.full(count, call >> 32, dtype=np.uint64)]
    k0, k1 = seed & 0xFFFFFFFF, ((seed >> 32) & 0xFFFFFFFF) ^ WEIGHTED_TAG
    for _ in range(10):
        p0 = np.uint64(0xD2511F53) * c[0]
        p1 = np.uint64(0xCD9E8D57) * c[2]
        c = [((p1 >> s32) ^ c[1] ^ np.uint64(k0)) & mask, p1 & mask, ((p0 >> s32) ^ c[3] ^ np.uint64(k1)) & mask, p0 & mask]
        k0, k1 = (k0 + 0x9E3779B9) & 0xFFFFFFFF, (k1 + 0xBB67AE85) & 0xFFFFFFFF
    odd = (g & np.uint64(1)).astype(bool)
    r64 = (np.where(odd, c[2], c[0]) << s32) | np.where(odd, c[3], c[1])
    rp, col, cdf = csr.rowptr.numpy(), csr.col.numpy(), csr.edge_cdf.numpy().view(np.uint64)
    beg, end = np.repeat(rp[idn], n), np.repeat(rp[idn + 1], n)
    T = np.where(end > beg, cdf[np.maximum(end, 1) - 1], np.uint64(0)).astype(np.uint64)
    live = T > 0
    x = _mulhi64(r64, T)
    lo, hi = np.where(live, beg, 0), np.where(live, end - 1, 0)
    while True:
        act = lo < hi
        if not act.any():
            break
        mid = (lo + hi) >> 1
        gt = cdf[mid] > x
        hi = np.where(act & gt, mid, hi)
        lo = np.where(act & ~gt, mid + 1, lo)
    vals = col[lo].astype(np.int64) if col.shape[0] else np.zeros(count, dtype=np.int64)
    return torch.from_numpy(np.where(live, vals, 0).astype(np.int64))


UNSUP_TAG_LEN, UNSUP_TAG_STEP, UNSUP_TAG_NEG = 0x4C000000, 0x53000000, 0x4E000000


def _philox4(ctr, key):
    c0, c1, c2, c3 = ctr
    k0, k1 = key
    m = 0xFFFFFFFF
    for _ in range(10):
        p0, p1 = 0xD2511F53 * c0, 0xCD9E8D57 * c2
        c0, c1, c2, c3 = ((p1 >> 32) ^ c1 ^ k0) & m, p1 & m, ((p0 >> 32) ^ c3 ^ k1) & m, p0 & m
        k0, k1 = (k0 + 0x9E3779B9) & m, (k1 + 0xBB67AE85) & m
    return c0, c1, c2, c3


def neg_cdf(csr):
    deg = (csr.rowptr[1:] - csr.rowptr[:-1]).to(torch.float64)
    cdf = torch.cumsum(deg.clamp(min=0).pow(0.75), 0).contiguous()
    cdf._gsage_total = float(cdf[-1].item())
    return cdf


def unsup_batch(csr, seeds, walk_len, Q, cdf, philox):
    seeds = seeds.contiguous().view(-1)
    B, Q, walk_len = int(seeds.shape[0]), int(Q), int(walk_len)
    total = getattr(cdf, "_gsage_total", None)
    if total is None:
        total = float(cdf[-1].item())
    seed, base, g0 = int(philox["seed"]), int(philox.get("call_base", 0)), int(philox.get("g0", 0))
    ctr = philox.get("call_ctr")
    if seeds.is_cuda:
        assert cdf.dtype == torch.float64 and cdf.is_cuda and cdf.is_contiguous() and cdf.numel() == csr.n_rows
        ids = torch.empty(2 * B + Q, dtype=torch.int64, device=seeds.device)
        pair_w = torch.empty(B, dtype=torch.float32, device=seeds.device)
        nat.check(nat.lib().gsage_unsup_batch(_ptr(csr.rowptr), _ptr(csr.col), csr.n_rows, _ptr(seeds), B, walk_len, Q,
                                              _ptr(cdf), total, seed, _ptr(ctr), base, g0, _ptr(ids), _ptr(pair_w),
                                              _ptr(csr.err_flag), _stream()), "unsup_batch")
        return ids, pair_w
    if not (B > 0 and Q > 0 and 1 <= walk_len <= 16):
        raise ValueError("unsup_batch: needs B > 0, Q > 0 and 1 <= walk_len <= 16")
    if not (total > 0.0 and total < float("inf")):
        raise ValueError("unsup_batch: the negatives' weights sum to %g" % total)
    call = (base + (int(ctr.item()) if ctr is not None else 0)) & 0xFFFFFFFFFFFFFFFF
    clo, chi = call & 0xFFFFFFFF, call >> 32
    klo, khi = seed & 0xFFFFFFFF, (seed >> 32) & 0xFFFFFFFF
    rp, col, sd, n_rows = csr.rowptr.numpy(), csr.col.numpy(), seeds.numpy(), csr.n_rows
    if sd.min() < 0 or sd.max() >= n_rows:
        raise IndexError("unsup_batch: node id out of range of the adjacency")
    ids = np.zeros(2 * B + Q, dtype=np.int64)
    pair_w = np.zeros(B, dtype=np.float32)
    for i in range(B):
        g = (g0 + i) & 0xFFFFFFFFFFFFFFFF
        c = (g & 0xFFFFFFFF, g >> 32, clo, chi)
        t = 1 + ((_philox4(c, (klo, khi ^ UNSUP_TAG_LEN))[0] * walk_len) >> 32)
        v, r = int(sd[i]), None
        for j in range(t):
            beg = int(rp[v])
            deg = int(rp[v + 1]) - beg
            if deg <= 0:
                break
            if j & 3 == 0:
                r = _philox4(c, (klo, khi ^ (UNSUP_TAG_STEP | (j >> 2))))
            word = r[j & 3]
            v = int(col[beg + ((word * deg) >> 32 if deg <= 0xFFFFFFFF else word)])
            if v < 0 or v >= n_rows:
                raise IndexError("unsup_batch: node id out of range of the adjacency")
        ids[i], ids[B + i], pair_w[i] = sd[i], v, 0.0 if v == sd[i] else 1.0
    cn = cdf.numpy()
    for q in range(Q):
        r = _philox4((q & 0xFFFFFFFF, q >> 32, clo, chi), (klo, khi ^ UNSUP_TAG_NEG))
        x = np.float64((r[0] << 21) | (r[1] >> 11)) * np.float64(2.0 ** -53) * np.float64(total)
        ids[2 * B + q] = min(int(np.searchsorted(cn, x, side="right")), n_rows - 1)
    return torch.from_numpy(ids), torch.from_numpy(pair_w)


def _gather_mean_raw(table, D, ids, M, n, out_dtype, out_ld=None, out=None):
    if out_ld is None:
        out_ld = D
    if table.is_cuda:
        if out is None:
            out = (torch.zeros if out_ld != D else torch.empty)(M, out_ld, dtype=out_dtype,
                                                                device=table.device)
        else:
            assert out.dtype == out_dtype and out.stride(0) == out_ld and out.shape[0] == M
        nat.check(nat.lib().gsage_gather_mean(_ptr(table), _code(table.dtype), table.stride(0),
                                              _ptr(ids), M, n, D, _ptr(out), _code(out_dtype),
                                              out_ld, _stream()), "gather_mean")
        return out
    rows = table[ids.view(-1), :D] if ids is not None else table[:M * n, :D]
    res = rows.float().view(M, n, D).mean(dim=1) if n > 1 else rows.float().view(M, D)
    out = torch.zeros(M, out_ld, dtype=out_dtype)
    out[:, :D] = res.to(out_dtype)
    return out


def quantize_fp8(table, D, ld_q):
    R = int(table.shape[0])
    assert table.dtype in (torch.float32, torch.bfloat16) and table.stride(1) == 1 and ld_q % 16 == 0 and ld_q >= D
    if table.is_cuda:
        q = torch.empty(R, ld_q, dtype=FP8, device=table.device)
        scale = torch.empty(ld_q, dtype=torch.float32, device=table.device)
        nat.check(nat.lib().gsage_quantize_fp8(_ptr(table), _code(table.dtype), table.stride(0), R, D, _ptr(q), ld_q,
                                               _ptr(scale), _stream()), "quantize_fp8")
        return q, scale
    q = torch.zeros(R, ld_q, dtype=torch.uint8).view(FP8)
    scale = torch.ones(ld_q, dtype=torch.float32)
    q[:, :D], scale[:D] = quantize_fp8_host(table[:, :D])
    return q, scale


def _gather_mean_fp8_raw(table_q, scale, D, ids, M, n, out_dtype, out_ld=None, out=None):
    assert table_q.dtype == FP8 and scale is not None and scale.dtype == torch.float32
    if out_ld is None:
        out_ld = D
    if table_q.is_cuda:
        if out is None:
            out = (torch.zeros if out_ld != D else torch.empty)(M, out_ld, dtype=out_dtype, device=table_q.device)
        else:
            assert out.dtype == out_dtype and out.stride(0) == out_ld and out.shape[0] == M
        nat.check(nat.lib().gsage_gather_mean_fp8(_ptr(table_q), table_q.stride(0), _ptr(scale), _ptr(ids), M, n, D,
                                                  _ptr(out), _code(out_dtype), out_ld, _stream()), "gather_mean_fp8")
        return out
    rows = table_q[ids.view(-1), :D] if ids is not None else table_q[:M * n, :D]
    res = (rows.float().view(M, n, D).mean(dim=1) if n > 1 else rows.float().view(M, D)) * scale[:D]
    out = torch.zeros(M, out_ld, dtype=out_dtype)
    out[:, :D] = res.to(out_dtype)
    return out


def _store_gather(store, D, ids, M, n, out_dtype, out_ld=None):
    if store.is_fp8:
        return _gather_mean_fp8_raw(store.data, store.scale, D, ids, M, n, out_dtype, out_ld)
    return _gather_mean_raw(store.data, D, ids, M, n, out_dtype, out_ld)


def decoded_rows(ref, compute_dtype=None):
    if not (isinstance(ref, RowRef) and ref.store.is_fp8):
        return ref
    st = ref.store
    cdt = torch_dtype(compute_dtype)
    ld = _round_up(st.dim, 64 if cdt == torch.bfloat16 else 32)
    buf = _gather_mean_fp8_raw(st.data, st.scale, st.dim, ref.ids, int(ref.ids.shape[0]), 1, cdt, ld)
    return mark_zero_padded(buf[:, :st.dim])


class _GatherTrainable(torch.autograd.Function):

    @staticmethod
    def forward(ctx, table, ids):
        ctx.save_for_backward(ids)
        ctx.tshape = table.shape
        ctx.table = table if (table.is_leaf and table.requires_grad) else None
        return _gather_mean_raw(table.detach(), table.shape[1], ids, int(ids.shape[0]), 1,
                                torch.float32)

    @staticmethod
    def backward(ctx, g):
        (ids,) = ctx.saved_tensors
        g = g.contiguous().float()
        t = ctx.table
        if (g.is_cuda and t is not None and t.grad is not None and t.grad.dtype == torch.float32 and
                t.grad.shape == t.shape and t.grad.is_contiguous() and not torch.is_grad_enabled()):
            nat.check(nat.lib().gsage_scatter_add_rows(_ptr(g), g.stride(0), _ptr(ids), int(ids.shape[0]), 1,
                                                       g.shape[1], 1.0, _ptr(t.grad), t.grad.stride(0),
                                                       _stream()), "scatter_add_rows")
            return None, None
        grad = torch.zeros(ctx.tshape, dtype=torch.float32, device=g.device)
        if g.is_cuda:
            nat.check(nat.lib().gsage_scatter_add_rows(_ptr(g), g.stride(0), _ptr(ids),
                                                       int(ids.shape[0]), 1, g.shape[1], 1.0,
                                                       _ptr(grad), grad.stride(0), _stream()),
                      "scatter_add_rows")
        else:
            grad.index_add_(0, ids, g)
        return grad, None


def embedding_rows(table, ids):
    return _GatherTrainable.apply(table, ids.contiguous().view(-1))


def gather_rows(store, ids, out_dtype=torch.float32):
    ids = ids.contiguous().view(-1)
    return _store_gather(store, store.dim, ids, int(ids.shape[0]), 1, out_dtype)


def gather_mean(store, ids, M, n, out_dtype=torch.float32, out_ld=None):
    ids = ids.contiguous().view(-1)
    assert ids.shape[0] == M * n
    if out_ld is not None and out_ld == store.ld:
        return _store_gather(store, store.ld, ids, M, n, out_dtype, out_ld)
    return _store_gather(store, store.dim, ids, M, n, out_dtype, out_ld)


class _SegmentMean(torch.autograd.Function):
    @staticmethod
    def forward(ctx, neibs, M, out_dtype):
        n = neibs.shape[0] // M
        ctx.dims = (M, n, neibs.shape[1], neibs.dtype)
        src = neibs.detach()
        if not src.is_contiguous():
            src = src.contiguous()
        return _gather_mean_raw(src, src.shape[1], None, M, n, out_dtype)

    @staticmethod
    def backward(ctx, g):
        M, n, D, dt = ctx.dims
        g = g.contiguous().float()
        if g.is_cuda:
            out = torch.empty(M * n, D, dtype=torch.float32, device=g.device)
            nat.check(nat.lib().gsage_segment_mean_bwd(_ptr(g), g.stride(0), M, n, D, _ptr(out), D,
                                                       _stream()), "segment_mean_bwd")
        else:
            out = (g / n).repeat_interleave(n, dim=0)
        return out.to(dt), None, None


def segment_mean(neibs, M, out_dtype=torch.float32):
    assert neibs.shape[0] % M == 0
    return _SegmentMean.apply(neibs, M, out_dtype)


def _linear_launch(A, lda, a_rows, a_rows_g0, W, ldw, bias, C, ldc, M, N, K, act, groups,
                   a_gs, w_gs, c_gs, dtype_code, c_code):
    nat.check(nat.lib().gsage_linear_nt(A, dtype_code, lda, a_rows, a_rows_g0, W, ldw, bias, C,
                                        c_code, ldc, M, N, K, act, groups, a_gs, w_gs, c_gs,
                                        _stream()), "linear_nt")


def pack_weight(W, K=None, out=None):
    W3 = W if W.dim() == 3 else W.unsqueeze(0)
    assert W3.stride(2) == 1 and W3.is_cuda
    groups, N, _ = W3.shape
    K = int(W3.shape[2] if K is None else K)
    n = nat.lib().gsage_packed_weight_elems(N, K, groups)
    if out is None:
        out = torch.empty(n, dtype=torch.bfloat16, device=W.device)
    assert out.numel() >= n and out.dtype == torch.bfloat16
    code = nat.BF16 if W3.dtype == torch.bfloat16 else nat.F32
    assert W3.dtype in (torch.bfloat16, torch.float32)
    nat.check(nat.lib().gsage_pack_weight(W3.data_ptr(), code, W3.stride(1), W3.stride(0) if groups > 1 else 0,
                                          N, K, groups, out.data_ptr(), _stream()), "pack_weight")
    return out


def _linear_packed_launch(A, lda, a_rows, a_rows_g0, Wp, bias, C, ldc, M, N, K, act, groups, a_gs, c_gs, c_code):
    nat.check(nat.lib().gsage_linear_nt_packed(A, lda, a_rows, a_rows_g0, Wp, bias, C, c_code, ldc, M, N, K,
                                               act, groups, a_gs, c_gs, _stream()), "linear_nt_packed")


def _prep_weight(W, cdt, epc):
    return _pad_cast(W.detach(), cdt, epc)


def gather_mean_multi(segments, ld, D, out_ld, adam=None, hops=None, scale=None):
    k = len(segments)
    T = (ctypes.c_void_p * k)(*[s[0].data_ptr() for s in segments])
    I = (ctypes.c_void_p * k)(*[(s[1].data_ptr() if s[1] is not None else None) for s in segments])
    O = (ctypes.c_void_p * k)(*[s[2].data_ptr() for s in segments])
    Ms = (ctypes.c_int64 * k)(*[int(s[3]) for s in segments])
    ns = (ctypes.c_int32 * k)(*[int(s[4]) for s in segments])
    code, ocode = _code(segments[0][0].dtype), _code(segments[0][2].dtype)
    assert all(s[0].dtype == segments[0][0].dtype and s[2].dtype == segments[0][2].dtype for s in segments)
    assert (code == nat.FP8) == (scale is not None), "an FP8 table, and only an FP8 table, comes with its scales"
    if code == nat.FP8:
        assert adam is None and hops is None, "gather_mean_multi: the FP8 launch carries no side roles"
        nat.check(nat.lib().gsage_gather_mean_multi_fp8(k, T, I, O, Ms, ns, _ptr(scale), ld, D, ocode, out_ld,
                                                        _stream()), "gather_mean_multi_fp8")
        return
    if adam is not None or hops is not None:
        nat.check(nat.lib().gsage_gather_mean_multi_adam(
            k, T, I, O, Ms, ns, code, ld, D, code, out_ld,
            ctypes.addressof(adam) if adam is not None else None,
            ctypes.addressof(hops) if hops is not None else None, _stream()), "gather_mean_multi_adam")
        return
    nat.check(nat.lib().gsage_gather_mean_multi(k, T, I, O, Ms, ns, code, ld, D, ocode, out_ld,
                                                _stream()), "gather_mean_multi")


def wgrad_plan(M, Ntot, K, target=240):
    ldk = _round_up(K, 4)
    tiles = ((Ntot + 127) // 128) * ((ldk + 127) // 128)
    s_target = max(1, target // tiles)
    rps = max(256, _round_up((M + s_target - 1) // s_target, 16))
    return rps, (M + rps - 1) // rps, ldk


def wgrad_balance(shapes, budget=248, group=8):
    targets = []
    for i in range(0, len(shapes), group):
        chunk = shapes[i:i + group]
        tiles = [((nt + 127) // 128) * ((_round_up(k, 4) + 127) // 128) for (_m, nt, k) in chunk]
        R = 256
        while sum(t * ((m + R - 1) // R) for t, (m, _nt, _k) in zip(tiles, chunk)) > budget and R < max(m for m, _, _ in chunk):
            R += 16
        targets += [t * ((m + R - 1) // R) for t, (m, _nt, _k) in zip(tiles, chunk)]
    return targets


def wgrad(dC, A, lda, a_gstride, M, Ntot, K, n_per_group, out=None, slabs=None, reduce=True):
    groups = (Ntot + n_per_group - 1) // n_per_group
    rps, S, ldk = wgrad_plan(M, Ntot, K)
    if slabs is None:
        slabs = torch.empty(S, Ntot, ldk, dtype=torch.float32, device=dC.device)
    if reduce and out is None:
        out = torch.empty(groups, n_per_group, K, dtype=torch.float32, device=dC.device)
    nat.check(nat.lib().gsage_wgrad(_ptr(dC), _code(dC.dtype), dC.stride(0), _ptr(A), lda, a_gstride, M, Ntot, K,
                                    n_per_group, rps, _ptr(slabs), ldk, _ptr(out) if reduce else None,
                                    n_per_group * K, _stream()), "wgrad")
    return out if reduce else slabs


def wgrad_multi(problems):
    descs = (nat.WgradDesc * len(problems))()
    for d, prob in zip(descs, problems):
        dC, A, lda, a_gs, M, Ntot, K, npg, slabs = prob[:9]
        rps, S, ldk = wgrad_plan(M, Ntot, K, *[v for v in prob[9:10] if v is not None])
        assert tuple(slabs.shape) == (S, Ntot, ldk) and slabs.is_contiguous()
        rows = prob[10] if len(prob) > 10 else None
        assert rows is None or (rows.dtype == torch.int64 and rows.is_contiguous() and rows.numel() >= M)
        d.a_rows = _ptr(rows) if rows is not None else None
        d.dC, d.A, d.slabs = _ptr(dC), _ptr(A), _ptr(slabs)
        d.ldc, d.lda, d.a_gstride = dC.stride(0), lda, a_gs
        d.M, d.Ntot, d.K, d.n_per_group, d.ldk, d.rows_per_split = M, Ntot, K, npg, ldk, rps
    code = _code(problems[0][0].dtype)
    assert all(prob[0].dtype == prob[1].dtype == problems[0][0].dtype for prob in problems)
    nat.check(nat.lib().gsage_wgrad_multi(len(problems), ctypes.cast(descs, ctypes.c_void_p), code, _stream()),
              "wgrad_multi")


class _Linear(torch.autograd.Function):

    @staticmethod
    def forward(ctx, x, W, b, act, cdt_name, out_dtype):
        cdt = torch_dtype(cdt_name)
        epc = 8 if cdt == torch.bfloat16 else 4
        M, K = x.shape
        N = W.shape[0]
        xa = _pad_cast(x.detach(), cdt, 8 * epc, _trusted(x))
        wa = _prep_weight(W, cdt, 8 * epc)
        out = torch.empty(M, N, dtype=out_dtype, device=x.device)
        bf = b.detach().float().contiguous() if b is not None else None
        _linear_launch(_ptr(xa), xa.stride(0), None, 0, _ptr(wa), wa.stride(0), _ptr(bf),
                       _ptr(out), N, M, N, K, act, 1, 0, 0, 0, _code(cdt), _code(out_dtype))
        ctx.save_for_backward(xa, wa, out if act != nat.ACT_NONE else None)
        ctx.meta = (act, K, x.dtype, b is not None, W.dtype)
        return out

    @staticmethod
    def backward(ctx, g):
        xa, wa, out = ctx.saved_tensors
        act, K, xdt, has_b, wdt = ctx.meta
        g = g.float()
        if act == nat.ACT_RELU:
            g = g * (out > 0)
        elif act == nat.ACT_TANH:
            o = out.float()
            g = g * (1 - o * o)
        gc = g.to(xa.dtype)
        dx = dw = db = None
        if ctx.needs_input_grad[0]:
            dx = _dgrad(gc, wa, K).to(xdt)
        if ctx.needs_input_grad[1]:
            dw = _wgrad_any(gc, xa, K).to(wdt)
        if has_b and ctx.needs_input_grad[2]:
            db = g.sum(dim=0)
        return dx, dw, db, None, None, None


def linear(x, W, b=None, act=nat.ACT_NONE, compute_dtype=None, out_dtype=torch.float32):
    if not x.is_cuda:
        y = F.linear(x.float(), W, b)
        if act == nat.ACT_RELU:
            y = torch.relu(y)
        elif act == nat.ACT_TANH:
            y = torch.tanh(y)
        return y
    return _Linear.apply(x, W, b, act, compute_dtype or config.compute_dtype, out_dtype)


class _SageProject(torch.autograd.Function):

    @staticmethod
    def forward(ctx, x, agg, Wx, Wn, x_table, x_ids, x_dim, act, cdt_name, out_dtype):
        cdt = torch_dtype(cdt_name)
        epc = 8 if cdt == torch.bfloat16 else 4
        h = Wx.shape[0]
        M = agg.shape[0]
        Dn = Wn.shape[1]
        an = _pad_cast(agg.detach(), cdt, 8 * epc, _trusted(agg))
        if x_ids is not None:
            Dx = x_dim
            if x_table.dtype != cdt or x_table.stride(0) % epc != 0:
                xa = _gather_mean_raw(x_table, Dx, x_ids, M, 1, cdt, _round_up(Dx, epc))
                a_rows = None
            else:
                xa, a_rows = x_table, x_ids
        else:
            Dx = x.shape[1]
            xa, a_rows = _pad_cast(x.detach(), cdt, 8 * epc, _trusted(x)), None
        out = torch.empty(M, 2 * h, dtype=out_dtype, device=agg.device)
        esz = xa.element_size()
        delta = an.data_ptr() - xa.data_ptr()
        grouped = (Dx == Dn and delta % esz == 0 and xa.stride(0) == an.stride(0))
        if grouped:
            ldw = _round_up(Dx, 8 * epc)
            w2 = torch.zeros(2, h, ldw, dtype=cdt, device=agg.device)
            w2[0, :, :Dx] = Wx.detach()
            w2[1, :, :Dn] = Wn.detach()
        if grouped:
            _linear_launch(_ptr(xa), xa.stride(0), _ptr(a_rows), 1, _ptr(w2), ldw, None, _ptr(out),
                           2 * h, M, h, Dx, act, 2, delta // esz, h * ldw, h, _code(cdt),
                           _code(out_dtype))
            wxa, wna = w2[0], w2[1]
        else:
            wxa = _prep_weight(Wx, cdt, 8 * epc)
            wna = _prep_weight(Wn, cdt, 8 * epc)
            _linear_launch(_ptr(xa), xa.stride(0), _ptr(a_rows), 1, _ptr(wxa), wxa.stride(0), None,
                           _ptr(out), 2 * h, M, h, Dx, act, 1, 0, 0, 0, _code(cdt), _code(out_dtype))
            _linear_launch(_ptr(an), an.stride(0), None, 0, _ptr(wna), wna.stride(0), None,
                           _vp(out.data_ptr() + h * out.element_size()), 2 * h, M, h, Dn, act, 1,
                           0, 0, 0, _code(cdt), _code(out_dtype))
        ctx.save_for_backward(xa, a_rows, an, wxa, wna, out if act == nat.ACT_RELU else None)
        ctx.grouped = (delta // esz) if grouped else None
        ctx.meta = (act, h, Dx, Dn, x.dtype if x is not None else None, agg.dtype, Wx.dtype, cdt, epc)
        return out

    @staticmethod
    def backward(ctx, g):
        xa, a_rows, an, wxa, wna, out = ctx.saved_tensors
        act, h, Dx, Dn, xdt, adt, wdt, cdt, epc = ctx.meta
        g = g.float()
        if act == nat.ACT_RELU:
            g = g * (out > 0)
        gc = g.to(cdt)
        gx, gn = gc[:, :h], gc[:, h:]
        dx = dagg = dwx = dwn = None
        fused_w = (cdt == torch.bfloat16 and ctx.grouped is not None and h % 128 == 0 and
                   xa.stride(0) % 8 == 0 and ctx.needs_input_grad[2] and ctx.needs_input_grad[3])
        k5b_ok = cdt == torch.bfloat16 and h % 8 == 0 and gc.shape[0] >= 64 and gc.is_contiguous()
        if fused_w:
            xm = xa if a_rows is None else _gather_mean_raw(xa, an.stride(0), a_rows, an.shape[0], 1,
                                                            cdt, an.stride(0))
            dw = wgrad(gc.contiguous(), xm, xm.stride(0), (an.data_ptr() - xm.data_ptr()) // 2,
                       an.shape[0], 2 * h, Dx, h)
            dwx, dwn = dw[0].to(wdt), dw[1].to(wdt)
        if ctx.needs_input_grad[2] and not fused_w:
            if a_rows is not None:
                M = an.shape[0]
                xm = _gather_mean_raw(xa, Dx, a_rows, M, 1, cdt, _round_up(Dx, epc))
            else:
                xm = xa
            if k5b_ok and xm.stride(0) % 8 == 0:
                dwx = wgrad(gx, xm, xm.stride(0), 0, gc.shape[0], h, Dx, h)[0].to(wdt)
            else:
                dwx = _wgrad_any(gx, xm, Dx).to(wdt)
        if ctx.needs_input_grad[3] and not fused_w:
            if k5b_ok and an.stride(0) % 8 == 0:
                dwn = wgrad(gn, an, an.stride(0), 0, gc.shape[0], h, Dn, h)[0].to(wdt)
            else:
                dwn = _wgrad_any(gn, an, Dn).to(wdt)
        if ctx.needs_input_grad[0]:
            dx = _dgrad(gx, wxa, Dx).to(xdt)
        if ctx.needs_input_grad[1]:
            dagg = _dgrad(gn, wna, Dn).to(adt)
        return dx, dagg, dwx, dwn, None, None, None, None, None, None


def sage_project(x, agg, Wx, Wn, act=nat.ACT_NONE, compute_dtype=None, out_dtype=torch.float32):
    if not agg.is_cuda:
        xt = x.materialize() if isinstance(x, RowRef) else x
        y = torch.cat([F.linear(xt.float(), Wx), F.linear(agg.float(), Wn)], dim=1)
        return torch.relu(y) if act == nat.ACT_RELU else y
    cd = compute_dtype or config.compute_dtype
    x = decoded_rows(x, cd)
    if isinstance(x, RowRef):
        return _SageProject.apply(None, agg, Wx, Wn, x.store.data, x.ids, x.store.dim, act, cd,
                                  out_dtype)
    return _SageProject.apply(x, agg, Wx, Wn, None, None, 0, act, cd, out_dtype)


class _PoolMLP(torch.autograd.Function):

    @staticmethod
    def forward(ctx, neibs, Wm, bm, table, ids, dim, M, n, mode, cdt_name):
        cdt = torch_dtype(cdt_name)
        epc = 8 if cdt == torch.bfloat16 else 4
        H = Wm.shape[0]
        if ids is not None:
            K = dim
            if table.dtype != cdt or table.stride(0) % epc != 0:
                A = _gather_mean_raw(table, K, ids, M * n, 1, cdt, _round_up(K, epc))
                a_rows = None
            else:
                A, a_rows = table, ids
        else:
            K = neibs.shape[1]
            A, a_rows = _pad_cast(neibs.detach(), cdt, epc, _trusted(neibs)), None
        wa = _prep_weight(Wm, cdt, epc)
        bf = bm.detach().float().contiguous()
        pooled = torch.empty(M, H, dtype=torch.float32, device=A.device)
        argmax = torch.empty(M, H, dtype=torch.int32, device=A.device) if mode == nat.POOL_MAX else None
        nat.check(nat.lib().gsage_pool_mlp(_ptr(A), _code(cdt), A.stride(0), _ptr(a_rows), _ptr(wa),
                                           wa.stride(0), _ptr(bf), M, n, H, K, mode, _ptr(pooled),
                                           H, _ptr(argmax), None, 0, None, _stream()), "pool_mlp")
        ctx.save_for_backward(A, a_rows, wa, bf, pooled, argmax)
        ctx.meta = (M, n, H, K, mode, cdt, neibs.dtype if neibs is not None else None, Wm.dtype, epc)
        return pooled

    @staticmethod
    def backward(ctx, g):
        A, a_rows, wa, bf, pooled, argmax = ctx.saved_tensors
        M, n, H, K, mode, cdt, ndt, wdt, epc = ctx.meta
        g = g.float()
        rows = A if a_rows is None else _gather_mean_raw(A, K, a_rows, M * n, 1, cdt,
                                                         _round_up(K, epc))
        dn = dw = db = None
        fast = mode == nat.POOL_MAX and cdt == torch.bfloat16 and H % 128 == 0 and g.is_cuda
        if fast:
            g = g.contiguous()
            ghc = torch.empty(M * n, H, dtype=torch.bfloat16, device=g.device)
            nat.check(nat.lib().gsage_pool_route_bwd(_ptr(g), H, _ptr(pooled), H, _ptr(argmax), H, M, n, H,
                                                     _ptr(ghc), nat.BF16, H, _stream()), "pool_route_bwd")
            if ctx.needs_input_grad[2]:
                db = (g * (pooled > 0)).sum(dim=0)
            if ctx.needs_input_grad[1]:
                dw = wgrad(ghc, rows, rows.stride(0), 0, M * n, H, K, H)[0].to(wdt)
        else:
            if mode == nat.POOL_MAX:
                gh = torch.zeros(M, n, H, dtype=torch.float32, device=g.device)
                gh.scatter_(1, argmax.long().unsqueeze(1), (g * (pooled > 0)).unsqueeze(1))
                gh = gh.view(M * n, H)
            else:
                hid = torch.empty(M * n, H, dtype=torch.float32, device=g.device)
                ra = _pad_cast(rows, cdt, 8 * epc, True) if rows.stride(0) % (8 * epc) == 0 else _pad_cast(rows[:, :K], cdt, 8 * epc)
                wl = _pad_cast(wa[:, :K], cdt, 8 * epc)
                _linear_launch(_ptr(ra), ra.stride(0), None, 0, _ptr(wl), wl.stride(0), _ptr(bf), _ptr(hid), H, M * n, H, K,
                               nat.ACT_RELU, 1, 0, 0, 0, _code(cdt), nat.F32)
                gh = (g / n).repeat_interleave(n, dim=0) * (hid > 0)
            ghc = gh.to(cdt)
            if ctx.needs_input_grad[1]:
                dw = _wgrad_any(ghc, rows, K).to(wdt)
            if ctx.needs_input_grad[2]:
                db = gh.sum(dim=0)
        if ctx.needs_input_grad[0]:
            dn = _dgrad(ghc, wa, K).to(ndt)
        return dn, dw, db, None, None, None, None, None, None, None


def pool_mlp(neibs, Wm, bm, M, mode, compute_dtype=None):
    total = neibs.shape[0]
# ... 703 lines not shown
```

Baseline: 6.355 million seed-nodes/sec.

## Fuse neighbor-sum and ReLU-mask computation into level-0 projection epilogue for tail

The level-0 packed projection gets a segmented mode: each workgroup tile holds whole seeds plus their fan-out rows. Its epilogue writes only the seed rows to H and reduces the neighbor rows into fp32 sums and ReLU sign bitmasks. The MFMA tail kernel then reads these precomputed sums and masks instead of reloading all B*n neighbor rows, which cuts global memory traffic and the tail's load work. In exchange the projection packs fewer rows per tile (BM/(n+1) seeds, so padded rows are wasted), launches more workgroups, and does a serial per-column sum in its epilogue.

```diff
diff --git a/include/gsage.h b/include/gsage.h
--- a/include/gsage.h
+++ b/include/gsage.h
@@ -159,6 +159,10 @@
                            const void *Wp, const float *bias, void *C, int c_dtype, int64_t ldc,
                            int64_t M, int64_t N, int64_t K, int act, int groups, int64_t a_gstride,
                            int64_t c_gstride, void *stream);
+int gsage_linear_nt_packed_seg(const void *A, int64_t lda, const int64_t *a_rows, int a_rows_group0_only,
+                               const void *Wp, const float *bias, void *C, int64_t ldc, int32_t B, int32_t n,
+                               int64_t N, int64_t K, int groups, int64_t a_gstride, int64_t c_gstride,
+                               float *sums, void *masks, void *stream);
 
 int gsage_wgrad(const void *dC, int dtype, int64_t ldc, const void *A, int64_t lda, int64_t a_gstride, int64_t M,
                 int64_t Ntot, int64_t K,
@@ -302,6 +306,11 @@
                          const int64_t *targets, const int64_t *batch_idx, int64_t n_batches, void *agg,
                          void *dE, float *preds, void *dH, float *partial,
                          const gsage_tail_gather_desc *gather, void *stream);
+int gsage_mean_tail_mfma_sums(const void *H, const float *sums, const void *masks, int32_t B, int32_t n, const void *w2,
+                              int64_t ldw2, const void *w2t, int64_t ldw2t, const float *Wfc, const float *bfc, int32_t C,
+                              const int64_t *targets, const int64_t *batch_idx, int64_t n_batches, void *agg,
+                              void *dE, float *preds, void *dH, float *partial,
+                              const gsage_tail_gather_desc *gather, void *stream);
 int64_t gsage_mean_tail_mfma_scratch(int32_t B, int32_t C);
 int32_t gsage_mean_tail_mfma_sampler_wgs(int64_t B, int64_t widest);
 
diff --git a/pytorch-graphsage_amd/_native.py b/pytorch-graphsage_amd/_native.py
--- a/pytorch-graphsage_amd/_native.py
+++ b/pytorch-graphsage_amd/_native.py
@@ -93,6 +93,8 @@
     "gsage_pack_weight": (_int, [_vp, _int, _i64, _i64, _i64, _i64, _i32, _vp, _vp]),
     "gsage_linear_nt_packed": (_int, [_vp, _i64, _vp, _int, _vp, _vp, _vp, _int, _i64, _i64, _i64, _i64, _int,
                                       _int, _i64, _i64, _vp]),
+    "gsage_linear_nt_packed_seg": (_int, [_vp, _i64, _vp, _int, _vp, _vp, _vp, _i64, _i32, _i32, _i64, _i64, _int,
+                                          _i64, _i64, _vp, _vp, _vp]),
     "gsage_wgrad": (_int, [_vp, _int, _i64, _vp, _i64, _i64, _i64, _i64, _i64, _i64, _i64, _vp, _i64, _vp,
                            _i64, _vp]),
     "gsage_wgrad_slabs": (_int, [_i64, _i64]),
@@ -113,6 +115,8 @@
     "gsage_mean_tail_ce_scratch": (_i64, [_i32, _i32]),
     "gsage_mean_tail_mfma": (_int, [_vp, _i32, _i32, _vp, _i64, _vp, _i64, _vp, _vp, _i32, _vp, _vp, _i64,
                                     _vp, _vp, _vp, _vp, _vp, _vp, _vp]),
+    "gsage_mean_tail_mfma_sums": (_int, [_vp, _vp, _vp, _i32, _i32, _vp, _i64, _vp, _i64, _vp, _vp, _i32, _vp, _vp, _i64,
+                                         _vp, _vp, _vp, _vp, _vp, _vp, _vp]),
     "gsage_mean_tail_mfma_scratch": (_i64, [_i32, _i32]),
     "gsage_mean_tail_mfma_sampler_wgs": (_i32, [_i64, _i64]),
     "gsage_clip_adam_step": (_int, [_vp, _vp, _vp, _vp, _i64, _vp, _vp, _vp, _f32, _f32, _f32, _f32,
diff --git a/pytorch-graphsage_amd/csrc/gsage_packed.hip b/pytorch-graphsage_amd/csrc/gsage_packed.hip
--- a/pytorch-graphsage_amd/csrc/gsage_packed.hip
+++ b/pytorch-graphsage_amd/csrc/gsage_packed.hip
@@ -27,11 +27,14 @@
     int32_t kc_total;
     int32_t a_rows_group0_only;
     int32_t c_dtype;
+    float *seg_sums;
+    uint8_t *seg_masks;
+    int32_t seg_B, seg_n, seg_spt;
 };
 
 constexpr int WP_SMEM_VEC = (BM * (BN + 4) * 4) / 16 > WP_NBUF * (BM * CH) ? (BM * (BN + 4) * 4) / 16 : WP_NBUF * (BM * CH);
 
-template <int ACT, int GN, bool HOPS>
+template <int ACT, int GN, bool HOPS, bool SEG = false>
 __global__ void __launch_bounds__(256)
 k_linear_nt_packed(const PackedParams p, const TailGather tg, const HopsParams hp)
 {
@@ -68,7 +71,13 @@
         const int R = 32 * s2 + 8 * wave + (lane >> 3);
         const int row = (R & ~9) | ((R & 1) << 3) | ((R >> 3) & 1);
         int64_t m = m0 + row;
-        if (m >= p.M) m = p.M - 1;
+        if (SEG) {
+            const int n1 = p.seg_n + 1;
+            const int f = row / n1, j = row - f * n1;
+            const int64_t seed = (int64_t)blockIdx.x * p.seg_spt + f;
+            const bool dead = f >= p.seg_spt || seed >= p.seg_B;
+            m = dead ? (int64_t)blockIdx.x * p.seg_spt : (j == 0 ? seed : p.seg_B + seed * p.seg_n + (j - 1));
+        } else if (m >= p.M) m = p.M - 1;
         const int64_t r = a_rows ? a_rows[m] : m;
         a_src[s2] = A + r * p.lda + (cdst ^ (row & 7)) * EPC;
     }
@@ -176,6 +185,43 @@
             }
         }
         __syncthreads();
+        if (SEG) {
+            const uint16_t *tile = (const uint16_t *)smem;
+            const int n = p.seg_n, rs = n + 1, r0 = 1;
+            const int64_t seed0 = (int64_t)blockIdx.x * p.seg_spt;
+            const int live = (int)min((int64_t)p.seg_spt, (int64_t)p.seg_B - seed0);
+            for (int q = tid; q < live * (BN / 8); q += 256) {
+                const int f = q >> 4, ch = q & 15;
+                const vec16 v = *reinterpret_cast<const vec16 *>(tile + (f * rs) * ldt + ch * 8);
+                *reinterpret_cast<vec16 *>((uint16_t *)p.C + (seed0 + f) * p.ldc + cbase + ch * 8) = v;
+            }
+            for (int q = tid; q < live * BN; q += 256) {
+                const int sl = q >> 7, col = q & (BN - 1);
+                const uint16_t *cp = tile + (sl * rs + r0) * ldt + col;
+                float s = 0.f;
+                for (int u = 0; u < n; ++u) s += bf16_to_f32(cp[u * ldt]);
+                p.seg_sums[(seed0 + sl) * p.ldc + cbase + col] = s;
+            }
+            uint32_t *mw = reinterpret_cast<uint32_t *>(p.seg_masks);
+            for (int q = tid; q < live * (BN / 8) * 8; q += 256) {
+                const int w = q & 7, cgl = (q >> 3) & (BN / 8 - 1), sl = q >> 7;
+                uint32_t bits = 0;
+#pragma unroll
+                for (int j = 0; j < 4; ++j) {
+                    const int u = 4 * w + j;
+                    if (u < n) {
+                        const vec16 v = *reinterpret_cast<const vec16 *>(tile + (sl * rs + r0 + u) * ldt + cgl * 8);
+#pragma unroll
+                        for (int e = 0; e < 8; ++e) {
+                            const uint16_t h = (uint16_t)(v[e >> 1] >> ((e & 1) * 16));
+                            bits |= (bf16_to_f32(h) > 0.f ? 1u : 0u) << (j * 8 + e);
+                        }
+                    }
+                }
+                mw[((seed0 + sl) * (p.ldc / 8) + cbase / 8 + cgl) * 8 + w] = bits;
+            }
+            return;
+        }
         const int cpr = BN / epc;
         for (int q = tid; q < BM * cpr; q += 256) {
             const int row = q / cpr, ch = q - row * cpr;
@@ -718,10 +764,11 @@
     return check_launch("pack_weight");
 }
 
-int gsage_linear_nt_packed(const void *A, int64_t lda, const int64_t *a_rows, int a_rows_group0_only,
-                           const void *Wp, const float *bias, void *C, int c_dtype, int64_t ldc,
-                           int64_t M, int64_t N, int64_t K, int act, int groups, int64_t a_gstride,
-                           int64_t c_gstride, void *stream)
+static int linear_nt_packed_impl(const void *A, int64_t lda, const int64_t *a_rows, int a_rows_group0_only,
+                                 const void *Wp, const float *bias, void *C, int c_dtype, int64_t ldc,
+                                 int64_t M, int64_t N, int64_t K, int act, int groups, int64_t a_gstride,
+                                 int64_t c_gstride, int32_t seg_B, int32_t seg_n, float *seg_sums, void *seg_masks,
+                                 void *stream)
 {
     const gsage_tail_gather_desc *gd = take_gather_role();
     const gsage_hops_desc *hd = t_hops_role;
@@ -741,7 +788,20 @@
     p.kc_total = (int32_t)(ceil_div(K, 64) * 4);
     p.wp_gstride = ceil_div(N, 32) * (int64_t)p.kc_total * 64 * 8;
     p.a_rows_group0_only = a_rows_group0_only; p.c_dtype = c_dtype;
+    p.seg_sums = seg_sums; p.seg_masks = (uint8_t *)seg_masks;
+    p.seg_B = seg_B; p.seg_n = seg_n; p.seg_spt = 0;
     dim3 grid((unsigned)ceil_div(M, BM), (unsigned)ceil_div(N, BN), (unsigned)groups);
+    const bool seg = seg_B > 0;
+    if (seg) {
+        GSAGE_REQUIRE(seg_sums && seg_masks && seg_n >= 1 && seg_n <= 32 && act == ACT_RELU && c_dtype == GSAGE_BF16,
+                      "linear_nt_packed_seg: needs sums, masks, fan-out <= 32, ReLU and bf16 rows");
+        GSAGE_REQUIRE(N % BN == 0 && ldc % 8 == 0 && c_gstride % 8 == 0 && ((uintptr_t)C % 16) == 0 &&
+                      ((uintptr_t)seg_sums % 16) == 0 && ((uintptr_t)seg_masks % 16) == 0 &&
+                      (groups - 1) * c_gstride + N <= ldc,
+                      "linear_nt_packed_seg: whole 128-column blocks and 16-byte aligned rows");
+        p.seg_spt = BM / (seg_n + 1);
+        grid.x = (unsigned)ceil_div((int64_t)seg_B, p.seg_spt);
+    }
     hipStream_t s = (hipStream_t)stream;
     TailGather tg = {};
     HopsParams hp = {};
@@ -760,7 +820,8 @@
                       "linear_nt_packed: the sampler role's frontier (%d seeds x %lld ids, twice) does not fit the "
                       "projection's LDS", hp.spw, (long long)widest);
         grid.z += 1;
-        launch(k_linear_nt_packed<ACT_RELU, 0, true>, grid, dim3(256), 0, s, p, tg, hp);
+        if (seg) launch(k_linear_nt_packed<ACT_RELU, 0, true, true>, grid, dim3(256), 0, s, p, tg, hp);
+        else launch(k_linear_nt_packed<ACT_RELU, 0, true>, grid, dim3(256), 0, s, p, tg, hp);
         return check_launch("linear_nt_packed");
     }
     if (gd && gd->rows > 0) {
@@ -770,8 +831,14 @@
                       "linear_nt_packed: the gather role rides with the ReLU projection, fan-out 5 or 10");
         tg.n_wg = (int32_t)(grid.x * grid.y);
         grid.z += 1;
-        if (gd->n == 10) launch(k_linear_nt_packed<ACT_RELU, 10, false>, grid, dim3(256), 0, s, p, tg, hp);
+        if (seg && gd->n == 10) launch(k_linear_nt_packed<ACT_RELU, 10, false, true>, grid, dim3(256), 0, s, p, tg, hp);
+        else if (seg) launch(k_linear_nt_packed<ACT_RELU, 5, false, true>, grid, dim3(256), 0, s, p, tg, hp);
+        else if (gd->n == 10) launch(k_linear_nt_packed<ACT_RELU, 10, false>, grid, dim3(256), 0, s, p, tg, hp);
         else launch(k_linear_nt_packed<ACT_RELU, 5, false>, grid, dim3(256), 0, s, p, tg, hp);
+        return check_launch("linear_nt_packed");
+    }
+    if (seg) {
+        launch(k_linear_nt_packed<ACT_RELU, 0, false, true>, grid, dim3(256), 0, s, p, tg, hp);
         return check_launch("linear_nt_packed");
     }
     {
@@ -833,6 +900,30 @@
     return check_launch("linear_nt_packed");
 }
 
+int gsage_linear_nt_packed(const void *A, int64_t lda, const int64_t *a_rows, int a_rows_group0_only,
+                           const void *Wp, const float *bias, void *C, int c_dtype, int64_t ldc,
+                           int64_t M, int64_t N, int64_t K, int act, int groups, int64_t a_gstride,
+                           int64_t c_gstride, void *stream)
+{
+    return linear_nt_packed_impl(A, lda, a_rows, a_rows_group0_only, Wp, bias, C, c_dtype, ldc, M, N, K, act, groups,
+                                 a_gstride, c_gstride, 0, 0, nullptr, nullptr, stream);
+}
+
+int gsage_linear_nt_packed_seg(const void *A, int64_t lda, const int64_t *a_rows, int a_rows_group0_only,
+                               const void *Wp, const float *bias, void *C, int64_t ldc, int32_t B, int32_t n,
+                               int64_t N, int64_t K, int groups, int64_t a_gstride, int64_t c_gstride,
+                               float *sums, void *masks, void *stream)
+{
+    if (B <= 0 || n < 1) {
+        (void)take_gather_role();
+        t_hops_role = nullptr;
+        GSAGE_REQUIRE(false, "linear_nt_packed_seg: bad B / fan-out");
+    }
+    return linear_nt_packed_impl(A, lda, a_rows, a_rows_group0_only, Wp, bias, C, GSAGE_BF16, ldc,
+                                 (int64_t)B * (1 + n), N, K, ACT_RELU, groups, a_gstride, c_gstride, B, n, sums, masks,
+                                 stream);
+}
+
 int gsage_pool_mlp_packed(const void *A, int64_t lda, const int64_t *a_rows, const void *Wp,
                           const float *bias, int64_t M, int32_t n, int64_t H, int64_t K, int pool,
                           float *pooled, int64_t pooled_ld, int32_t *argmax, void *pooled_bf16,
diff --git a/pytorch-graphsage_amd/csrc/gsage_tail_mfma.hip b/pytorch-graphsage_amd/csrc/gsage_tail_mfma.hip
--- a/pytorch-graphsage_amd/csrc/gsage_tail_mfma.hip
+++ b/pytorch-graphsage_amd/csrc/gsage_tail_mfma.hip
@@ -34,6 +34,8 @@
     int32_t B, n, C;
     int32_t stop;
     int32_t n_smp;
+    const float *sums;
+    const uint32_t *masks;
 };
 
 constexpr size_t tm_lds_bytes()
@@ -98,7 +100,7 @@
 #ifndef GSAGE_TM_ROLE_U
 #define GSAGE_TM_ROLE_U 2
 #endif
-template <int N, int GN>
+template <int N, int GN, bool SUMS = false>
 __global__ void __launch_bounds__(TM_T)
 k_mean_tail_mfma(const TailMfmaParams p, const TailGather tg, const HopsParams hp)
 {
@@ -151,10 +153,18 @@
 #pragma unroll
         for (int u = 0; u < 8; ++u) wf[u] = tm_bload(rF, (uint32_t)t * 16u, (uint32_t)u * TM_T * 16u);
     }
-    const __amdgpu_buffer_rsrc_t rH = tm_rsrc(p.H, (uint32_t)(B * (1 + n) * TM_D * 2));
+    const __amdgpu_buffer_rsrc_t rH = tm_rsrc(p.H, (uint32_t)(B * (SUMS ? 1 : 1 + n) * TM_D * 2));
     vec16 xraw = tm_bload(rH, (uint32_t)(iwc * TM_D + cg * 8) * 2u, 0u);
-    vec16 nb[NB];
-    {
+    vec16 nb[SUMS ? 1 : NB];
+    vec16 sm[2], mk[2];
+    if (SUMS) {
+        const __amdgpu_buffer_rsrc_t rS = tm_rsrc(p.sums, (uint32_t)(B * TM_D * 4));
+        const __amdgpu_buffer_rsrc_t rM = tm_rsrc(p.masks, (uint32_t)(B * 32 * 32));
+        sm[0] = tm_bload(rS, (uint32_t)(iwc * TM_D + cg * 8) * 4u, 0u);
+        sm[1] = tm_bload(rS, (uint32_t)(iwc * TM_D + cg * 8) * 4u, 16u);
+        mk[0] = tm_bload(rM, (uint32_t)(iwc * 32 + cg) * 32u, 0u);
+        mk[1] = tm_bload(rM, (uint32_t)(iwc * 32 + cg) * 32u, 16u);
+    } else {
         const uint32_t base = (uint32_t)((B + iwc * n) * TM_D + cg * 8) * 2u;
 #pragma unroll
         for (int u = 0; u < NB; ++u) {
@@ -174,7 +184,7 @@
             bw[1][ks] = tm_bload(rW, wr + ct1, 64u * ks);
         }
     };
-    if (N > 0) load_fwd_frags();
+    if (N > 0 || SUMS) load_fwd_frags();
     __builtin_amdgcn_sched_barrier(0);
 #pragma unroll
     for (int u = 0; u < 8; ++u) {
@@ -191,8 +201,14 @@
         for (int e = 0; e < 8; ++e) s[e] = 0.f;
 #pragma unroll
         for (int w = 0; w < (NB + 3) / 4; ++w) mbits[w] = 0;
-#pragma unroll
-        for (int u = 0; u < NB; ++u) {
+        if (SUMS) {
+#pragma unroll
+            for (int e = 0; e < 8; ++e) s[e] = __uint_as_float(sm[e >> 2][e & 3]);
+#pragma unroll
+            for (int w = 0; w < (NB + 3) / 4; ++w) mbits[w] = mk[w >> 2][w & 3];
+        }
+#pragma unroll
+        for (int u = 0; u < (SUMS ? 0 : NB); ++u) {
             const bool valid = N > 0 || u < n;
 #pragma unroll
             for (int e = 0; e < 8; ++e) {
@@ -218,7 +234,7 @@
         *reinterpret_cast<vec16 *>(xs + sr * TM_LDH + cg * 8) = live ? xraw : zero;
         *reinterpret_cast<vec16 *>(as + sr * TM_LDH + cg * 8) = live ? am : zero;
     }
-    if (N == 0) load_fwd_frags();
+    if (N == 0 && !SUMS) load_fwd_frags();
     const float my_bias = (lane < C) ? p.bfc[lane] : 0.f;
     const int64_t tg0 = (row0 + 2 * wave < B) ? tgt[row0 + 2 * wave] : -1;
     const int64_t tg1 = (row0 + 2 * wave + 1 < B) ? tgt[row0 + 2 * wave + 1] : -1;
@@ -466,11 +482,11 @@
     return (int32_t)ceil_div(B_hops, spw);
 }
 
-int gsage_mean_tail_mfma(const void *H, int32_t B, int32_t n, const void *w2, int64_t ldw2,
-                         const void *w2t, int64_t ldw2t, const float *Wfc, const float *bfc, int32_t C,
-                         const int64_t *targets, const int64_t *batch_idx, int64_t n_batches, void *agg,
-                         void *dE, float *preds, void *dH, float *partial, const gsage_tail_gather_desc *gather,
-                         void *stream)
+static int mean_tail_mfma_impl(const void *H, int32_t B, int32_t n, const void *w2, int64_t ldw2,
+                               const void *w2t, int64_t ldw2t, const float *Wfc, const float *bfc, int32_t C,
+                               const int64_t *targets, const int64_t *batch_idx, int64_t n_batches, void *agg,
+                               void *dE, float *preds, void *dH, float *partial, const gsage_tail_gather_desc *gather,
+                               const float *sums, const void *masks, void *stream)
 {
     const int32_t *n_valid = take_head_n_valid();
     const gsage_hops_desc *hd = t_hops_role;
@@ -493,6 +509,8 @@
     p.n_valid = n_valid;
     p.agg = (uint16_t *)agg; p.dE = (uint16_t *)dE; p.preds = preds; p.dH = (uint16_t *)dH;
     p.partial = partial; p.ldw2 = ldw2; p.ldw2t = ldw2t; p.B = B; p.n = n; p.C = C;
+    p.sums = sums; p.masks = (const uint32_t *)masks;
+    GSAGE_REQUIRE((((uintptr_t)sums | (uintptr_t)masks) & 15) == 0, "mean_tail_mfma_sums: buffers must be 16-byte aligned");
     {
         const char *e = getenv("GSAGE_TAIL_STOP");
         p.stop = e ? atoi(e) : 0;
@@ -520,16 +538,25 @@
     const int gn = fused ? gather->n : 0;
     const int ex = n == 25 ? 1 : n == 15 ? 2 : n == 10 ? 3 : 0;
     typedef void (*kern_t)(const TailMfmaParams, const TailGather, const HopsParams);
-    static const kern_t table[4][4] = {
+    static const kern_t table[2][4][4] = {{
         {k_mean_tail_mfma<0, 0>, k_mean_tail_mfma<0, 10>, k_mean_tail_mfma<0, 5>, k_mean_tail_mfma<0, 15>},
         {k_mean_tail_mfma<25, 0>, k_mean_tail_mfma<25, 10>, k_mean_tail_mfma<25, 5>, k_mean_tail_mfma<25, 15>},
         {k_mean_tail_mfma<15, 0>, k_mean_tail_mfma<15, 10>, k_mean_tail_mfma<15, 5>, k_mean_tail_mfma<15, 15>},
-        {k_mean_tail_mfma<10, 0>, k_mean_tail_mfma<10, 10>, k_mean_tail_mfma<10, 5>, k_mean_tail_mfma<10, 15>}};
+        {k_mean_tail_mfma<10, 0>, k_mean_tail_mfma<10, 10>, k_mean_tail_mfma<10, 5>, k_mean_tail_mfma<10, 15>}}, {
+        {k_mean_tail_mfma<0, 0, true>, k_mean_tail_mfma<0, 10, true>, k_mean_tail_mfma<0, 5, true>,
+         k_mean_tail_mfma<0, 15, true>},
+        {k_mean_tail_mfma<25, 0, true>, k_mean_tail_mfma<25, 10, true>, k_mean_tail_mfma<25, 5, true>,
+         k_mean_tail_mfma<25, 15, true>},
+        {k_mean_tail_mfma<15, 0, true>, k_mean_tail_mfma<15, 10, true>, k_mean_tail_mfma<15, 5, true>,
+         k_mean_tail_mfma<15, 15, true>},
+        {k_mean_tail_mfma<10, 0, true>, k_mean_tail_mfma<10, 10, true>, k_mean_tail_mfma<10, 5, true>,
+         k_mean_tail_mfma<10, 15, true>}}};
     const int gi = gn == 10 ? 1 : gn == 5 ? 2 : gn == 15 ? 3 : 0;
-    kern_t kern = table[ex][gi];
-    {
-        static bool raised[16] = {};
-        const int slot = ex * 4 + gi;
+    const int si = sums ? 1 : 0;
+    kern_t kern = table[si][ex][gi];
+    {
+        static bool raised[32] = {};
+        const int slot = si * 16 + ex * 4 + gi;
         if (!raised[slot]) {
             if (hipFuncSetAttribute((const void *)kern, hipFuncAttributeMaxDynamicSharedMemorySize,
                                     (int)tm_lds_bytes()) != hipSuccess) {
@@ -546,4 +573,29 @@
     return check_launch("mean_tail_mfma");
 }
 
-}
+int gsage_mean_tail_mfma(const void *H, int32_t B, int32_t n, const void *w2, int64_t ldw2,
+                         const void *w2t, int64_t ldw2t, const float *Wfc, const float *bfc, int32_t C,
+                         const int64_t *targets, const int64_t *batch_idx, int64_t n_batches, void *agg,
+                         void *dE, float *preds, void *dH, float *partial, const gsage_tail_gather_desc *gather,
+                         void *stream)
+{
+    return mean_tail_mfma_impl(H, B, n, w2, ldw2, w2t, ldw2t, Wfc, bfc, C, targets, batch_idx, n_batches, agg, dE, preds,
+                               dH, partial, gather, nullptr, nullptr, stream);
+}
+
+int gsage_mean_tail_mfma_sums(const void *H, const float *sums, const void *masks, int32_t B, int32_t n, const void *w2,
+                              int64_t ldw2, const void *w2t, int64_t ldw2t, const float *Wfc, const float *bfc, int32_t C,
+                              const int64_t *targets, const int64_t *batch_idx, int64_t n_batches, void *agg,
+                              void *dE, float *preds, void *dH, float *partial, const gsage_tail_gather_desc *gather,
+                              void *stream)
+{
+    if (!sums || !masks) {
+        (void)take_head_n_valid();
+        t_hops_role = nullptr;
+        GSAGE_REQUIRE(false, "mean_tail_mfma_sums: null pointer");
+    }
+    return mean_tail_mfma_impl(H, B, n, w2, ldw2, w2t, ldw2t, Wfc, bfc, C, targets, batch_idx, n_batches, agg, dE, preds,
+                               dH, partial, gather, sums, masks, stream);
+}
+
+}
diff --git a/pytorch-graphsage_amd/engine/mean.py b/pytorch-graphsage_amd/engine/mean.py
--- a/pytorch-graphsage_amd/engine/mean.py
+++ b/pytorch-graphsage_amd/engine/mean.py
@@ -79,6 +79,11 @@
             self.dc.append(torch.zeros(R, 2 * self.h[l], dtype=bf, device=dev))
             self.dg.append(torch.zeros(R, 2 * (self.din[l] if l > 0 else self.E), dtype=f32, device=dev)
                            if (l > 0 or self.emb) else None)
+        self.tail_sums_why = self._tail_sums_why(example_targets)
+        self.tail_sums = self.tail_sums_why is None
+        if self.tail_sums:
+            self.nsum = torch.zeros(B, 256, dtype=f32, device=dev)
+            self.nmask = torch.zeros(B, 32, 32, dtype=torch.uint8, device=dev)
 
     def _will_fuse_tail(self, example_targets):
         L = self.L
@@ -86,6 +91,17 @@
         return bool(self._will_fuse_head(example_targets) and L >= 2 and
                     2 * hs[L - 2] == 256 and 2 * hs[L - 1] == 256 and self.fan[1] <= 32 and
                     os.environ.get("GSAGE_NO_FUSED_TAIL", "0") != "1")
+
+    def _tail_sums_why(self, example_targets):
+        if os.environ.get("GSAGE_TAIL_SUMS", "1") == "0":
+            return "GSAGE_TAIL_SUMS=0"
+        if not (self._will_fuse_tail(example_targets) and self._tail_on_mfma()):
+            return "the seed level does not run on gsage_mean_tail_mfma"
+        if self.L != 2:
+            return "more than two levels"
+        if self.wp[0] is None or self.h[0] % 128 != 0:
+            return "the level-0 projection does not run on the packed kernel"
+        return None
 
     def _tail_on_mfma(self):
         return self.code == nat.BF16 and os.environ.get("GSAGE_TAIL_MFMA", "1") == "1"
@@ -186,6 +202,11 @@
                     nat.check(lib.gsage_hops_role_next(ctypes.addressof(self._k5_hops)), "hops_role_next")
                 if l == 0:
                     self._time_next(4, 5)
+                if self.tail_sums and l == L - 2:
+                    ops._linear_packed_seg_launch(xbuf.data_ptr(), lda, rows, int(rows is not None), self.wp[l].data_ptr(),
+                                                  None, self.hout[l].data_ptr(), 2 * h, B, self.fan[1], h, din, 2,
+                                                  delta // esz, h, self.nsum.data_ptr(), self.nmask.data_ptr())
+                    continue
                 ops._linear_packed_launch(xbuf.data_ptr(), lda, rows, int(rows is not None), self.wp[l].data_ptr(), None,
                                           self.hout[l].data_ptr(), 2 * h, R, h, din,
                                           nat.ACT_NONE if last else nat.ACT_RELU, 2, delta // esz, h,
@@ -212,7 +233,11 @@
             if self._tail_on_mfma():
                 if self._k5_hops is not None and self._tail_gather is not None and self._k1_in_tail():
                     nat.check(lib.gsage_hops_role_next(ctypes.addressof(self._k5_hops)), "hops_role_next")
-                nat.check(lib.gsage_mean_tail_mfma(*args, stream), "mean_tail_mfma")
+                if self.tail_sums:
+                    nat.check(lib.gsage_mean_tail_mfma_sums(args[0], self.nsum.data_ptr(), self.nmask.data_ptr(), *args[1:],
+                                                            stream), "mean_tail_mfma_sums")
+                else:
+                    nat.check(lib.gsage_mean_tail_mfma(*args, stream), "mean_tail_mfma")
             else:
                 nat.check(lib.gsage_mean_tail_ce(*args, self.code, stream), "mean_tail_ce")
         else:
diff --git a/pytorch-graphsage_amd/ops.py b/pytorch-graphsage_amd/ops.py
--- a/pytorch-graphsage_amd/ops.py
+++ b/pytorch-graphsage_amd/ops.py
@@ -590,6 +590,11 @@
 def _linear_packed_launch(A, lda, a_rows, a_rows_g0, Wp, bias, C, ldc, M, N, K, act, groups, a_gs, c_gs, c_code):
     nat.check(nat.lib().gsage_linear_nt_packed(A, lda, a_rows, a_rows_g0, Wp, bias, C, c_code, ldc, M, N, K,
                                                act, groups, a_gs, c_gs, _stream()), "linear_nt_packed")
+
+
+def _linear_packed_seg_launch(A, lda, a_rows, a_rows_g0, Wp, bias, C, ldc, B, n, N, K, groups, a_gs, c_gs, sums, masks):
+    nat.check(nat.lib().gsage_linear_nt_packed_seg(A, lda, a_rows, a_rows_g0, Wp, bias, C, ldc, B, n, N, K, groups,
+                                                   a_gs, c_gs, sums, masks, _stream()), "linear_nt_packed_seg")
 
 
 def _prep_weight(W, cdt, epc):
```

Result: slower. 6.280 million seed-nodes/sec (-1.2%).
